# EnricoMiccoli/nodal

Hardware: NVIDIA B200
Metric: unknowns_per_second (higher is better)
Workload: dtype f64

## Files before the change

### __graft_entry__.py

```python
import os
import subprocess
import sys

ROOT = os.path.dirname(os.path.abspath(__file__))
if ROOT not in sys.path:
    sys.path.insert(0, ROOT)


def build():
    subprocess.check_call(["make", "-C", os.path.join(ROOT, "nodal_b200", "csrc"), "-j8"])
    sys.path.insert(0, os.path.join(ROOT, "tests"))
    import helpers
    helpers.stamp_host_lib()
    helpers.amg_host_lib()
    import sources_host
    sources_host.sources_host_lib()
    import amg_cycle_host
    amg_cycle_host.amg_cycle_host_lib()
    ref_nodal = os.path.join(os.environ.get("NODAL_REFERENCE", "/root/reference"), "nodal")
    if os.path.isdir(ref_nodal) and not os.path.isfile(os.path.join(ROOT, "baseline", "_ref", "nodal", "nodal.py")):
        subprocess.call([sys.executable, os.path.join(ROOT, "baseline", "install_ref.py")])
    import nodal_b200
    from nodal_b200 import _lib
    _lib.load()


def smoke():
    import numpy as np
    import nodal_b200 as n
    import nodal_b200.equiv
    from nodal_b200 import dist as ndist
    from nodal_b200 import generators as gen
    from nodal_b200.device import Device
    from oracle import mna_oracle as orc

    N = 24
    r_cpu = orc.equivalent_resistance(orc.grid2d_rows(N), "1", "g", sparse=True, backend="dict")
    r_gpu = n.equiv.equivalent_resistance(gen.grid2d(N), "1", "g", sparse=True)
    r_jac = n.equiv.equivalent_resistance(gen.grid2d(N), "1", "g", sparse=True, precond="jacobi")
    r_amg = n.equiv.equivalent_resistance(gen.grid2d(N), "1", "g", sparse=True, precond="amg", amg={"coarse": 64})
    for r in (r_gpu, r_jac, r_amg):
        assert abs(r - r_cpu) <= 1e-9 * abs(r_cpu), (r, r_cpu)
    dev = Device.get(0)
    import copy
    net = copy.deepcopy(gen.grid2d(64))
    net.process_component(["a1", "A", "1", "1", "g"])
    table = net.table()
    csr, rhs = dev.assemble_csr(table)
    x, info = ndist.single_solver(dev).solve_amg(csr.n, np.array([0, csr.n], dtype=np.int32), csr.indptr, csr.indices,
                                                  csr.data, rhs, rtol=1e-10, gather_below=300)
    r_dist = float(x[net.nodenum["1"]])
    r64 = orc.equivalent_resistance(orc.grid2d_rows(64), "1", "g", sparse=True, backend="dict")
    assert info["status"] == 0 and info["distributed_levels"] >= 1 and abs(r_dist - r64) <= 1e-9 * abs(r64), (info, r_dist, r64)
    pg = gen.power_grid(16, 5, vdd=1.0, load=1e-3, seed=0)
    sol = n.Circuit(pg, sparse=True, eliminate_sources=True).solve()
    red = sol.stats["reduction"]
    assert red["eliminated"] and red["relres_full"] <= 1e-9 and np.all(sol.potentials() <= 1.0), sol.stats
    print(f"smoke ok: R({N}x{N} grid) default={float(r_gpu)!r} jacobi={float(r_jac)!r} amg={float(r_amg)!r} "
          f"oracle={float(r_cpu)!r}; R(64x64) partitioned-AMG form={r_dist!r} oracle={float(r64)!r}; "
          f"power grid 16x16 relres_full={red['relres_full']:.1e}")


if __name__ == "__main__":
    build()
    if len(sys.argv) > 1 and sys.argv[1] == "smoke":
        smoke()
```

### include/nodal_b200.h

```cpp
#ifndef NODAL_B200_H
#define NODAL_B200_H

#include <stdint.h>

#ifdef __cplusplus
extern "C" {
#endif

#define NODAL_ABI_VERSION 1

enum {
    NODAL_OK = 0,
    NODAL_SINGULAR = 1,
    NODAL_NOT_CONVERGED = 2,
    NODAL_BREAKDOWN = 3,
    NODAL_CUDA_ERROR = 4,
    NODAL_BAD_ARG = -1
};

enum { NODAL_T_R = 0, NODAL_T_A = 1, NODAL_T_E = 2, NODAL_T_VCVS = 3, NODAL_T_VCCS = 4,
       NODAL_T_CCVS = 5, NODAL_T_CCCS = 6 };
#define NODAL_GROUND (-1)
#define NODAL_UNUSED (-2)

typedef struct nodal_ctx nodal_ctx;

int nodal_abi_version(void);
const char* nodal_last_error(void);
uint64_t nodal_launch_count(void);
int nodal_ctx_create(int device, nodal_ctx** out);
int nodal_ctx_destroy(nodal_ctx* ctx);
int64_t nodal_ctx_workspace_bytes(nodal_ctx* ctx);

int nodal_stamp_coo(nodal_ctx* ctx, int64_t ncomp,
                    const uint8_t* type, const double* value,
                    const int32_t* a, const int32_t* b, const int32_t* c, const int32_t* d,
                    const int32_t* drv, const int32_t* branch,
                    int32_t kcl, int32_t n, int32_t stride, int32_t colbits,
                    uint64_t* keys, double* vals, void* stream);

int nodal_csr_build(nodal_ctx* ctx, int32_t n, int64_t nslots, int32_t colbits,
                    uint64_t* keys, double* vals, double* rhs,
                    int64_t* nnz_h, void* stream);
int nodal_csr_fetch(nodal_ctx* ctx, int32_t n, int64_t nnz,
                    int32_t* indptr, int32_t* indices, double* data, void* stream);
int nodal_csr_build_ordered(nodal_ctx* ctx, int32_t n, int64_t nslots, int32_t colbits,
                            uint64_t* keys, double* vals, int32_t order, double* rhs, int64_t* nnz_h,
                            void* stream);

int nodal_csr_to_dense(nodal_ctx* ctx, int32_t n, const int32_t* indptr, const int32_t* indices,
                       const double* data, double* G, void* stream);
int nodal_coo_to_dense_atomic(nodal_ctx* ctx, int32_t n, int64_t nslots, int32_t colbits,
                              const uint64_t* keys, const double* vals, double* G, double* rhs,
                              void* stream);

int nodal_spmv(nodal_ctx* ctx, int32_t n, int64_t nnz, const int32_t* indptr,
               const int32_t* indices, const double* data, const double* x, double* y,
               void* stream);

typedef struct nodal_sell nodal_sell;
int nodal_sell_create(nodal_ctx* ctx, int32_t n, int64_t nnz, const int32_t* indptr,
                      const int32_t* indices, const double* data, nodal_sell** out, void* stream);
int nodal_sell_destroy(nodal_sell* m);
int64_t nodal_sell_padded_nnz(const nodal_sell* m);
int nodal_sell_spmv(nodal_ctx* ctx, const nodal_sell* m, const double* x, double* y, void* stream);

int nodal_pcg(nodal_ctx* ctx, int32_t n, int64_t nnz, const int32_t* indptr,
              const int32_t* indices, const double* data, const double* rhs, double* x,
              double rtol, int32_t maxit, int32_t flags,
              int32_t* iters_h, double* relres_h, double* stats_h, void* stream);
#define NODAL_PCG_FORCE_CSR 1
#define NODAL_PCG_NO_GRAPH 2
#define NODAL_PCG_PROFILE 4
#define NODAL_PCG_NO_SCALE 8

int nodal_gmres(nodal_ctx* ctx, int32_t n, int64_t nnz, const int32_t* indptr,
                const int32_t* indices, const double* data, const double* rhs, double* x,
                double rtol, int32_t restart, int32_t maxit,
                int32_t* iters_h, double* relres_h, void* stream);

typedef struct nodal_amg nodal_amg;
int nodal_amg_create(nodal_ctx* ctx, int32_t n, int64_t nnz, const int32_t* indptr,
                     const int32_t* indices, const double* data, const double* params,
                     nodal_amg** out, void* stream);
int nodal_amg_destroy(nodal_amg* amg);
int nodal_amg_info(const nodal_amg* amg, int32_t cap, int32_t* nlevels, int64_t* rows, int64_t* nnz,
                   double* setup_ms, int32_t* direct);
int nodal_amg_fetch_level(nodal_ctx* ctx, const nodal_amg* amg, int32_t level, int32_t* agg,
                          int32_t* indptr, int32_t* indices, double* data, void* stream);
int nodal_amg_apply(nodal_ctx* ctx, const nodal_amg* amg, const double* r, double* z, void* stream);
int nodal_amg_pcg(nodal_ctx* ctx, nodal_amg* amg, const double* rhs, double* x, double rtol,
                  int32_t maxit, int32_t* iters_h, double* relres_h, double* stats_h, void* stream);

int nodal_connected_components(nodal_ctx* ctx, int64_t ncomp, const int32_t* a, const int32_t* b,
                               int32_t kcl, int32_t* labels, int32_t* ncomponents_h,
                               int32_t* reached_h, void* stream);

int nodal_source_forest(nodal_ctx* ctx, int64_t ncomp, const uint8_t* type, const double* value,
                        const int32_t* a, const int32_t* b, const int32_t* branch, int32_t kcl, int32_t be,
                        int32_t* erow, int32_t* adj_ptr, int32_t* adj_row, int32_t* rep_row, double* offset,
                        int32_t* parent_edge, int32_t* depth, int32_t* roots, int64_t* info_h, void* stream);
int nodal_source_reduce_scan(nodal_ctx* ctx, int64_t ncomp, const uint8_t* type, const int32_t* a,
                             const int32_t* b, int32_t kcl, const int32_t* rep_row, const double* offset,
                             uint32_t* pos, int64_t* count_h, void* stream);
int nodal_source_reduce_table(nodal_ctx* ctx, int64_t ncomp, const uint8_t* type, const double* value,
                              const int32_t* a, const int32_t* b, int32_t kcl, const int32_t* rep_row,
                              const double* offset, const uint32_t* pos, uint8_t* out_type, double* out_value,
                              int32_t* out_a, int32_t* out_b, void* stream);
int nodal_source_expand(nodal_ctx* ctx, int32_t kcl, int32_t n, int32_t nsrc, const int32_t* erow,
                        const int32_t* a, const int32_t* b, const int32_t* branch, const int32_t* adj_ptr,
                        const int32_t* adj_row, const int32_t* rep_row, const double* offset,
                        const int32_t* depth, int32_t max_depth, const double* y, const double* rhs,
                        int64_t nnz, const int32_t* indptr, const int32_t* indices, const double* data,
                        double* x, double* relres_h, void* stream);
int nodal_source_potentials(nodal_ctx* ctx, int32_t kcl, int32_t n, const int32_t* rep_row, const double* offset,
                            const double* y, double* x, void* stream);
int nodal_source_tree_rows(nodal_ctx* ctx, int32_t kcl, int32_t n, int64_t nnz_full, int32_t rb, int32_t re,
                           const int32_t* depth, const double* rhs, int64_t nnz, const int32_t* indptr,
                           const int32_t* indices, const double* data, const double* x, int32_t* out_row,
                           double* out_rhs, double* out_gx, int64_t* count_h, void* stream);
int nodal_source_currents(nodal_ctx* ctx, int32_t kcl, int32_t nsrc, const int32_t* erow, const int32_t* a,
                          const int32_t* b, const int32_t* branch, const int32_t* adj_ptr, const int32_t* adj_row,
                          const int32_t* depth, int32_t max_depth, int64_t ntree, const int32_t* tree_row,
                          const double* tree_rhs, const double* tree_gx, double* x, void* stream);
int nodal_source_residual(nodal_ctx* ctx, int32_t n, int64_t nnz_full, int32_t rows, const double* rhs, int64_t nnz,
                          const int32_t* indptr, const int32_t* indices, const double* data, const double* x,
                          double* sums_h, void* stream);

int nodal_lu_solve(nodal_ctx* ctx, int32_t n, double* G, const double* rhs, double* x,
                   int32_t* info_h, void* stream);

int nodal_dgemm_sub_profile(nodal_ctx* ctx, double* C, const double* A, const double* B, int32_t M, int32_t N,
                            int32_t K, int32_t ld, int32_t reps, double* ms_out, void* stream);

int nodal_lu_batched(nodal_ctx* ctx, int64_t batch, int32_t ncomp,
                     const uint8_t* type, const int32_t* a, const int32_t* b,
                     const int32_t* c, const int32_t* d, const int32_t* drv, const int32_t* branch,
                     int32_t kcl, int32_t n, const double* values, double* x, int32_t* info,
                     void* stream);

int nodal_lu_batched_soa(nodal_ctx* ctx, int64_t batch, int32_t ncomp,
                         const uint8_t* type, const int32_t* a, const int32_t* b,
                         const int32_t* c, const int32_t* d, const int32_t* drv, const int32_t* branch,
                         int32_t kcl, int32_t n, const double* values_t, double* x_t, int32_t* info,
                         void* stream);

typedef struct nodal_dist nodal_dist;
int nodal_dist_unique_id(uint8_t id_h[128]);
int nodal_dist_create(nodal_ctx* ctx, const uint8_t id_h[128], int32_t rank, int32_t nranks,
                      nodal_dist** out);
int nodal_dist_create_single(nodal_ctx* ctx, nodal_dist** out);
int nodal_dist_destroy(nodal_dist* d);
int nodal_dist_pcg(nodal_ctx* ctx, nodal_dist* d, int32_t n_global, const int32_t* bounds_h,
                   int64_t nnz, const int32_t* indptr, const int32_t* indices, const double* data,
                   const double* rhs_local, double* x_local,
                   double rtol, int32_t maxit,
                   int32_t* iters_h, double* relres_h, double* stats_h, void* stream);

int nodal_amg_pcg_multi(nodal_ctx* ctx, nodal_amg* amg, int32_t K, const double* rhs, double* x, double rtol,
                        int32_t maxit, int32_t* iters_h, double* relres_h, int32_t* status_h, void* stream);

int nodal_amg_profile_sweeps(nodal_ctx* ctx, nodal_amg* h, int32_t reps, double* ms_out, void* stream);

int nodal_amg_profile_cycle(nodal_ctx* ctx, nodal_amg* h, int32_t reps, double* ms_out, void* stream);

int nodal_table_select_scan(nodal_ctx* ctx, int64_t ncomp, const int32_t* a, const int32_t* b,
                            int32_t rb, int32_t re, uint32_t* pos, int64_t* count_h, void* stream);
int nodal_table_select_gather(nodal_ctx* ctx, int64_t ncomp, const uint32_t* pos, int32_t rb, int32_t re,
                              const uint8_t* type, const double* value, const int32_t* a, const int32_t* b,
                              const int32_t* c, const int32_t* d, const int32_t* drv, const int32_t* branch,
                              uint8_t* out_type, double* out_value, int32_t* out_a, int32_t* out_b,
                              int32_t* out_c, int32_t* out_d, int32_t* out_drv, int32_t* out_branch,
                              void* stream);
int nodal_table_select_mna_scan(nodal_ctx* ctx, int64_t ncomp, const uint8_t* type, const int32_t* a,
                                const int32_t* b, const int32_t* branch, int32_t kcl, int32_t rb, int32_t re,
                                uint32_t* pos, int64_t* count_h, void* stream);
int nodal_table_select_mna_gather(nodal_ctx* ctx, int64_t ncomp, const uint32_t* pos, int32_t kcl, int32_t rb,
                                  int32_t re, const uint8_t* type, const double* value, const int32_t* a,
                                  const int32_t* b, const int32_t* c, const int32_t* d, const int32_t* drv,
                                  const int32_t* branch, uint8_t* out_type, double* out_value, int32_t* out_a,
                                  int32_t* out_b, int32_t* out_c, int32_t* out_d, int32_t* out_drv,
                                  int32_t* out_branch, void* stream);
int nodal_table_select_type_scan(nodal_ctx* ctx, int64_t ncomp, const uint8_t* type, const int32_t* a,
                                 const int32_t* b, int32_t t, uint32_t* pos, int64_t* count_h, void* stream);
int nodal_table_select_type_gather(nodal_ctx* ctx, int64_t ncomp, const uint32_t* pos, int32_t t,
                                   const uint8_t* type, const double* value, const int32_t* a, const int32_t* b,
                                   const int32_t* c, const int32_t* d, const int32_t* drv, const int32_t* branch,
                                   uint8_t* out_type, double* out_value, int32_t* out_a, int32_t* out_b,
                                   int32_t* out_c, int32_t* out_d, int32_t* out_drv, int32_t* out_branch,
                                   void* stream);

int nodal_dist_amg_pcg(nodal_ctx* ctx, nodal_dist* d, int32_t n_global, const int32_t* bounds_h,
                       int64_t nnz, const int32_t* indptr, const int32_t* indices, const double* data,
                       const double* rhs_local, double* x_local, const double* params,
                       double rtol, int32_t maxit,
                       int32_t* iters_h, double* relres_h, double* stats_h, void* stream);

#ifdef __cplusplus
}
#endif
#endif
```

### nodal_b200/_lib.py

```python
from __future__ import annotations

import ctypes as C
import os

_HERE = os.path.dirname(os.path.abspath(__file__))
LIB_PATH = os.path.join(_HERE, "libnodal_b200.so")

OK, SINGULAR, NOT_CONVERGED, BREAKDOWN, CUDA_ERROR, BAD_ARG = 0, 1, 2, 3, 4, -1
PCG_FORCE_CSR, PCG_NO_GRAPH, PCG_PROFILE, PCG_NO_SCALE = 1, 2, 4, 8

_vp, _i32, _i64, _f64 = C.c_void_p, C.c_int32, C.c_int64, C.c_double

SIGNATURES = {
    "nodal_abi_version": (C.c_int, []),
    "nodal_last_error": (C.c_char_p, []),
    "nodal_launch_count": (C.c_uint64, []),
    "nodal_ctx_create": (C.c_int, [C.c_int, C.POINTER(_vp)]),
    "nodal_ctx_destroy": (C.c_int, [_vp]),
    "nodal_ctx_workspace_bytes": (_i64, [_vp]),
    "nodal_stamp_coo": (C.c_int, [_vp, _i64, _vp, _vp, _vp, _vp, _vp, _vp, _vp, _vp,
                                  _i32, _i32, _i32, _i32, _vp, _vp, _vp]),
    "nodal_csr_build": (C.c_int, [_vp, _i32, _i64, _i32, _vp, _vp, _vp, C.POINTER(_i64), _vp]),
    "nodal_csr_build_ordered": (C.c_int, [_vp, _i32, _i64, _i32, _vp, _vp, _i32, _vp, C.POINTER(_i64), _vp]),
    "nodal_csr_fetch": (C.c_int, [_vp, _i32, _i64, _vp, _vp, _vp, _vp]),
    "nodal_csr_to_dense": (C.c_int, [_vp, _i32, _vp, _vp, _vp, _vp, _vp]),
    "nodal_coo_to_dense_atomic": (C.c_int, [_vp, _i32, _i64, _i32, _vp, _vp, _vp, _vp, _vp]),
    "nodal_spmv": (C.c_int, [_vp, _i32, _i64, _vp, _vp, _vp, _vp, _vp, _vp]),
    "nodal_sell_create": (C.c_int, [_vp, _i32, _i64, _vp, _vp, _vp, C.POINTER(_vp), _vp]),
    "nodal_sell_destroy": (C.c_int, [_vp]),
    "nodal_sell_padded_nnz": (_i64, [_vp]),
    "nodal_sell_spmv": (C.c_int, [_vp, _vp, _vp, _vp, _vp]),
    "nodal_pcg": (C.c_int, [_vp, _i32, _i64, _vp, _vp, _vp, _vp, _vp, _f64, _i32, _i32,
                            C.POINTER(_i32), C.POINTER(_f64), C.POINTER(_f64), _vp]),
    "nodal_gmres": (C.c_int, [_vp, _i32, _i64, _vp, _vp, _vp, _vp, _vp, _f64, _i32, _i32,
                              C.POINTER(_i32), C.POINTER(_f64), _vp]),
    "nodal_amg_create": (C.c_int, [_vp, _i32, _i64, _vp, _vp, _vp, C.POINTER(_f64), C.POINTER(_vp), _vp]),
    "nodal_amg_destroy": (C.c_int, [_vp]),
    "nodal_amg_info": (C.c_int, [_vp, _i32, C.POINTER(_i32), C.POINTER(_i64), C.POINTER(_i64),
                                 C.POINTER(_f64), C.POINTER(_i32)]),
    "nodal_amg_fetch_level": (C.c_int, [_vp, _vp, _i32, _vp, _vp, _vp, _vp, _vp]),
    "nodal_amg_apply": (C.c_int, [_vp, _vp, _vp, _vp, _vp]),
    "nodal_amg_pcg": (C.c_int, [_vp, _vp, _vp, _vp, _f64, _i32, C.POINTER(_i32), C.POINTER(_f64),
                                C.POINTER(_f64), _vp]),
    "nodal_connected_components": (C.c_int, [_vp, _i64, _vp, _vp, _i32, _vp, C.POINTER(_i32),
                                             C.POINTER(_i32), _vp]),
    "nodal_source_forest": (C.c_int, [_vp, _i64, _vp, _vp, _vp, _vp, _vp, _i32, _i32] + [_vp] * 8
                            + [C.POINTER(_i64), _vp]),
    "nodal_source_reduce_scan": (C.c_int, [_vp, _i64, _vp, _vp, _vp, _i32, _vp, _vp, _vp, C.POINTER(_i64), _vp]),
    "nodal_source_reduce_table": (C.c_int, [_vp, _i64, _vp, _vp, _vp, _vp, _i32, _vp, _vp, _vp, _vp, _vp, _vp, _vp,
                                            _vp]),
    "nodal_source_expand": (C.c_int, [_vp, _i32, _i32, _i32] + [_vp] * 9 + [_i32, _vp, _vp, _i64, _vp, _vp, _vp, _vp,
                                                                             C.POINTER(_f64), _vp]),
    "nodal_lu_solve": (C.c_int, [_vp, _i32, _vp, _vp, _vp, C.POINTER(_i32), _vp]),
    "nodal_dgemm_sub_profile": (C.c_int, [_vp, _vp, _vp, _vp, _i32, _i32, _i32, _i32, _i32, C.POINTER(_f64), _vp]),
    "nodal_lu_batched": (C.c_int, [_vp, _i64, _i32, _vp, _vp, _vp, _vp, _vp, _vp, _vp,
                                   _i32, _i32, _vp, _vp, _vp, _vp]),
    "nodal_lu_batched_soa": (C.c_int, [_vp, _i64, _i32, _vp, _vp, _vp, _vp, _vp, _vp, _vp,
                                       _i32, _i32, _vp, _vp, _vp, _vp]),
    "nodal_dist_unique_id": (C.c_int, [_vp]),
    "nodal_dist_create": (C.c_int, [_vp, _vp, _i32, _i32, C.POINTER(_vp)]),
    "nodal_dist_create_single": (C.c_int, [_vp, C.POINTER(_vp)]),
    "nodal_dist_destroy": (C.c_int, [_vp]),
    "nodal_dist_pcg": (C.c_int, [_vp, _vp, _i32, _vp, _i64, _vp, _vp, _vp, _vp, _vp, _f64, _i32,
                                 C.POINTER(_i32), C.POINTER(_f64), C.POINTER(_f64), _vp]),
    "nodal_amg_pcg_multi": (C.c_int, [_vp, _vp, _i32, _vp, _vp, _f64, _i32, C.POINTER(_i32), C.POINTER(_f64),
                                      C.POINTER(_i32), _vp]),
    "nodal_amg_profile_sweeps": (C.c_int, [_vp, _vp, _i32, C.POINTER(_f64), _vp]),
    "nodal_amg_profile_cycle": (C.c_int, [_vp, _vp, _i32, C.POINTER(_f64), _vp]),
    "nodal_table_select_scan": (C.c_int, [_vp, _i64, _vp, _vp, _i32, _i32, _vp, C.POINTER(_i64), _vp]),
    "nodal_table_select_gather": (C.c_int, [_vp, _i64, _vp, _i32, _i32] + [_vp] * 16 + [_vp]),
    "nodal_table_select_mna_scan": (C.c_int, [_vp, _i64, _vp, _vp, _vp, _vp, _i32, _i32, _i32, _vp, C.POINTER(_i64),
                                              _vp]),
    "nodal_table_select_mna_gather": (C.c_int, [_vp, _i64, _vp, _i32, _i32, _i32] + [_vp] * 16 + [_vp]),
    "nodal_table_select_type_scan": (C.c_int, [_vp, _i64, _vp, _vp, _vp, _i32, _vp, C.POINTER(_i64), _vp]),
    "nodal_table_select_type_gather": (C.c_int, [_vp, _i64, _vp, _i32] + [_vp] * 16 + [_vp]),
    "nodal_source_potentials": (C.c_int, [_vp, _i32, _i32, _vp, _vp, _vp, _vp, _vp]),
    "nodal_source_tree_rows": (C.c_int, [_vp, _i32, _i32, _i64, _i32, _i32, _vp, _vp, _i64, _vp, _vp, _vp, _vp, _vp,
                                         _vp, _vp, C.POINTER(_i64), _vp]),
    "nodal_source_currents": (C.c_int, [_vp, _i32, _i32] + [_vp] * 7 + [_i32, _i64, _vp, _vp, _vp, _vp, _vp]),
    "nodal_source_residual": (C.c_int, [_vp, _i32, _i64, _i32, _vp, _i64, _vp, _vp, _vp, _vp, C.POINTER(_f64), _vp]),
    "nodal_dist_amg_pcg": (C.c_int, [_vp, _vp, _i32, _vp, _i64, _vp, _vp, _vp, _vp, _vp, C.POINTER(_f64), _f64,
                                     _i32, C.POINTER(_i32), C.POINTER(_f64), C.POINTER(_f64), _vp]),
}

_lib = None


class NodalLibraryError(RuntimeError):
    """The CUDA extension is missing or a CUDA call failed."""


def load():
    global _lib
    if _lib is not None:
        return _lib
    if not os.path.exists(LIB_PATH):
        raise NodalLibraryError(
            f"{LIB_PATH} not found: build it with `python -c 'import __graft_entry__ as g; g.build()'`"
            " (or `make -C nodal_b200/csrc`). nodal_b200 has no CPU fallback.")
    lib = C.CDLL(LIB_PATH)
    for name, (res, args) in SIGNATURES.items():
        fn = getattr(lib, name)
        fn.restype = res
        fn.argtypes = args
    if lib.nodal_abi_version() != 1:
        raise NodalLibraryError("libnodal_b200.so ABI version mismatch")
    _lib = lib
    return lib


def last_error():
    return load().nodal_last_error().decode("utf-8", "replace")


def check(status, what, allowed=(OK,)):
    if status in allowed:
        return status
    raise NodalLibraryError(f"{what} failed with status {status}: {last_error()}")
```

### nodal_b200/csrc/amg.cu

```cuda
#include <algorithm>
#include <cmath>

#include "amg_host.cuh"

void amg_free_csr(nodal_ctx* ctx, AmgCsr& a) {
    if (a.owned) {
        ctx_pool_free(ctx, const_cast<int32_t*>(a.indptr));
        ctx_pool_free(ctx, const_cast<int32_t*>(a.indices));
        ctx_pool_free(ctx, const_cast<double*>(a.data));
    }
    a = AmgCsr();
}

int amg_aggregate(nodal_ctx* ctx, int rounds, const AmgCsr& A, int32_t nown, int32_t base,
                  int32_t** agg_out, int32_t* nc_out, cudaStream_t st) {
    const int32_t n = A.n;
    AmgScratch<int32_t> match(ctx, n), best(ctx, n);
    AmgScratch<u32> leader(ctx, n);
    if (!match.ptr || !best.ptr || !leader.ptr) return NODAL_CUDA_ERROR;
    const int grid = amg_rows_grid(ctx, n);
    CUDA_TRY(cudaMemsetAsync(match, 0xFF, sizeof(int32_t) * (size_t)n, st));
    for (int r = 0; r < rounds; ++r) {
        amg_propose_kernel<<<grid, AT, 0, st>>>(n, A.indptr, A.indices, A.data, match, best, nown, base);
        KERNEL_CHECK();
        amg_accept_kernel<<<grid, AT, 0, st>>>(n, best, match);
        KERNEL_CHECK();
    }
    int32_t* root = best;
    amg_root_kernel<<<grid, AT, 0, st>>>(n, A.indptr, A.indices, A.data, match, root, leader, nown, base);
    KERNEL_CHECK();
    NODAL_TRY(ctx_reserve(ctx, scan_scratch_bytes(n) + 4096));
    u32* total = carve<u32>(ctx, 16);
    if (!total) return NODAL_CUDA_ERROR;
    NODAL_TRY(scan_exclusive_u32(ctx, leader, leader, n, total, st));
    int32_t* agg = match;
    amg_assign_kernel<<<grid, AT, 0, st>>>(n, root, leader, agg);
    KERNEL_CHECK();
    u32* total_h = reinterpret_cast<u32*>(ctx->pinned);
    CUDA_TRY(cudaMemcpyAsync(total_h, total, sizeof(u32), cudaMemcpyDeviceToHost, st));
    CUDA_TRY(cudaStreamSynchronize(st));
    *nc_out = (int32_t)total_h[0];
    *agg_out = match.keep();
    return NODAL_OK;
}

int amg_transpose_pattern(nodal_ctx* ctx, int32_t n, const int32_t* agg, int32_t** pt_ptr_out,
                          int32_t** pt_idx_out, cudaStream_t st) {
    AmgScratch<u64> keys(ctx, n);
    AmgScratch<double> vals(ctx, n), rhs(ctx, (size_t)n + 1), ones(ctx, n);
    if (!keys.ptr || !vals.ptr || !rhs.ptr || !ones.ptr) return NODAL_CUDA_ERROR;
    const int cb = amg_bit_length(n);
    amg_pt_keys_kernel<<<amg_rows_grid(ctx, n), AT, 0, st>>>(n, agg, cb, keys, vals);
    KERNEL_CHECK();
    int64_t cnt = 0;
    NODAL_TRY(nodal_csr_build(ctx, n, n, cb, reinterpret_cast<uint64_t*>(keys.ptr), vals, rhs, &cnt, st));
    if (cnt != n) {
        nodal_set_error("amg: internal error, P^T has %lld entries for %d rows", (long long)cnt, n);
        return NODAL_CUDA_ERROR;
    }
    AmgScratch<int32_t> pp(ctx, (size_t)n + 1), pi(ctx, n);
    if (!pp.ptr || !pi.ptr) return NODAL_CUDA_ERROR;
    NODAL_TRY(nodal_csr_fetch(ctx, n, n, pp, pi, ones, st));
    *pt_ptr_out = pp.keep();
    *pt_idx_out = pi.keep();
    return NODAL_OK;
}

int amg_members(nodal_ctx* ctx, int32_t n, const int32_t* agg, int32_t nc, int32_t** pt_ptr_out,
                int32_t** pt_idx_out, cudaStream_t st) {
    AmgScratch<u32> cnt(ctx, (size_t)nc + 1), cursor(ctx, (size_t)nc + 1);
    AmgScratch<int32_t> pp(ctx, (size_t)nc + 1), pi(ctx, (size_t)std::max(n, 1));
    if (!cnt.ptr || !cursor.ptr || !pp.ptr || !pi.ptr) return NODAL_CUDA_ERROR;
    CUDA_TRY(cudaMemsetAsync(cnt, 0, sizeof(u32) * ((size_t)nc + 1), st));
    CUDA_TRY(cudaMemsetAsync(cursor, 0, sizeof(u32) * ((size_t)nc + 1), st));
    const int grid = amg_rows_grid(ctx, n);
    amg_count_members_kernel<<<grid, AT, 0, st>>>(n, agg, cnt);
    KERNEL_CHECK();
    NODAL_TRY(ctx_reserve(ctx, scan_scratch_bytes((int64_t)nc + 1) + 4096));
    NODAL_TRY(scan_exclusive_u32(ctx, cnt, reinterpret_cast<u32*>(pp.ptr), (int64_t)nc + 1, nullptr, st));
    amg_place_members_kernel<<<grid, AT, 0, st>>>(n, agg, pp, cursor, pi);
    KERNEL_CHECK();
    amg_sort_members_kernel<<<amg_rows_grid(ctx, nc), AT, 0, st>>>(nc, pp, pi);
    KERNEL_CHECK();
    *pt_ptr_out = pp.keep();
    *pt_idx_out = pi.keep();
    return NODAL_OK;
}

int amg_galerkin_merge(nodal_ctx* ctx, const AmgCsr& A, const int32_t* pt_ptr, const int32_t* pt_idx, int32_t nc,
                       const int32_t* label, int32_t ncol_limit, AmgCsr* out, cudaStream_t st) {
    if (A.nnz >= ((int64_t)1 << 32) - 1) return NODAL_BAD_ARG;
    AmgScratch<u32> bound(ctx, (size_t)nc + 1), kept(ctx, (size_t)nc + 1);
    AmgScratch<int32_t> tmp_cols(ctx, (size_t)std::max<int64_t>(A.nnz, 1)), ip(ctx, (size_t)nc + 1);
    AmgScratch<double> tmp_vals(ctx, (size_t)std::max<int64_t>(A.nnz, 1));
    if (!bound.ptr || !kept.ptr || !tmp_cols.ptr || !tmp_vals.ptr || !ip.ptr) return NODAL_CUDA_ERROR;
    const int grid = amg_rows_grid(ctx, nc);
    CUDA_TRY(cudaMemsetAsync(bound.ptr + nc, 0, sizeof(u32), st));
    CUDA_TRY(cudaMemsetAsync(kept.ptr + nc, 0, sizeof(u32), st));
    amg_merge_bound_kernel<<<grid, AT, 0, st>>>(nc, pt_ptr, pt_idx, A.indptr, bound);
    KERNEL_CHECK();
    NODAL_TRY(ctx_reserve(ctx, scan_scratch_bytes((int64_t)nc + 1) + 4096));
    u32* total = carve<u32>(ctx, 16);
    if (!total) return NODAL_CUDA_ERROR;
    const size_t mark = ctx->arena_used;
    NODAL_TRY(scan_exclusive_u32(ctx, bound, bound, (int64_t)nc + 1, nullptr, st));
    ctx->arena_used = mark;
    amg_merge_rows_kernel<<<grid, AT, 0, st>>>(nc, pt_ptr, pt_idx, A.indptr, A.indices, A.data, label, ncol_limit,
                                               bound, tmp_cols, tmp_vals, kept);
    KERNEL_CHECK();
    NODAL_TRY(scan_exclusive_u32(ctx, kept, reinterpret_cast<u32*>(ip.ptr), (int64_t)nc + 1, total, st));
    u32* total_h = reinterpret_cast<u32*>(ctx->pinned);
    CUDA_TRY(cudaMemcpyAsync(total_h, total, sizeof(u32), cudaMemcpyDeviceToHost, st));
    CUDA_TRY(cudaStreamSynchronize(st));
    const int64_t nnzc = total_h[0];
    AmgScratch<int32_t> ix(ctx, (size_t)std::max<int64_t>(nnzc, 1));
    AmgScratch<double> dv(ctx, (size_t)std::max<int64_t>(nnzc, 1));
    if (!ix.ptr || !dv.ptr) return NODAL_CUDA_ERROR;
    amg_merge_compact_kernel<<<grid, AT, 0, st>>>(nc, bound, ip, tmp_cols, tmp_vals, ix, dv);
    KERNEL_CHECK();
    out->n = nc;
    out->nnz = nnzc;
    out->indptr = ip.keep();
    out->indices = ix.keep();
    out->data = dv.keep();
    out->owned = true;
    return NODAL_OK;
}

namespace {

int rows_grid(const nodal_ctx* ctx, int64_t work) { return amg_rows_grid(ctx, work); }
int sell_grid(const nodal_ctx* ctx, int32_t nslices) { return amg_sell_grid(ctx, nslices); }
int bit_length(int64_t v) { return amg_bit_length(v); }
template <typename T>
T* pool(nodal_ctx* ctx, size_t count) { return amg_pool<T>(ctx, count); }
template <typename T>
using Scratch = AmgScratch<T>;
using Csr = AmgCsr;
void free_csr(nodal_ctx* ctx, Csr& a) { amg_free_csr(ctx, a); }
int aggregate(nodal_amg* h, const Csr& A, int32_t** agg_out, int32_t* nc_out, cudaStream_t st) {
    return amg_aggregate(h->ctx, h->rounds, A, 0x7fffffff, 0, agg_out, nc_out, st);
}

bool sorted_galerkin() {
    static const bool on = getenv("NODAL_AMG_SORT_GALERKIN") != nullptr;
    return on;
}

int galerkin(nodal_amg* h, const Csr& A, const int32_t* agg, int32_t nc, Csr* out, cudaStream_t st) {
    nodal_ctx* ctx = h->ctx;
    if (!sorted_galerkin() && amg_merge_pays(A.nnz, nc)) {
        int32_t *pp = nullptr, *pi = nullptr;
        NODAL_TRY(amg_members(ctx, A.n, agg, nc, &pp, &pi, st));
        const int rc = amg_galerkin_merge(ctx, A, pp, pi, nc, agg, 0x7fffffff, out, st);
        ctx_pool_free(ctx, pp);
        ctx_pool_free(ctx, pi);
        return rc;
    }
    Scratch<u64> keys(ctx, A.nnz);
    Scratch<double> vals(ctx, A.nnz), rhs(ctx, (size_t)nc + 1);
    if (!keys.ptr || !vals.ptr || !rhs.ptr) return NODAL_CUDA_ERROR;
    const int cb = bit_length(nc);
    amg_relabel_kernel<<<rows_grid(ctx, A.n), AT, 0, st>>>(A.n, A.indptr, A.indices, A.data, agg, cb,
                                                         keys, vals);
    KERNEL_CHECK();
    int64_t nnzc = 0;
    NODAL_TRY(nodal_csr_build(ctx, nc, A.nnz, cb, reinterpret_cast<uint64_t*>(keys.ptr), vals, rhs,
                              &nnzc, st));
    Scratch<int32_t> ip(ctx, (size_t)nc + 1), ix(ctx, nnzc);
    Scratch<double> dv(ctx, nnzc);
    if (!ip.ptr || !ix.ptr || !dv.ptr) return NODAL_CUDA_ERROR;
    NODAL_TRY(nodal_csr_fetch(ctx, nc, nnzc, ip, ix, dv, st));
    out->n = nc;
    out->nnz = nnzc;
    out->indptr = ip.keep();
    out->indices = ix.keep();
    out->data = dv.keep();
    out->owned = true;
    return NODAL_OK;
}

int transpose_pattern(nodal_amg* h, AmgLevel& L, cudaStream_t st) {
    if (!sorted_galerkin()) return amg_members(h->ctx, L.n, L.agg, L.nc, &L.pt_ptr, &L.pt_idx, st);
    return amg_transpose_pattern(h->ctx, L.n, L.agg, &L.pt_ptr, &L.pt_idx, st);
}

int invert_coarsest(nodal_amg* h, const AmgLevel& L, cudaStream_t st) {
    nodal_ctx* ctx = h->ctx;
    const int32_t n = L.n;
    const size_t elems = (size_t)n * 2 * n;
    Scratch<double> m0(ctx, elems + 32), m1(ctx, elems);
    if (!m0.ptr || !m1.ptr) return NODAL_CUDA_ERROR;
    int* bad = reinterpret_cast<int*>(m0.ptr + elems);
    CUDA_TRY(cudaMemsetAsync(m0, 0, sizeof(double) * (elems + 32), st));
    amg_dense_init_kernel<<<rows_grid(ctx, n), AT, 0, st>>>(n, L.indptr, L.indices, L.data, m0);
    KERNEL_CHECK();
    double *src = m0.ptr, *dst = m1.ptr;
    const int grid = rows_grid(ctx, (int64_t)elems);
    for (int32_t k = 0; k < n; ++k) {
        amg_gj_step_kernel<<<grid, AT, 0, st>>>(n, k, src, dst, bad);
        KERNEL_CHECK();
        std::swap(src, dst);
    }
    h->inv = pool<double>(ctx, (size_t)n * n);
    if (!h->inv) return NODAL_CUDA_ERROR;
    amg_dense_extract_kernel<<<rows_grid(ctx, (int64_t)n * n), AT, 0, st>>>(n, src, h->inv);
    KERNEL_CHECK();
    int* bad_h = reinterpret_cast<int*>(ctx->pinned);
    CUDA_TRY(cudaMemcpyAsync(bad_h, bad, sizeof(int), cudaMemcpyDeviceToHost, st));
    CUDA_TRY(cudaStreamSynchronize(st));
    if (*bad_h != 0) {
        nodal_set_error("amg: the coarsest operator is not positive definite (pivot %d of %d); "
                        "the matrix is not SPD", *bad_h, n);
        return NODAL_BREAKDOWN;
    }
    return NODAL_OK;
}

int build_hierarchy(nodal_amg* h, int32_t n, int64_t nnz, const int32_t* indptr, const int32_t* indices,
                    const double* data, cudaStream_t st) {
    nodal_ctx* ctx = h->ctx;
    Csr cur;
    cur.n = n; cur.nnz = nnz; cur.indptr = indptr; cur.indices = indices; cur.data = data;
    while (cur.n > h->coarse && (int)h->lv.size() < h->maxlevels) {
        Csr A = cur;
        A.owned = false;
        int32_t* comp = nullptr;
        int rc = NODAL_OK;
        for (int pass = 0; pass < h->passes && rc == NODAL_OK; ++pass) {
            int32_t* agg = nullptr;
            int32_t nc = 0;
            Csr Ac;
            rc = aggregate(h, A, &agg, &nc, st);
            if (rc == NODAL_OK) rc = galerkin(h, A, agg, nc, &Ac, st);
            if (rc == NODAL_OK && comp) {
                amg_compose_kernel<<<rows_grid(ctx, cur.n), AT, 0, st>>>(cur.n, comp, agg);
                ++g_nodal_launches;
                if (cudaGetLastError() != cudaSuccess) {
                    nodal_set_error("amg: amg_compose_kernel launch failed");
                    rc = NODAL_CUDA_ERROR;
                }
            }
            if (!comp) comp = agg;
            else ctx_pool_free(ctx, agg);
            free_csr(ctx, A);
            A = Ac;
        }
        double total_nnz = (double)cur.nnz + (double)A.nnz;
        for (const AmgLevel& P : h->lv) total_nnz += (double)P.nnz;
        const bool too_dense = (double)A.nnz > h->max_fill * (double)cur.nnz ||
                               total_nnz > h->max_complexity * (double)(h->lv.empty() ? cur.nnz : h->lv[0].nnz);
        if (rc != NODAL_OK || (double)A.n > 0.9 * (double)cur.n || too_dense) {
            free_csr(ctx, A);
            ctx_pool_free(ctx, comp);
            if (rc != NODAL_OK) {
                free_csr(ctx, cur);
                return rc;
            }
            break;
        }
        AmgLevel L;
        L.n = cur.n; L.nnz = cur.nnz; L.indptr = cur.indptr; L.indices = cur.indices; L.data = cur.data;
        L.owned = cur.owned;
        L.agg = comp;
        L.nc = A.n;
        h->lv.push_back(L);
        cur = A;
        rc = transpose_pattern(h, h->lv.back(), st);
        if (rc != NODAL_OK) {
            free_csr(ctx, cur);
            return rc;
        }
    }
    AmgLevel L;
    L.n = cur.n; L.nnz = cur.nnz; L.indptr = cur.indptr; L.indices = cur.indices; L.data = cur.data;
    L.owned = cur.owned;
    h->lv.push_back(L);
    for (size_t l = 0; l < h->lv.size(); ++l) {
        AmgLevel& V = h->lv[l];
        NODAL_TRY(sell_from_csr(ctx, V.n, V.nnz, V.indptr, V.indices, V.data, &V.sell, st, nullptr));
        V.x = pool<double>(ctx, V.n);
        V.r = pool<double>(ctx, V.n);
        if (l > 0) V.b = pool<double>(ctx, V.n);
        if (!V.x || !V.r || (l > 0 && !V.b)) return NODAL_CUDA_ERROR;
    }
    if (h->lv.back().n <= h->direct_max) NODAL_TRY(invert_coarsest(h, h->lv.back(), st));
    return NODAL_OK;
}

template <int MODE>
int sell_sweep(const nodal_amg* h, const AmgLevel& V, const double* b, const double* x, double* y,
               double* part, cudaStream_t st) {
    const nodal_sell* m = V.sell;
    amg_sell_kernel<MODE><<<sell_grid(h->ctx, m->nslices), AT, 0, st>>>(
        m->n, m->nslices, m->slice_w, m->cols, m->vals, m->dinv, b, x, h->omega, y, part);
    KERNEL_CHECK();
    return NODAL_OK;
}

template <int MODE>
int cycle_sweep(const nodal_amg* h, const AmgLevel& V, const double* b, const double* xc, double* y,
                cudaStream_t st) {
    const nodal_sell* m = V.sell;
    amg_cycle_sweep_kernel<MODE><<<sell_grid(h->ctx, m->nslices), AT, 0, st>>>(
        m->n, m->nslices, m->slice_w, m->cols, m->vals, m->dinv, b, h->omega, V.agg, xc, h->scale, y);
    KERNEL_CHECK();
    return NODAL_OK;
}

int cycle(const nodal_amg* h, const double* b0, double* z0, cudaStream_t st) {
    const nodal_ctx* ctx = h->ctx;
    const int last = (int)h->lv.size() - 1;
    for (int l = 0; l < last; ++l) {
        const AmgLevel& V = h->lv[l];
        const double* b = l == 0 ? b0 : V.b;
        NODAL_TRY(cycle_sweep<1>(h, V, b, nullptr, V.r, st));
        amg_restrict_kernel<<<rows_grid(ctx, V.nc), AT, 0, st>>>(V.nc, V.pt_ptr, V.pt_idx, V.r,
                                                              h->lv[l + 1].b);
        KERNEL_CHECK();
    }
    {
        const AmgLevel& V = h->lv[last];
        const double* b = last == 0 ? b0 : V.b;
        double* x = last == 0 ? z0 : V.x;
        if (h->inv) amg_gemv_kernel<<<rows_grid(ctx, (int64_t)V.n * 32), AT, 0, st>>>(V.n, h->inv, b, x);
        else amg_jacobi0_kernel<<<rows_grid(ctx, V.n), AT, 0, st>>>(V.n, V.sell->dinv, b, h->omega, x);
        KERNEL_CHECK();
    }
    for (int l = last - 1; l >= 0; --l) {
        const AmgLevel& V = h->lv[l];
        const double* b = l == 0 ? b0 : V.b;
        NODAL_TRY(cycle_sweep<2>(h, V, b, h->lv[l + 1].x, l == 0 ? z0 : V.x, st));
    }
    return NODAL_OK;
}

}

extern "C" int nodal_amg_destroy(nodal_amg* h) {
    if (!h) return NODAL_OK;
    cudaSetDevice(h->device);
    nodal_ctx* ctx = h->ctx;
    for (AmgLevel& V : h->lv) {
        sell_free(V.sell);
        if (V.owned) {
            ctx_pool_free(ctx, const_cast<int32_t*>(V.indptr));
            ctx_pool_free(ctx, const_cast<int32_t*>(V.indices));
            ctx_pool_free(ctx, const_cast<double*>(V.data));
        }
        ctx_pool_free(ctx, V.agg);
        ctx_pool_free(ctx, V.pt_ptr);
        ctx_pool_free(ctx, V.pt_idx);
        ctx_pool_free(ctx, V.b);
        ctx_pool_free(ctx, V.x);
        ctx_pool_free(ctx, V.r);
    }
    ctx_pool_free(ctx, h->inv);
    ctx_pool_free(ctx, h->p);
    ctx_pool_free(ctx, h->q);
    ctx_pool_free(ctx, h->r);
    ctx_pool_free(ctx, h->z);
    ctx_pool_free(ctx, h->part);
    delete h;
    return NODAL_OK;
}

extern "C" int nodal_amg_create(nodal_ctx* ctx, int32_t n, int64_t nnz, const int32_t* indptr,
                                const int32_t* indices, const double* data, const double* params,
                                nodal_amg** out, void* stream) {
    NvtxRange nvtx_range("nodal_amg_create");
    if (!ctx || n < 0 || nnz < 0 || !out) return NODAL_BAD_ARG;
    *out = nullptr;
    cudaStream_t st = (cudaStream_t)stream;
    CUDA_TRY(cudaSetDevice(ctx->device));
    nodal_amg* h = new nodal_amg();
    h->ctx = ctx;
    h->device = ctx->device;
    if (params) {
        if (params[0] >= 1.0) h->passes = (int)params[0];
        if (params[1] >= 1.0) h->coarse = (int)params[1];
        if (params[2] > 0.0) h->omega = params[2];
        if (params[3] > 0.0) h->scale = params[3];
        if (params[4] >= 1.0) h->maxlevels = (int)params[4];
        if (params[5] >= 1.0) h->rounds = (int)params[5];
        if (params[6] >= 1.0) h->direct_max = (int)params[6];
        if (params[7] > 0.0) h->max_fill = params[7];
    }
    cudaEvent_t e0, e1;
    CUDA_TRY(cudaEventCreate(&e0));
    CUDA_TRY(cudaEventCreate(&e1));
    cudaEventRecord(e0, st);
    int rc = NODAL_OK;
    if (n > 0) rc = build_hierarchy(h, n, nnz, indptr, indices, data, st);
    if (rc == NODAL_OK && n > 0) {
        h->nparts = std::max(sell_grid(ctx, h->lv[0].sell->nslices), rows_grid(ctx, n));
        h->p = pool<double>(ctx, n);
        h->q = pool<double>(ctx, n);
        h->r = pool<double>(ctx, n);
        h->z = pool<double>(ctx, n);
        h->part = pool<double>(ctx, 3 * (size_t)h->nparts + 16);
        if (!h->p || !h->q || !h->r || !h->z || !h->part) rc = NODAL_CUDA_ERROR;
    }
    cudaEventRecord(e1, st);
    if (cudaEventSynchronize(e1) == cudaSuccess) cudaEventElapsedTime(&h->setup_ms, e0, e1);
    cudaEventDestroy(e0);
    cudaEventDestroy(e1);
    if (rc != NODAL_OK) {
        nodal_amg_destroy(h);
        return rc;
    }
    *out = h;
    return NODAL_OK;
}

extern "C" int nodal_amg_info(const nodal_amg* h, int32_t cap, int32_t* nlevels, int64_t* rows,
                              int64_t* nnz, double* setup_ms, int32_t* direct) {
    if (!h || !nlevels) return NODAL_BAD_ARG;
    *nlevels = (int32_t)h->lv.size();
    for (int32_t l = 0; l < *nlevels && l < cap; ++l) {
        if (rows) rows[l] = h->lv[l].n;
        if (nnz) nnz[l] = h->lv[l].nnz;
    }
    if (setup_ms) *setup_ms = h->setup_ms;
    if (direct) *direct = h->inv ? 1 : 0;
    return NODAL_OK;
}

extern "C" int nodal_amg_fetch_level(nodal_ctx* ctx, const nodal_amg* h, int32_t level, int32_t* agg,
                                     int32_t* indptr, int32_t* indices, double* data, void* stream) {
    if (!ctx || !h || level < 0 || level >= (int32_t)h->lv.size()) return NODAL_BAD_ARG;
    cudaStream_t st = (cudaStream_t)stream;
    CUDA_TRY(cudaSetDevice(ctx->device));
    const AmgLevel& V = h->lv[level];
    if (agg) {
        if (!V.agg) return NODAL_BAD_ARG;
        CUDA_TRY(cudaMemcpyAsync(agg, V.agg, sizeof(int32_t) * (size_t)V.n, cudaMemcpyDeviceToDevice, st));
    }
    if (indptr) CUDA_TRY(cudaMemcpyAsync(indptr, V.indptr, sizeof(int32_t) * ((size_t)V.n + 1), cudaMemcpyDeviceToDevice, st));
    if (indices) CUDA_TRY(cudaMemcpyAsync(indices, V.indices, sizeof(int32_t) * (size_t)V.nnz, cudaMemcpyDeviceToDevice, st));
    if (data) CUDA_TRY(cudaMemcpyAsync(data, V.data, sizeof(double) * (size_t)V.nnz, cudaMemcpyDeviceToDevice, st));
    return NODAL_OK;
}

extern "C" int nodal_amg_apply(nodal_ctx* ctx, const nodal_amg* h, const double* r, double* z,
                               void* stream) {
    if (!ctx || !h || h->ctx != ctx) return NODAL_BAD_ARG;
    if (h->lv.empty()) return NODAL_OK;
    CUDA_TRY(cudaSetDevice(ctx->device));
    return cycle(h, r, z, (cudaStream_t)stream);
}

extern "C" int nodal_amg_pcg(nodal_ctx* ctx, nodal_amg* h, const double* rhs, double* x, double rtol,
                             int32_t maxit, int32_t* iters_h, double* relres_h, double* stats_h,
                             void* stream) {
    NvtxRange nvtx_range("nodal_amg_pcg");
    if (!ctx || !h || h->ctx != ctx || !iters_h || !relres_h) return NODAL_BAD_ARG;
    *iters_h = 0;
    *relres_h = 0.0;
    if (stats_h) memset(stats_h, 0, 16 * sizeof(double));
    if (h->lv.empty()) return NODAL_OK;
    cudaStream_t st = (cudaStream_t)stream;
    CUDA_TRY(cudaSetDevice(ctx->device));
    const AmgLevel& A = h->lv[0];
    const int32_t n = A.n;
    const int gv = rows_grid(ctx, n);
    const int gs = sell_grid(ctx, A.sell->nslices);
    double* part_pq = h->part;
    double* part_rr = h->part + h->nparts;
    double* part_rz = h->part + 2 * (size_t)h->nparts;
    double* scal = h->part + 3 * (size_t)h->nparts;
    double* host = reinterpret_cast<double*>(ctx->pinned);
    cudaEvent_t e0, e1;
    CUDA_TRY(cudaEventCreate(&e0));
    CUDA_TRY(cudaEventCreate(&e1));
    int iters = 0, restarts = 0, rc = NODAL_NOT_CONVERGED;
    double relres = 0.0;
    bool timed = false;

    auto dot_to_host = [&](const double* a, const double* b, double* result) -> int {
        apcg_dot_kernel<<<gv, AT, 0, st>>>(n, a, b, part_rr);
        KERNEL_CHECK();
        apcg_sum_kernel<<<1, AT, 0, st>>>(part_rr, gv, scal + 2);
        KERNEL_CHECK();
        CUDA_TRY(cudaMemcpyAsync(host, scal + 2, sizeof(double), cudaMemcpyDeviceToHost, st));
        CUDA_TRY(cudaStreamSynchronize(st));
        *result = host[0];
        return NODAL_OK;
    };
    auto run = [&]() -> int {
        CUDA_TRY(cudaEventRecord(e0, st));
        double bb = 0.0, rr = 0.0;
        NODAL_TRY(dot_to_host(rhs, rhs, &bb));
        if (!(bb > 0.0)) {
            if (bb == 0.0) {
                CUDA_TRY(cudaMemsetAsync(x, 0, sizeof(double) * (size_t)n, st));
                rc = NODAL_OK;
                return NODAL_OK;
            }
            nodal_set_error("nodal_amg_pcg: the right-hand side is not finite");
            rc = NODAL_BREAKDOWN;
            return NODAL_OK;
        }
        const double bnorm = sqrt(bb);
        NODAL_TRY(sell_sweep<1>(h, A, rhs, x, h->r, nullptr, st));
        NODAL_TRY(dot_to_host(h->r, h->r, &rr));
        relres = sqrt(rr) / bnorm;
        while (true) {
            if (relres <= rtol) { rc = NODAL_OK; break; }
            if (iters >= maxit) { rc = NODAL_NOT_CONVERGED; break; }
            if (restarts > 8) { rc = NODAL_NOT_CONVERGED; break; }
            int par = 0;
            NODAL_TRY(cycle(h, h->r, h->z, st));
            apcg_dot_kernel<<<gv, AT, 0, st>>>(n, h->r, h->z, part_rz);
            KERNEL_CHECK();
            apcg_direction_kernel<<<gv, AT, 0, st>>>(n, part_rz, gv, scal + (par ^ 1), scal + par, h->z, h->p, 1);
            KERNEL_CHECK();
            bool broke = false;
            while (iters < maxit) {
                NODAL_TRY(sell_sweep<0>(h, A, nullptr, h->p, h->q, part_pq, st));
                apcg_update_kernel<<<gv, AT, 0, st>>>(n, part_pq, gs, scal + par, h->p, h->q, x, h->r, part_rr);
                KERNEL_CHECK();
                apcg_sum_kernel<<<1, AT, 0, st>>>(part_rr, gv, scal + 2);
                KERNEL_CHECK();
                CUDA_TRY(cudaMemcpyAsync(host, scal + 2, sizeof(double), cudaMemcpyDeviceToHost, st));
                CUDA_TRY(cudaStreamSynchronize(st));
                ++iters;
                rr = host[0];
                if (!std::isfinite(rr)) { broke = true; break; }
                if (sqrt(rr) <= rtol * bnorm) break;
                NODAL_TRY(cycle(h, h->r, h->z, st));
                apcg_dot_kernel<<<gv, AT, 0, st>>>(n, h->r, h->z, part_rz);
                KERNEL_CHECK();
                apcg_direction_kernel<<<gv, AT, 0, st>>>(n, part_rz, gv, scal + par, scal + (par ^ 1), h->z, h->p, 0);
                KERNEL_CHECK();
                par ^= 1;
            }
            if (broke) {
                nodal_set_error("nodal_amg_pcg: breakdown (non-finite residual) at iteration %d", iters);
                rc = NODAL_BREAKDOWN;
                break;
            }
            NODAL_TRY(sell_sweep<1>(h, A, rhs, x, h->r, nullptr, st));
            NODAL_TRY(dot_to_host(h->r, h->r, &rr));
            relres = sqrt(rr) / bnorm;
            if (!std::isfinite(relres)) { rc = NODAL_BREAKDOWN; break; }
            if (relres > rtol) ++restarts;
        }
        CUDA_TRY(cudaEventRecord(e1, st));
        CUDA_TRY(cudaEventSynchronize(e1));
        timed = true;
        return NODAL_OK;
    };
    const int st_run = run();
    float ms = 0.f;
    if (st_run == NODAL_OK && timed) cudaEventElapsedTime(&ms, e0, e1);
    cudaEventDestroy(e0);
    cudaEventDestroy(e1);
    if (st_run != NODAL_OK) return st_run;
    *iters_h = iters;
    *relres_h = relres;
    if (stats_h) {
        double rows = 0.0, nnz = 0.0;
        for (const AmgLevel& V : h->lv) { rows += V.n; nnz += (double)V.nnz; }
        stats_h[0] = (double)h->lv.size();
        stats_h[1] = A.nnz ? nnz / (double)A.nnz : 0.0;
        stats_h[2] = restarts;
        stats_h[3] = ms;
        stats_h[4] = h->setup_ms;
        stats_h[5] = h->lv.back().n;
        stats_h[6] = n ? rows / n : 0.0;
        stats_h[7] = h->inv ? 1.0 : 0.0;
    }
    return rc;
}

extern "C" int nodal_amg_profile_sweeps(nodal_ctx* ctx, nodal_amg* h, int32_t reps, double* ms_out, void* stream) {
    if (!ctx || !h || h->ctx != ctx || !ms_out || reps < 1 || h->lv.empty()) return NODAL_BAD_ARG;
    cudaStream_t st = (cudaStream_t)stream;
    CUDA_TRY(cudaSetDevice(ctx->device));
    const AmgLevel& A = h->lv[0];
    CUDA_TRY(cudaMemsetAsync(h->p, 0, sizeof(double) * (size_t)A.n, st));
    CUDA_TRY(cudaMemsetAsync(h->r, 0, sizeof(double) * (size_t)A.n, st));
    cudaEvent_t e0, e1;
    CUDA_TRY(cudaEventCreate(&e0));
    CUDA_TRY(cudaEventCreate(&e1));
    int rc = NODAL_OK;
    for (int mode = 0; mode < 3 && rc == NODAL_OK; ++mode) {
        for (int k = -2; k < reps && rc == NODAL_OK; ++k) {
            if (k == 0) cudaEventRecord(e0, st);
            if (mode == 0) rc = sell_sweep<0>(h, A, nullptr, h->p, h->q, h->part, st);
            if (mode == 1) rc = sell_sweep<1>(h, A, h->r, h->p, h->q, nullptr, st);
            if (mode == 2) rc = sell_sweep<2>(h, A, h->r, h->p, h->q, nullptr, st);
        }
        cudaEventRecord(e1, st);
        float ms = 0.f;
        if (cudaEventSynchronize(e1) == cudaSuccess) cudaEventElapsedTime(&ms, e0, e1);
        ms_out[mode] = ms / reps;
    }
    cudaEventDestroy(e0);
    cudaEventDestroy(e1);
    return rc;
}

extern "C" int nodal_amg_profile_cycle(nodal_ctx* ctx, nodal_amg* h, int32_t reps, double* ms_out, void* stream) {
    if (!ctx || !h || h->ctx != ctx || !ms_out || reps < 1 || h->lv.size() < 2) return NODAL_BAD_ARG;
    cudaStream_t st = (cudaStream_t)stream;
    CUDA_TRY(cudaSetDevice(ctx->device));
    const AmgLevel& A = h->lv[0];
    const AmgLevel& C = h->lv[1];
    double* b = h->r;
    CUDA_TRY(cudaMemsetAsync(b, 0, sizeof(double) * (size_t)A.n, st));
    CUDA_TRY(cudaMemsetAsync(A.x, 0, sizeof(double) * (size_t)A.n, st));
    CUDA_TRY(cudaMemsetAsync(C.x, 0, sizeof(double) * (size_t)C.n, st));
    cudaEvent_t e0, e1;
    CUDA_TRY(cudaEventCreate(&e0));
    CUDA_TRY(cudaEventCreate(&e1));
    int rc = NODAL_OK;
    for (int k = 0; k < 6 && rc == NODAL_OK; ++k) {
        for (int i = -2; i < reps && rc == NODAL_OK; ++i) {
            if (i == 0) cudaEventRecord(e0, st);
            switch (k) {
                case 0:
                    amg_jacobi0_kernel<<<rows_grid(ctx, A.n), AT, 0, st>>>(A.n, A.sell->dinv, b, h->omega, A.x);
                    KERNEL_CHECK();
                    break;
                case 1: rc = sell_sweep<1>(h, A, b, A.x, A.r, nullptr, st); break;
                case 2:
                    amg_prolong_kernel<<<rows_grid(ctx, A.n), AT, 0, st>>>(A.n, A.agg, C.x, h->scale, A.x, A.r);
                    KERNEL_CHECK();
                    break;
                case 3: rc = sell_sweep<2>(h, A, b, A.r, h->z, nullptr, st); break;
                case 4: rc = cycle_sweep<1>(h, A, b, nullptr, A.r, st); break;
                default: rc = cycle_sweep<2>(h, A, b, C.x, h->z, st); break;
            }
        }
        cudaEventRecord(e1, st);
        float ms = 0.f;
        if (cudaEventSynchronize(e1) == cudaSuccess) cudaEventElapsedTime(&ms, e0, e1);
        ms_out[k] = ms / reps;
    }
    cudaEventDestroy(e0);
    cudaEventDestroy(e1);
    return rc;
}
```

### nodal_b200/csrc/amg_kernels.cuh

```cuda
#pragma once
#include "amg_core.cuh"
#include "amg_merge_core.cuh"
#include "sparse.cuh"

constexpr int AT = 256;

#define ROW_LOOP(i, n)                                                              \
    for (int64_t i = (int64_t)blockIdx.x * blockDim.x + threadIdx.x; i < (int64_t)(n); \
         i += (int64_t)gridDim.x * blockDim.x)

static __global__ void __launch_bounds__(AT)
amg_propose_kernel(int32_t n, const int32_t* __restrict__ indptr, const int32_t* __restrict__ indices,
                   const double* __restrict__ data, const int32_t* __restrict__ match,
                   int32_t* __restrict__ best, int32_t nown, int32_t base) {
    ROW_LOOP(i, n) best[i] = match[i] >= 0 ? -1 : amg_pick((int32_t)i, indptr, indices, data, match, nown, base);
}

static __global__ void __launch_bounds__(AT)
amg_accept_kernel(int32_t n, const int32_t* __restrict__ best, int32_t* __restrict__ match) {
    ROW_LOOP(i, n) {
        if (match[i] >= 0) continue;
        const int32_t b = best[i];
        if (b >= 0 && best[b] == (int32_t)i) match[i] = b;
    }
}

static __global__ void __launch_bounds__(AT)
amg_root_kernel(int32_t n, const int32_t* __restrict__ indptr, const int32_t* __restrict__ indices,
                const double* __restrict__ data, const int32_t* __restrict__ match,
                int32_t* __restrict__ root, u32* __restrict__ leader, int32_t nown, int32_t base) {
    ROW_LOOP(i, n) {
        const int32_t r = amg_root((int32_t)i, indptr, indices, data, match, nown, base);
        root[i] = r;
        leader[i] = r == (int32_t)i ? 1u : 0u;
    }
}

static __global__ void __launch_bounds__(AT)
amg_assign_kernel(int32_t n, const int32_t* __restrict__ root, const u32* __restrict__ ids,
                  int32_t* __restrict__ agg) {
    ROW_LOOP(i, n) agg[i] = (int32_t)ids[root[i]];
}

static __global__ void __launch_bounds__(AT)
amg_compose_kernel(int32_t n, int32_t* __restrict__ comp, const int32_t* __restrict__ next) {
    ROW_LOOP(i, n) comp[i] = next[comp[i]];
}

static __global__ void __launch_bounds__(AT)
amg_relabel_kernel(int32_t n, const int32_t* __restrict__ indptr, const int32_t* __restrict__ indices,
                   const double* __restrict__ data, const int32_t* __restrict__ agg, int cb,
                   u64* __restrict__ keys, double* __restrict__ vals) {
    ROW_LOOP(i, n) {
        const u64 hi = (u64)agg[i] << cb;
        const int32_t e = indptr[i + 1];
        for (int32_t p = indptr[i]; p < e; ++p) {
            keys[p] = hi | (u64)agg[indices[p]];
            vals[p] = data[p];
        }
    }
}

static __global__ void __launch_bounds__(AT)
amg_pt_keys_kernel(int32_t n, const int32_t* __restrict__ agg, int cb, u64* __restrict__ keys,
                   double* __restrict__ vals) {
    ROW_LOOP(i, n) {
        keys[i] = ((u64)agg[i] << cb) | (u64)i;
        vals[i] = 1.0;
    }
}

static __global__ void __launch_bounds__(AT)
amg_dense_init_kernel(int32_t n, const int32_t* __restrict__ indptr, const int32_t* __restrict__ indices,
                      const double* __restrict__ data, double* __restrict__ M) {
    const int64_t W = 2 * (int64_t)n;
    ROW_LOOP(i, n) {
        M[i * W + n + i] = 1.0;
        const int32_t e = indptr[i + 1];
        for (int32_t p = indptr[i]; p < e; ++p) M[i * W + indices[p]] = data[p];
    }
}

static __global__ void __launch_bounds__(AT)
amg_gj_step_kernel(int32_t n, int32_t k, const double* __restrict__ src, double* __restrict__ dst,
                   int* __restrict__ bad) {
    const int64_t W = 2 * (int64_t)n;
    const double piv = src[k * W + k];
    if (blockIdx.x == 0 && threadIdx.x == 0 && !(piv > 0.0) && *bad == 0) *bad = k + 1;
    ROW_LOOP(idx, (int64_t)n * W) {
        const int64_t i = idx / W, j = idx - i * W;
        const double rkj = src[k * W + j] / piv;
        dst[idx] = i == k ? rkj : src[idx] - src[i * W + k] * rkj;
    }
}

static __global__ void __launch_bounds__(AT)
amg_dense_extract_kernel(int32_t n, const double* __restrict__ M, double* __restrict__ inv) {
    const int64_t W = 2 * (int64_t)n;
    ROW_LOOP(idx, (int64_t)n * n) {
        const int64_t i = idx / n, j = idx - i * n;
        inv[idx] = M[i * W + n + j];
    }
}

static __global__ void __launch_bounds__(AT)
amg_gemv_kernel(int32_t n, const double* __restrict__ inv, const double* __restrict__ b,
                double* __restrict__ x) {
    const int lane = threadIdx.x & 31;
    const int64_t warp = ((int64_t)blockIdx.x * blockDim.x + threadIdx.x) >> 5;
    const int64_t nwarps = ((int64_t)gridDim.x * blockDim.x) >> 5;
    for (int64_t r = warp; r < n; r += nwarps) {
        double acc = 0.0;
        for (int32_t j = lane; j < n; j += 32) acc = fma(inv[r * n + j], b[j], acc);
        acc = warp_sum(acc);
        if (lane == 0) x[r] = acc;
    }
}

static __global__ void __launch_bounds__(AT)
amg_jacobi0_kernel(int32_t n, const double* __restrict__ dinv, const double* __restrict__ b,
                   double omega, double* __restrict__ x) {
    ROW_LOOP(i, n) x[i] = amg_jacobi_start(omega, dinv[i], b[i]);
}

template <int MODE>
static __global__ void __launch_bounds__(AT, 5)
amg_sell_kernel(int32_t n, int32_t nslices, const u32* __restrict__ slice_w,
                const int32_t* __restrict__ cols, const double* __restrict__ vals,
                const double* __restrict__ dinv, const double* __restrict__ b,
                const double* __restrict__ x, double omega, double* __restrict__ y,
                double* __restrict__ part) {
    __shared__ double red[33];
    const int lane = threadIdx.x & 31;
    const int64_t warp = ((int64_t)blockIdx.x * blockDim.x + threadIdx.x) >> 5;
    const int64_t nwarps = ((int64_t)gridDim.x * blockDim.x) >> 5;
    double dot = 0.0;
    for (int64_t s = warp; s < nslices; s += nwarps) {
        const u32 w0 = slice_w[s];
        const int w = (int)(slice_w[s + 1] - w0);
        const double acc = sell_row_dot(cols, vals, (int64_t)w0 * 32 + lane, w, x);
        const int64_t r = s * 32 + lane;
        if (r < n) {
            if (MODE == 0) { y[r] = acc; dot = fma(x[r], acc, dot); }
            if (MODE == 1) y[r] = amg_residual(b[r], acc);
            if (MODE == 2) y[r] = amg_jacobi_update(omega, dinv[r], b[r], acc, x[r]);
        }
    }
    if (MODE == 0) {
        const double t = block_sum(dot, red);
        if (threadIdx.x == 0) part[blockIdx.x] = t;
    }
}

static __global__ void __launch_bounds__(AT)
amg_restrict_kernel(int32_t nc, const int32_t* __restrict__ pt_ptr, const int32_t* __restrict__ pt_idx,
                    const double* __restrict__ r, double* __restrict__ bc) {
    ROW_LOOP(I, nc) {
        double s = 0.0;
        const int32_t e = pt_ptr[I + 1];
        for (int32_t p = pt_ptr[I]; p < e; ++p) s += r[pt_idx[p]];
        bc[I] = s;
    }
}

static __global__ void __launch_bounds__(AT)
amg_prolong_kernel(int32_t n, const int32_t* __restrict__ agg, const double* __restrict__ xc,
                   double scale, const double* __restrict__ x, double* __restrict__ xa) {
    ROW_LOOP(i, n) xa[i] = amg_prolong_add(scale, xc[agg[i]], x[i]);
}

struct JacobiStartAt {
    const double* __restrict__ dinv;
    const double* __restrict__ b;
    double omega;
    __device__ __forceinline__ double operator()(int32_t c) const {
        return amg_jacobi_start(omega, __ldg(&dinv[c]), __ldg(&b[c]));
    }
};

struct ProlongatedAt {
    JacobiStartAt x0;
    const int32_t* __restrict__ agg;
    const double* __restrict__ xc;
    double scale;
    __device__ __forceinline__ double operator()(int32_t c) const {
        return amg_prolong_add(scale, __ldg(&xc[__ldg(&agg[c])]), x0(c));
    }
};

template <int MODE>
static __global__ void __launch_bounds__(AT, 5)
amg_cycle_sweep_kernel(int32_t n, int32_t nslices, const u32* __restrict__ slice_w,
                       const int32_t* __restrict__ cols, const double* __restrict__ vals,
                       const double* __restrict__ dinv, const double* __restrict__ b, double omega,
                       const int32_t* __restrict__ agg, const double* __restrict__ xc, double scale,
                       double* __restrict__ y) {
    const int lane = threadIdx.x & 31;
    const int64_t warp = ((int64_t)blockIdx.x * blockDim.x + threadIdx.x) >> 5;
    const int64_t nwarps = ((int64_t)gridDim.x * blockDim.x) >> 5;
    const JacobiStartAt x0{dinv, b, omega};
    const ProlongatedAt xa{x0, agg, xc, scale};
    for (int64_t s = warp; s < nslices; s += nwarps) {
        const u32 w0 = slice_w[s];
        const int w = (int)(slice_w[s + 1] - w0);
        const int64_t base = (int64_t)w0 * 32 + lane;
        const int64_t r = s * 32 + lane;
        if (MODE == 1) {
            const double acc = sell_row_gather(cols, vals, base, w, x0);
            if (r < n) y[r] = amg_residual(b[r], acc);
        }
        if (MODE == 2) {
            const double acc = sell_row_gather(cols, vals, base, w, xa);
            if (r < n) y[r] = amg_jacobi_update(omega, dinv[r], b[r], acc, xa((int32_t)r));
        }
    }
}

static __global__ void __launch_bounds__(AT)
apcg_dot_kernel(int32_t n, const double* __restrict__ a, const double* __restrict__ b,
                double* __restrict__ part) {
    __shared__ double red[33];
    double t = 0.0;
    ROW_LOOP(i, n) t = fma(a[i], b[i], t);
    t = block_sum(t, red);
    if (threadIdx.x == 0) part[blockIdx.x] = t;
}

static __global__ void __launch_bounds__(AT)
apcg_sum_kernel(const double* __restrict__ part, int count, double* __restrict__ out) {
    __shared__ double red[33];
    const double t = reduce_partials(part, count, red);
    if (threadIdx.x == 0) out[0] = t;
}

static __global__ void __launch_bounds__(AT)
apcg_update_kernel(int32_t n, const double* __restrict__ part_pq, int npq, const double* __restrict__ rz,
                   const double* __restrict__ p, const double* __restrict__ q, double* __restrict__ x,
                   double* __restrict__ r, double* __restrict__ part_rr) {
    __shared__ double red[33];
    const double pq = reduce_partials(part_pq, npq, red);
    const double alpha = rz[0] / pq;
    double t = 0.0;
    ROW_LOOP(i, n) {
        x[i] = fma(alpha, p[i], x[i]);
        const double ri = fma(-alpha, q[i], r[i]);
        r[i] = ri;
        t = fma(ri, ri, t);
    }
    t = block_sum(t, red);
    if (threadIdx.x == 0) part_rr[blockIdx.x] = t;
}

static __global__ void __launch_bounds__(AT)
apcg_direction_kernel(int32_t n, const double* __restrict__ part_rz, int nrz,
                      const double* __restrict__ rz_old, double* __restrict__ rz_new,
                      const double* __restrict__ z, double* __restrict__ p, int first) {
    __shared__ double red[33];
    const double rzn = reduce_partials(part_rz, nrz, red);
    const double beta = first ? 0.0 : rzn / rz_old[0];
    ROW_LOOP(i, n) p[i] = first ? z[i] : fma(beta, p[i], z[i]);
    if (blockIdx.x == 0 && threadIdx.x == 0) rz_new[0] = rzn;
}


static __global__ void __launch_bounds__(AT)
amg_count_members_kernel(int32_t n, const int32_t* __restrict__ agg, u32* __restrict__ cnt) {
    ROW_LOOP(i, n) atomicAdd(&cnt[agg[i]], 1u);
}

static __global__ void __launch_bounds__(AT)
amg_place_members_kernel(int32_t n, const int32_t* __restrict__ agg, const int32_t* __restrict__ pt_ptr,
                         u32* __restrict__ cursor, int32_t* __restrict__ pt_idx) {
    ROW_LOOP(i, n) {
        const int32_t a = agg[i];
        pt_idx[pt_ptr[a] + (int32_t)atomicAdd(&cursor[a], 1u)] = (int32_t)i;
    }
}

static __global__ void __launch_bounds__(AT)
amg_sort_members_kernel(int32_t nc, const int32_t* __restrict__ pt_ptr, int32_t* __restrict__ pt_idx) {
    ROW_LOOP(I, nc) {
        const int32_t b = pt_ptr[I], e = pt_ptr[I + 1];
        for (int32_t p = b + 1; p < e; ++p) {
            const int32_t v = pt_idx[p];
            int32_t q = p;
            while (q > b && pt_idx[q - 1] > v) { pt_idx[q] = pt_idx[q - 1]; --q; }
            pt_idx[q] = v;
        }
    }
}

static __global__ void __launch_bounds__(AT)
amg_merge_bound_kernel(int32_t nc, const int32_t* __restrict__ pt_ptr, const int32_t* __restrict__ pt_idx,
                       const int32_t* __restrict__ indptr, u32* __restrict__ bound) {
    ROW_LOOP(I, nc) bound[I] = (u32)amg_merge_bound((int32_t)I, pt_ptr, pt_idx, indptr);
}

static __global__ void __launch_bounds__(AT)
amg_merge_rows_kernel(int32_t nc, const int32_t* __restrict__ pt_ptr, const int32_t* __restrict__ pt_idx,
                      const int32_t* __restrict__ indptr, const int32_t* __restrict__ indices,
                      const double* __restrict__ data, const int32_t* __restrict__ label, int32_t ncol_limit,
                      const u32* __restrict__ off, int32_t* tmp_cols, double* tmp_vals, u32* __restrict__ kept) {
    constexpr int LOCAL = 32;
    ROW_LOOP(I, nc) {
        const u32 o = off[I];
        if (off[I + 1] - o <= (u32)LOCAL) {
            int32_t lc[LOCAL];
            double lv[LOCAL];
            const int32_t k = amg_merge_row((int32_t)I, pt_ptr, pt_idx, indptr, indices, data, label, lc, lv, ncol_limit);
            for (int32_t e = 0; e < k; ++e) { tmp_cols[o + e] = lc[e]; tmp_vals[o + e] = lv[e]; }
            kept[I] = (u32)k;
        } else {
            kept[I] = (u32)amg_merge_row((int32_t)I, pt_ptr, pt_idx, indptr, indices, data, label, tmp_cols + o,
                                         tmp_vals + o, ncol_limit);
        }
    }
}

static __global__ void __launch_bounds__(AT)
amg_merge_compact_kernel(int32_t nc, const u32* __restrict__ off, const int32_t* __restrict__ out_ptr,
                         const int32_t* __restrict__ tmp_cols, const double* __restrict__ tmp_vals,
                         int32_t* __restrict__ out_cols, double* __restrict__ out_vals) {
    ROW_LOOP(I, nc) {
        const int32_t b = out_ptr[I], cnt = out_ptr[I + 1] - b;
        const u32 src = off[I];
        for (int32_t k = 0; k < cnt; ++k) {
            out_cols[b + k] = tmp_cols[src + k];
            out_vals[b + k] = tmp_vals[src + k];
        }
    }
}
```

### nodal_b200/csrc/dist_amg.cu

```cuda
#include <algorithm>
#include <chrono>
#include <cmath>
#include <memory>
#include <vector>

#include "amg_host.cuh"
#include "dist_common.cuh"
#include "pcg_kernels.cuh"

namespace {

constexpr int DA = 256;
constexpr size_t AMG_HDR = 8192;
constexpr int AMG_SLOTS = 60;
struct AmgMail {
    double red[2][P2P_MAXR][4];
    unsigned long long rtag[2][P2P_MAXR];
    unsigned long long flag[AMG_SLOTS][P2P_MAXR];
    unsigned long long cnt[AMG_SLOTS];
    unsigned int ticket[AMG_SLOTS];
    unsigned long long rseq;
    unsigned long long err;
};
static_assert(sizeof(AmgMail) <= AMG_HDR, "mailbox must fit the header");

#define GRID_LOOP(i, n)                                                                \
    for (int64_t i = (int64_t)blockIdx.x * blockDim.x + threadIdx.x; i < (int64_t)(n); \
         i += (int64_t)gridDim.x * blockDim.x)

__global__ void __launch_bounds__(DA)
da_flag_external_kernel(int64_t nnz, const int32_t* __restrict__ cols, int32_t rb, int32_t re, u32* __restrict__ flag) {
    GRID_LOOP(i, nnz) { const int32_t c = cols[i]; flag[i] = (c < rb || c >= re) ? 1u : 0u; }
}
__global__ void __launch_bounds__(DA)
da_compact_external_kernel(int64_t nnz, const int32_t* __restrict__ cols, int32_t rb, int32_t re,
                           const u32* __restrict__ pos, u64* __restrict__ keys) {
    GRID_LOOP(i, nnz) { const int32_t c = cols[i]; if (c < rb || c >= re) keys[pos[i]] = (u64)(u32)c; }
}
__global__ void __launch_bounds__(DA)
da_unique_flag_kernel(int64_t m, const u64* __restrict__ keys, u32* __restrict__ flag) {
    GRID_LOOP(i, m) flag[i] = (i == 0 || keys[i] != keys[i - 1]) ? 1u : 0u;
}
__global__ void __launch_bounds__(DA)
da_unique_compact_kernel(int64_t m, const u64* __restrict__ keys, const u32* __restrict__ pos, int32_t* __restrict__ halo) {
    GRID_LOOP(i, m) if (i == 0 || keys[i] != keys[i - 1]) halo[pos[i]] = (int32_t)keys[i];
}
__global__ void __launch_bounds__(DA)
da_remap_kernel(int64_t nnz, const int32_t* __restrict__ cols, int32_t rb, int32_t re,
                const int32_t* __restrict__ halo, int32_t nhalo, int32_t* __restrict__ out) {
    const int32_t nloc = re - rb;
    GRID_LOOP(i, nnz) {
        const int32_t c = cols[i];
        if (c >= rb && c < re) { out[i] = c - rb; continue; }
        int lo = 0, hi = nhalo - 1;
        while (lo < hi) {
            const int mid = (lo + hi) >> 1;
            if (halo[mid] < c) lo = mid + 1; else hi = mid;
        }
        out[i] = nloc + lo;
    }
}
__global__ void __launch_bounds__(DA)
da_rebase_kernel(int64_t m, int32_t* __restrict__ idx, int32_t rb) { GRID_LOOP(i, m) idx[i] -= rb; }
__global__ void __launch_bounds__(DA)
da_gather_kernel(int64_t m, const int32_t* __restrict__ idx, const double* __restrict__ src, double* __restrict__ dst) {
    GRID_LOOP(i, m) dst[i] = src[idx[i]];
}

__global__ void __launch_bounds__(DA)
da_labels_kernel(int32_t n, const int32_t* __restrict__ comp, int32_t first, double* __restrict__ lab) {
    GRID_LOOP(i, n) lab[i] = (double)(first + comp[i]);
}
__global__ void __launch_bounds__(DA)
da_relabel_local_kernel(int32_t n, const int32_t* __restrict__ indptr, const int32_t* __restrict__ lcols,
                        const double* __restrict__ data, const int32_t* __restrict__ agg, int32_t nown,
                        int32_t nc, int cb, u64* __restrict__ keys, double* __restrict__ vals) {
    GRID_LOOP(i, n) {
        const u64 hi = (u64)agg[i] << cb;
        const int32_t e = indptr[i + 1];
        for (int32_t p = indptr[i]; p < e; ++p) {
            const int32_t c = lcols[p];
            keys[p] = c < nown ? (hi | (u64)agg[c]) : ((u64)nc << cb);
            vals[p] = data[p];
        }
    }
}
__global__ void __launch_bounds__(DA)
da_relabel_global_kernel(int32_t n, const int32_t* __restrict__ indptr, const int32_t* __restrict__ lcols,
                         const double* __restrict__ data, const double* __restrict__ lab, int cb,
                         u64* __restrict__ keys, double* __restrict__ vals) {
    GRID_LOOP(i, n) {
        const u64 hi = (u64)(int64_t)lab[i] << cb;
        const int32_t e = indptr[i + 1];
        for (int32_t p = indptr[i]; p < e; ++p) {
            keys[p] = hi | (u64)(int64_t)lab[lcols[p]];
            vals[p] = data[p];
        }
    }
}
__global__ void __launch_bounds__(DA)
da_labels_to_i32_kernel(int32_t n, const double* __restrict__ lab, int32_t* __restrict__ out) {
    GRID_LOOP(i, n) out[i] = (int32_t)lab[i];
}
__global__ void __launch_bounds__(DA)
da_slice_indptr_kernel(int32_t nloc, const int32_t* __restrict__ src, int32_t* __restrict__ dst) {
    const int32_t first = src[0];
    GRID_LOOP(i, (int64_t)nloc + 1) dst[i] = src[i] - first;
}
__global__ void __launch_bounds__(DA)
da_offset_indptr_kernel(int32_t count, int32_t* __restrict__ indptr, int32_t add) {
    GRID_LOOP(i, count) indptr[i] += add;
}
__global__ void da_set_i32_kernel(int32_t* p, int32_t v) { if (threadIdx.x == 0 && blockIdx.x == 0) *p = v; }

__global__ void __launch_bounds__(1024)
da_exchange_kernel(const PcgDev* __restrict__ dev, int slot, int R, int me, long long voff,
                   const double* __restrict__ src, const int32_t* __restrict__ send_idx,
                   const int32_t* __restrict__ send_off, const long long* __restrict__ dest_off,
                   const int32_t* __restrict__ need_cnt, char* const* __restrict__ peer, int mode, int32_t nown) {
    __shared__ int s_last;
    __shared__ unsigned long long s_tag;
    if (dev && block_done(&dev->done)) return;
    AmgMail* mine = reinterpret_cast<AmgMail*>(peer[me]);
    if (threadIdx.x == 0) s_tag = *reinterpret_cast<volatile unsigned long long*>(&mine->cnt[slot]) + 1;
    __syncthreads();
    const unsigned long long tag = s_tag;
    const int64_t gtid = (int64_t)blockIdx.x * blockDim.x + threadIdx.x, gstride = (int64_t)gridDim.x * blockDim.x;
    if (mode == 0) {
        for (int o = 0; o < R; ++o) {
            if (o == me) continue;
            const int b = send_off[o], e = send_off[o + 1];
            double* dst = reinterpret_cast<double*>(peer[o] + voff) + dest_off[o];
            for (int64_t j = b + gtid; j < e; j += gstride) dst[j - b] = src[send_idx[j]];
        }
    } else {
        for (int o = 0; o < R; ++o) {
            double* dst = reinterpret_cast<double*>(peer[o] + voff) + dest_off[o];
            for (int64_t j = gtid; j < nown; j += gstride) dst[j] = src[j];
        }
    }
    __syncthreads();
    if (threadIdx.x == 0) {
        __threadfence_system();
        const unsigned int t = atomicAdd(&mine->ticket[slot], 1u);
        s_last = (t == gridDim.x - 1);
        if (s_last) mine->ticket[slot] = 0;
    }
    __syncthreads();
    if (!s_last) return;
    __threadfence_system();
    if (threadIdx.x < R && threadIdx.x != me) {
        const bool sends = mode == 1 ? nown > 0 : send_off[threadIdx.x + 1] > send_off[threadIdx.x];
        if (sends) st_sys_u64(&reinterpret_cast<AmgMail*>(peer[threadIdx.x])->flag[slot][me], tag);
        if (need_cnt[threadIdx.x] > 0) {
            const long long t0 = clock64();
            while (ld_sys_u64(&mine->flag[slot][threadIdx.x]) < tag) {
                if (clock64() - t0 > P2P_SPIN_LIMIT) { mine->err = 1; break; }
            }
        }
    }
    __threadfence_system();
    __syncthreads();
    if (threadIdx.x == 0) mine->cnt[slot] = tag;
}

__global__ void __launch_bounds__(DA)
acg_vector_kernel(PcgDev* __restrict__ dev, int32_t n, double* __restrict__ cur, const double* __restrict__ prev,
                  double* __restrict__ x, double* __restrict__ r, double* __restrict__ p, double* __restrict__ s,
                  const double* __restrict__ u, const double* __restrict__ w, double* __restrict__ part_rr) {
    __shared__ double sm[40];
    if (block_done(&dev->done)) return;
    const double g = cur[0], dl = cur[1], rr = cur[2];
    const double gp = prev[0], ap = prev[3];
    const bool conv = rr <= dev->tol2;
    double beta = 0.0, den = dl;
    if (ap != 0.0) { beta = g / gp; den = dl - beta * g / ap; }
    const double alpha = g / den;
    const bool bad = !(den > 0.0) || !(rr == rr) || !(g == g);
    if (blockIdx.x == 0 && threadIdx.x == 0) {
        dev->rr = rr;
        if (conv) { dev->done = 1; dev->status = NODAL_OK; }
        else if (bad) { dev->done = 1; dev->status = NODAL_BREAKDOWN; }
        else { dev->iters = dev->iters + 1; cur[3] = alpha; }
    }
    if (conv || bad) return;
    double lrr = 0.0;
    const int64_t n2 = n >> 1;
    double2* x2 = reinterpret_cast<double2*>(x);
    double2* r2 = reinterpret_cast<double2*>(r);
    double2* p2 = reinterpret_cast<double2*>(p);
    double2* s2 = reinterpret_cast<double2*>(s);
    const double2* u2 = reinterpret_cast<const double2*>(u);
    const double2* w2 = reinterpret_cast<const double2*>(w);
    GRID_LOOP(i, n2) {
        double2 pv = p2[i], sv = s2[i], rv = r2[i], xv = x2[i];
        const double2 uv = u2[i], wv = w2[i];
        pv.x = fma(beta, pv.x, uv.x);   pv.y = fma(beta, pv.y, uv.y);
        sv.x = fma(beta, sv.x, wv.x);   sv.y = fma(beta, sv.y, wv.y);
        rv.x = fma(-alpha, sv.x, rv.x); rv.y = fma(-alpha, sv.y, rv.y);
        xv.x = fma(alpha, pv.x, xv.x);  xv.y = fma(alpha, pv.y, xv.y);
        p2[i] = pv; s2[i] = sv; r2[i] = rv; x2[i] = xv;
        lrr = fma(rv.x, rv.x, lrr);
        lrr = fma(rv.y, rv.y, lrr);
    }
    if ((n & 1) && blockIdx.x == 0 && threadIdx.x == 0) {
        const int64_t i = n - 1;
        const double pv = fma(beta, p[i], u[i]);
        const double sv = fma(beta, s[i], w[i]);
        const double rv = fma(-alpha, sv, r[i]);
        p[i] = pv; s[i] = sv; r[i] = rv;
        x[i] = fma(alpha, pv, x[i]);
        lrr = fma(rv, rv, lrr);
    }
    lrr = block_sum(lrr, sm);
    if (threadIdx.x == 0) part_rr[blockIdx.x] = lrr;
}

__global__ void __launch_bounds__(DA, 5)
acg_spmv_dots_kernel(int32_t n, int32_t nslices, const u32* __restrict__ slice_w, const int32_t* __restrict__ cols,
                     const double* __restrict__ vals, const double* __restrict__ u, const double* __restrict__ r,
                     double* __restrict__ w, double* __restrict__ part_g, double* __restrict__ part_d) {
    __shared__ double sm[40];
    const int lane = threadIdx.x & 31;
    const int64_t warp = ((int64_t)blockIdx.x * blockDim.x + threadIdx.x) >> 5;
    const int64_t nwarps = ((int64_t)gridDim.x * blockDim.x) >> 5;
    double lg = 0.0, ld = 0.0;
    for (int64_t s = warp; s < nslices; s += nwarps) {
        const u32 w0 = slice_w[s];
        const int wd = (int)(slice_w[s + 1] - w0);
        const double acc = sell_row_dot(cols, vals, (int64_t)w0 * 32 + lane, wd, u);
        const int64_t row = s * 32 + lane;
        if (row < n) {
            const double uv = __ldg(&u[row]);
            w[row] = acc;
            lg = fma(r[row], uv, lg);
            ld = fma(acc, uv, ld);
        }
    }
    lg = block_sum(lg, sm);
    ld = block_sum(ld, sm);
    if (threadIdx.x == 0) { part_g[blockIdx.x] = lg; part_d[blockIdx.x] = ld; }
}

__global__ void __launch_bounds__(DA)
acg_start_kernel(int32_t n, const double* __restrict__ b, const double* __restrict__ r,
                 double* __restrict__ p, double* __restrict__ s, double* __restrict__ part_rr, double* __restrict__ part_bb) {
    __shared__ double sm[40];
    double lrr = 0.0, lbb = 0.0;
    GRID_LOOP(i, n) {
        const double bv = b[i], rv = r[i];
        p[i] = 0.0; s[i] = 0.0;
        lrr = fma(rv, rv, lrr);
        lbb = fma(bv, bv, lbb);
    }
    lrr = block_sum(lrr, sm);
    lbb = block_sum(lbb, sm);
    if (threadIdx.x == 0) { part_rr[blockIdx.x] = lrr; part_bb[blockIdx.x] = lbb; }
}

__global__ void __launch_bounds__(DA)
acg_allreduce_kernel(PcgDev* __restrict__ dev, int check_done, const double* __restrict__ a, int na,
                     const double* __restrict__ b, int nb, const double* __restrict__ c, int nc,
                     const double* __restrict__ d4, int nd, int R, int me, char* const* __restrict__ peer,
                     int use_mail, double* __restrict__ out, int enforce_maxit) {
    __shared__ double sm[40];
    __shared__ int s_timeout;
    if (check_done && block_done(&dev->done)) return;
    const double va = a ? reduce_partials(a, na, sm) : 0.0;
    const double vb = b ? reduce_partials(b, nb, sm) : 0.0;
    const double vc = c ? reduce_partials(c, nc, sm) : 0.0;
    const double vd = d4 ? reduce_partials(d4, nd, sm) : 0.0;
    if (!use_mail) {
        if (threadIdx.x == 0) {
            out[0] = va; out[1] = vb; out[2] = vc; out[3] = vd;
            if (enforce_maxit && dev->iters >= dev->maxit) { dev->done = 1; dev->status = NODAL_NOT_CONVERGED; }
        }
        return;
    }
    AmgMail* mine = reinterpret_cast<AmgMail*>(peer[me]);
    const unsigned long long s0 = *reinterpret_cast<volatile unsigned long long*>(&mine->rseq);
    const unsigned long long tag = s0 + 1;
    const int par = (int)(s0 & 1ull);
    if (threadIdx.x == 0) s_timeout = 0;
    __syncthreads();
    if (threadIdx.x < R) {
        AmgMail* m = reinterpret_cast<AmgMail*>(peer[threadIdx.x]);
        volatile double* slot = m->red[par][me];
        slot[0] = va; slot[1] = vb; slot[2] = vc; slot[3] = vd;
        __threadfence_system();
        st_sys_u64(&m->rtag[par][me], tag);
        const long long t0 = clock64();
        while (ld_sys_u64(&mine->rtag[par][threadIdx.x]) != tag) {
            if (clock64() - t0 > P2P_SPIN_LIMIT) { s_timeout = 1; break; }
        }
    }
    __threadfence_system();
    __syncthreads();
    if (threadIdx.x == 0) {
        if (s_timeout) {
            dev->done = 1; dev->status = NODAL_CUDA_ERROR; mine->err = 1;
        } else {
            double t0 = 0.0, t1 = 0.0, t2 = 0.0, t3 = 0.0;
            for (int t = 0; t < R; ++t) {
                const volatile double* slot = mine->red[par][t];
                t0 += slot[0]; t1 += slot[1]; t2 += slot[2]; t3 += slot[3];
            }
            out[0] = t0; out[1] = t1; out[2] = t2; out[3] = t3;
            mine->rseq = tag;
            if (enforce_maxit && dev->iters >= dev->maxit) { dev->done = 1; dev->status = NODAL_NOT_CONVERGED; }
        }
    }
}

__global__ void acg_scalars_kernel(PcgDev* dev, double* SC, double rtol, int maxit, int first) {
    if (threadIdx.x != 0) return;
    const double rr = SC[2], bb = SC[3];
    if (first) {
        dev->bb = bb;
        dev->tol2 = rtol * rtol * bb;
        dev->iters = 0;
        dev->maxit = maxit;
    }
    SC[3] = 0.0;
    SC[4] = 1.0;
    SC[7] = 0.0;
    dev->rr = rr;
    dev->status = NODAL_OK;
    dev->done = 0;
    if (rr <= dev->tol2) dev->done = 1;
    else if (dev->iters >= dev->maxit) { dev->done = 1; dev->status = NODAL_NOT_CONVERGED; }
    else if (!(rr == rr)) { dev->done = 1; dev->status = NODAL_BREAKDOWN; }
}

struct Halo {
    int32_t nloc = 0, nhalo = 0;
    int64_t send_total = 0;
    int32_t* halo = nullptr;
    int32_t* send_idx = nullptr;
    double* send_buf = nullptr;
    std::vector<int32_t> need_from, need_off, send_cnt, send_off, cnt;
    int32_t* send_off_dev = nullptr;
    int32_t* need_cnt_dev = nullptr;
    long long* dest_off_dev = nullptr;
    int32_t ext_len = 0;
};

struct DLevel {
    std::vector<int32_t> bounds;
    int32_t nloc = 0, row0 = 0, nglob = 0;
    AmgCsr A;
    int32_t* lcols = nullptr;
    Halo halo;
    nodal_sell* sell = nullptr;
    int32_t* agg = nullptr;
    int32_t nc = 0;
    int32_t* pt_ptr = nullptr;
    int32_t* pt_idx = nullptr;
    double* b = nullptr;
    double* x = nullptr;
    double* r = nullptr;
    long long x_off = 0, r_off = 0;
    int64_t slot_len = 0;
};

struct Solver {
    nodal_ctx* ctx = nullptr;
    nodal_dist* d = nullptr;
    int R = 1, me = 0;
    cudaStream_t st = nullptr;
    bool p2p = false;
    char* base = nullptr;
    char** peer_dev = nullptr;
    std::vector<void*> owned;
    std::vector<DLevel> lv;
    nodal_amg* rep = nullptr;
    AmgCsr repA;
    std::vector<int32_t> rep_bounds;
    int32_t rep_n = 0;
    double *bfull = nullptr, *xfull = nullptr;
    long long bfull_off = 0;
    long long* gather_dest_dev = nullptr;
    int32_t* gather_need_dev = nullptr;
    double* gather_stage = nullptr;
    int32_t gmax = 0;
    double omega = 0.8, scale = 1.8, max_fill = 1.2, max_complexity = 4.0;
    double nnz_k_fine = 0.0, nnz_k_total = 0.0;
    bool sorted_galerkin = getenv("NODAL_AMG_SORT_GALERKIN") != nullptr;
    int passes = 2, rounds = 8, maxlevels = 30;
    int64_t gather_below = 400000;
    double params_rep[8] = {0};
    unsigned long long launches_exchange = 0;
    int64_t halo_total = 0;

    template <typename T>
    T* alloc(size_t count) {
        T* p = amg_pool<T>(ctx, count);
        if (p) owned.push_back(p);
        return p;
    }
};

int exchange_nccl(Solver& S, const Halo& H, double* v, cudaStream_t sx) {
    const int R = S.R, me = S.me;
    if (R == 1) return NODAL_OK;
    if (H.send_total) {
        da_gather_kernel<<<amg_rows_grid(S.ctx, H.send_total), DA, 0, sx>>>(H.send_total, H.send_idx, v, H.send_buf);
        KERNEL_CHECK();
    }
    NCCL_TRY(g_nccl.GroupStart());
    for (int o = 0; o < R; ++o) {
        if (o == me) continue;
        if (H.send_cnt[o]) NCCL_TRY(g_nccl.Send(H.send_buf + H.send_off[o], H.send_cnt[o], ncclFloat64, o, S.d->comm, sx));
        if (H.need_from[o]) NCCL_TRY(g_nccl.Recv(v + H.nloc + H.need_off[o], H.need_from[o], ncclFloat64, o, S.d->comm, sx));
    }
    NCCL_TRY(g_nccl.GroupEnd());
    return NODAL_OK;
}

int exchange(Solver& S, const PcgDev* dev, int slot, const Halo& H, long long voff, cudaStream_t sx) {
    if (S.R == 1) return NODAL_OK;
    double* v = reinterpret_cast<double*>(S.base + voff);
    if (!S.p2p) return exchange_nccl(S, H, v, sx);
    const int grid = (int)std::max<int64_t>(1, std::min<int64_t>(16, (H.send_total + 4095) / 4096));
    da_exchange_kernel<<<grid, 1024, 0, sx>>>(dev, slot, S.R, S.me, voff, v, H.send_idx, H.send_off_dev, H.dest_off_dev,
                                              H.need_cnt_dev, S.peer_dev, 0, 0);
    KERNEL_CHECK();
    return NODAL_OK;
}

int build_halo(Solver& S, DLevel& L) {
    nodal_ctx* ctx = S.ctx;
    cudaStream_t st = S.st;
    const int R = S.R, me = S.me;
    const int32_t rb = L.bounds[me], re = L.bounds[me + 1];
    const int64_t nnz = L.A.nnz;
    Halo& H = L.halo;
    H.nloc = L.nloc;
    const size_t need = align_up((size_t)std::max<int64_t>(nnz, 1) * 4, 256) * 2 +
                        align_up((size_t)std::max<int64_t>(nnz, 1) * 8, 256) * 4 +
                        radix_sort_scratch_bytes(std::max<int64_t>(nnz, 1)) +
                        2 * scan_scratch_bytes(std::max<int64_t>(nnz, 1)) + (1 << 16);
    NODAL_TRY(ctx_reserve(ctx, need));
    u32* flag = carve<u32>(ctx, (size_t)std::max<int64_t>(nnz, 1));
    u32* tot = carve<u32>(ctx, 16);
    if (!flag || !tot) return NODAL_CUDA_ERROR;
    u32* host_tot = reinterpret_cast<u32*>(ctx->pinned);
    const int gnz = amg_rows_grid(ctx, nnz);
    int64_t next = 0, nhalo = 0;
    if (nnz > 0 && R > 1) {
        da_flag_external_kernel<<<gnz, DA, 0, st>>>(nnz, L.A.indices, rb, re, flag);
        KERNEL_CHECK();
        const size_t mark = ctx->arena_used;
        NODAL_TRY(scan_exclusive_u32(ctx, flag, flag, nnz, tot, st));
        ctx->arena_used = mark;
        CUDA_TRY(cudaMemcpyAsync(host_tot, tot, sizeof(u32), cudaMemcpyDeviceToHost, st));
        CUDA_TRY(cudaStreamSynchronize(st));
        next = host_tot[0];
    }
    if (next > 0) {
        u64* keys = carve<u64>(ctx, (size_t)next);
        u64* vals = carve<u64>(ctx, (size_t)next);
        u64* keys_alt = carve<u64>(ctx, (size_t)next);
        u64* vals_alt = carve<u64>(ctx, (size_t)next);
        u32* uflag = carve<u32>(ctx, (size_t)next);
        if (!keys || !vals || !keys_alt || !vals_alt || !uflag) return NODAL_CUDA_ERROR;
        da_compact_external_kernel<<<gnz, DA, 0, st>>>(nnz, L.A.indices, rb, re, flag, keys);
        KERNEL_CHECK();
        const int bits = amg_bit_length(L.nglob);
        bool in_alt = false;
        const size_t mark = ctx->arena_used;
        NODAL_TRY(radix_sort_pairs(ctx, keys, vals, keys_alt, vals_alt, next, bits, &in_alt, st));
        ctx->arena_used = mark;
        const u64* sk = in_alt ? keys_alt : keys;
        da_unique_flag_kernel<<<amg_rows_grid(ctx, next), DA, 0, st>>>(next, sk, uflag);
        KERNEL_CHECK();
        NODAL_TRY(scan_exclusive_u32(ctx, uflag, uflag, next, tot, st));
        ctx->arena_used = mark;
        CUDA_TRY(cudaMemcpyAsync(host_tot, tot, sizeof(u32), cudaMemcpyDeviceToHost, st));
        CUDA_TRY(cudaStreamSynchronize(st));
        nhalo = host_tot[0];
        H.halo = S.alloc<int32_t>((size_t)nhalo);
        if (!H.halo) return NODAL_CUDA_ERROR;
        da_unique_compact_kernel<<<amg_rows_grid(ctx, next), DA, 0, st>>>(next, sk, uflag, H.halo);
        KERNEL_CHECK();
    }
    H.nhalo = (int32_t)nhalo;
    H.ext_len = L.nloc + H.nhalo;
    S.halo_total += nhalo;
    L.lcols = S.alloc<int32_t>((size_t)std::max<int64_t>(nnz, 1));
    if (!L.lcols) return NODAL_CUDA_ERROR;
    if (nnz > 0) {
        da_remap_kernel<<<gnz, DA, 0, st>>>(nnz, L.A.indices, rb, re, H.halo, H.nhalo, L.lcols);
        KERNEL_CHECK();
    }
    H.need_from.assign(R, 0); H.need_off.assign(R + 1, 0);
    H.send_cnt.assign(R, 0); H.send_off.assign(R + 1, 0);
    H.cnt.assign((size_t)R * R, 0);
    L.slot_len = (int64_t)align_up((size_t)H.ext_len + 2, 32);
    if (R == 1) return NODAL_OK;
    std::vector<int32_t> halo_h((size_t)nhalo);
    if (nhalo) CUDA_TRY(cudaMemcpyAsync(halo_h.data(), H.halo, sizeof(int32_t) * (size_t)nhalo, cudaMemcpyDeviceToHost, st));
    CUDA_TRY(cudaStreamSynchronize(st));
    {
        int o = 0;
        for (int64_t i = 0; i < nhalo; ++i) {
            while (halo_h[i] >= L.bounds[o + 1]) ++o;
            H.need_from[o]++;
        }
        for (int o2 = 0; o2 < R; ++o2) H.need_off[o2 + 1] = H.need_off[o2] + H.need_from[o2];
    }
    const int W = R + 1;
    int32_t* cnt_dev = S.alloc<int32_t>((size_t)W * (R + 1));
    if (!cnt_dev) return NODAL_CUDA_ERROR;
    std::vector<int32_t> mine_row(W, 0);
    for (int o = 0; o < R; ++o) mine_row[o] = H.need_from[o];
    mine_row[R] = (int32_t)(L.slot_len / 32);
    CUDA_TRY(cudaMemcpyAsync(cnt_dev + (size_t)W * R, mine_row.data(), sizeof(int32_t) * W, cudaMemcpyHostToDevice, st));
    NCCL_TRY(g_nccl.AllGather(cnt_dev + (size_t)W * R, cnt_dev, W, ncclInt32, S.d->comm, st));
    std::vector<int32_t> gathered((size_t)W * R);
    CUDA_TRY(cudaMemcpyAsync(gathered.data(), cnt_dev, sizeof(int32_t) * (size_t)W * R, cudaMemcpyDeviceToHost, st));
    CUDA_TRY(cudaStreamSynchronize(st));
    int64_t max_units = 0;
    for (int s2 = 0; s2 < R; ++s2) {
        for (int o = 0; o < R; ++o) H.cnt[(size_t)s2 * R + o] = gathered[(size_t)s2 * W + o];
        max_units = std::max<int64_t>(max_units, gathered[(size_t)s2 * W + R]);
    }
    L.slot_len = max_units * 32;
    for (int s = 0; s < R; ++s) H.send_cnt[s] = H.cnt[(size_t)s * R + me];
    for (int s = 0; s < R; ++s) H.send_off[s + 1] = H.send_off[s] + H.send_cnt[s];
    H.send_total = H.send_off[R];
    H.send_idx = S.alloc<int32_t>((size_t)std::max<int64_t>(H.send_total, 1));
    H.send_buf = S.alloc<double>((size_t)std::max<int64_t>(H.send_total, 1));
    if (!H.send_idx || !H.send_buf) return NODAL_CUDA_ERROR;
    NCCL_TRY(g_nccl.GroupStart());
    for (int o = 0; o < R; ++o) {
        if (o == me) continue;
        if (H.need_from[o]) NCCL_TRY(g_nccl.Send(H.halo + H.need_off[o], H.need_from[o], ncclInt32, o, S.d->comm, st));
        if (H.send_cnt[o]) NCCL_TRY(g_nccl.Recv(H.send_idx + H.send_off[o], H.send_cnt[o], ncclInt32, o, S.d->comm, st));
    }
    NCCL_TRY(g_nccl.GroupEnd());
    if (H.send_total) {
        da_rebase_kernel<<<amg_rows_grid(ctx, H.send_total), DA, 0, st>>>(H.send_total, H.send_idx, rb);
        KERNEL_CHECK();
    }
    std::vector<long long> dest_off(R, 0);
    for (int o = 0; o < R; ++o) {
        long long off = L.bounds[o + 1] - L.bounds[o];
        for (int o2 = 0; o2 < me; ++o2) off += H.cnt[(size_t)o * R + o2];
        dest_off[o] = off;
    }
    H.send_off_dev = S.alloc<int32_t>((size_t)R + 1);
    H.need_cnt_dev = S.alloc<int32_t>((size_t)R);
    H.dest_off_dev = S.alloc<long long>((size_t)R);
    if (!H.send_off_dev || !H.need_cnt_dev || !H.dest_off_dev) return NODAL_CUDA_ERROR;
    CUDA_TRY(cudaMemcpyAsync(H.send_off_dev, H.send_off.data(), sizeof(int32_t) * (size_t)(R + 1), cudaMemcpyHostToDevice, st));
    CUDA_TRY(cudaMemcpyAsync(H.need_cnt_dev, H.need_from.data(), sizeof(int32_t) * (size_t)R, cudaMemcpyHostToDevice, st));
    CUDA_TRY(cudaMemcpyAsync(H.dest_off_dev, dest_off.data(), sizeof(long long) * (size_t)R, cudaMemcpyHostToDevice, st));
    CUDA_TRY(cudaStreamSynchronize(st));
    return NODAL_OK;
}

int gather_counts(Solver& S, int32_t mine, std::vector<int32_t>& bounds) {
    const int R = S.R;
    bounds.assign(R + 1, 0);
    if (R == 1) { bounds[1] = mine; return NODAL_OK; }
    int32_t* dev = S.alloc<int32_t>((size_t)R + 1);
    if (!dev) return NODAL_CUDA_ERROR;
    CUDA_TRY(cudaMemcpyAsync(dev + R, &mine, sizeof(int32_t), cudaMemcpyHostToDevice, S.st));
    NCCL_TRY(g_nccl.AllGather(dev + R, dev, 1, ncclInt32, S.d->comm, S.st));
    std::vector<int32_t> h(R);
    CUDA_TRY(cudaMemcpyAsync(h.data(), dev, sizeof(int32_t) * (size_t)R, cudaMemcpyDeviceToHost, S.st));
    CUDA_TRY(cudaStreamSynchronize(S.st));
    for (int o = 0; o < R; ++o) bounds[o + 1] = bounds[o] + h[o];
    return NODAL_OK;
}

int build_rows(Solver& S, int32_t n_shape, int64_t nslots, int cb, u64* keys, double* vals, int32_t row_first,
               int32_t nrows, AmgCsr* out) {
    nodal_ctx* ctx = S.ctx;
    cudaStream_t st = S.st;
    AmgScratch<double> rhs(ctx, (size_t)n_shape + 1);
    if (!rhs.ptr) return NODAL_CUDA_ERROR;
    int64_t nnz = 0;
    NODAL_TRY(nodal_csr_build(ctx, n_shape, nslots, cb, reinterpret_cast<uint64_t*>(keys), vals, rhs, &nnz, st));
    AmgScratch<int32_t> ip_full(ctx, (size_t)n_shape + 1), ix(ctx, (size_t)std::max<int64_t>(nnz, 1));
    AmgScratch<double> dv(ctx, (size_t)std::max<int64_t>(nnz, 1));
    if (!ip_full.ptr || !ix.ptr || !dv.ptr) return NODAL_CUDA_ERROR;
    NODAL_TRY(nodal_csr_fetch(ctx, n_shape, nnz, ip_full, ix, dv, st));
    out->n = nrows;
    out->nnz = nnz;
    out->owned = true;
    if (row_first == 0 && nrows == n_shape) {
        out->indptr = ip_full.keep();
    } else {
        AmgScratch<int32_t> ip(ctx, (size_t)nrows + 1);
        if (!ip.ptr) return NODAL_CUDA_ERROR;
        da_slice_indptr_kernel<<<amg_rows_grid(ctx, nrows + 1), DA, 0, st>>>(nrows, ip_full.ptr + row_first, ip);
        KERNEL_CHECK();
        out->indptr = ip.keep();
    }
    out->indices = ix.keep();
    out->data = dv.keep();
    return NODAL_OK;
}

int coarsen(Solver& S, DLevel& L, AmgCsr* next, std::vector<int32_t>* next_bounds, bool* stalled) {
    nodal_ctx* ctx = S.ctx;
    cudaStream_t st = S.st;
    const int32_t nloc = L.nloc;
    const int64_t nnz = L.A.nnz;
    *stalled = false;
    AmgCsr loc;
    loc.n = nloc; loc.nnz = nnz; loc.indptr = L.A.indptr; loc.indices = L.lcols; loc.data = L.A.data;
    int32_t* comp = nullptr;
    int32_t ncur = nloc;
    AmgCsr cur = loc;
    int32_t cur_own = nloc, cur_base = L.row0;
    for (int pass = 0; pass < S.passes; ++pass) {
        int32_t* agg = nullptr;
        int32_t nc = 0;
        NODAL_TRY(amg_aggregate(ctx, S.rounds, cur, cur_own, cur_base, &agg, &nc, st));
        if (comp) {
            amg_compose_kernel<<<amg_rows_grid(ctx, nloc), AT, 0, st>>>(nloc, comp, agg);
            KERNEL_CHECK();
        }
        if (pass + 1 < S.passes && !S.sorted_galerkin && amg_merge_pays(cur.nnz, nc)) {
            int32_t *pp = nullptr, *pi = nullptr;
            NODAL_TRY(amg_members(ctx, cur.n, agg, nc, &pp, &pi, st));
            AmgCsr nxt;
            const int rc = amg_galerkin_merge(ctx, cur, pp, pi, nc, agg, cur_own, &nxt, st);
            ctx_pool_free(ctx, pp);
            ctx_pool_free(ctx, pi);
            NODAL_TRY(rc);
            if (cur.owned) amg_free_csr(ctx, cur);
            cur = nxt;
            std::vector<int32_t> ib;
            NODAL_TRY(gather_counts(S, nc, ib));
            cur_own = nc;
            cur_base = ib[S.me];
        } else if (pass + 1 < S.passes) {
            AmgScratch<u64> keys(ctx, (size_t)std::max<int64_t>(cur.nnz, 1));
            AmgScratch<double> vals(ctx, (size_t)std::max<int64_t>(cur.nnz, 1));
            if (!keys.ptr || !vals.ptr) return NODAL_CUDA_ERROR;
            const int cb = amg_bit_length(nc);
            da_relabel_local_kernel<<<amg_rows_grid(ctx, cur.n), DA, 0, st>>>(cur.n, cur.indptr, cur.indices, cur.data, agg,
                                                                             cur_own, nc, cb, keys, vals);
            KERNEL_CHECK();
            AmgCsr nxt;
            NODAL_TRY(build_rows(S, nc, cur.nnz, cb, keys, vals, 0, nc, &nxt));
            if (cur.owned) amg_free_csr(ctx, cur);
            cur = nxt;
            std::vector<int32_t> ib;
            NODAL_TRY(gather_counts(S, nc, ib));
            cur_own = nc;
            cur_base = ib[S.me];
        }
        if (!comp) comp = agg;
        else ctx_pool_free(ctx, agg);
        ncur = nc;
    }
    if (cur.owned) amg_free_csr(ctx, cur);
    NODAL_TRY(gather_counts(S, ncur, *next_bounds));
    const int32_t nc_glob = (*next_bounds)[S.R];
    if ((double)nc_glob > 0.9 * (double)L.nglob) {
        ctx_pool_free(ctx, comp);
        *stalled = true;
        return NODAL_OK;
    }
    AmgScratch<double> lab(ctx, (size_t)L.halo.ext_len + 2);
    if (!lab.ptr) return NODAL_CUDA_ERROR;
    da_labels_kernel<<<amg_rows_grid(ctx, nloc), DA, 0, st>>>(nloc, comp, (*next_bounds)[S.me], lab);
    KERNEL_CHECK();
    NODAL_TRY(exchange_nccl(S, L.halo, lab, st));
    bool have_members = false;
    if (!S.sorted_galerkin && amg_merge_pays(nnz, ncur)) {
        AmgScratch<int32_t> lab32(ctx, (size_t)L.halo.ext_len + 2);
        if (!lab32.ptr) return NODAL_CUDA_ERROR;
        da_labels_to_i32_kernel<<<amg_rows_grid(ctx, L.halo.ext_len), DA, 0, st>>>(L.halo.ext_len, lab, lab32);
        KERNEL_CHECK();
        NODAL_TRY(amg_members(ctx, nloc, comp, ncur, &L.pt_ptr, &L.pt_idx, st));
        S.owned.push_back(L.pt_ptr);
        S.owned.push_back(L.pt_idx);
        have_members = true;
        NODAL_TRY(amg_galerkin_merge(ctx, loc, L.pt_ptr, L.pt_idx, ncur, lab32, 0x7fffffff, next, st));
    } else {
        AmgScratch<u64> keys(ctx, (size_t)std::max<int64_t>(nnz, 1));
        AmgScratch<double> vals(ctx, (size_t)std::max<int64_t>(nnz, 1));
        if (!keys.ptr || !vals.ptr) return NODAL_CUDA_ERROR;
        const int cb = amg_bit_length(nc_glob);
        da_relabel_global_kernel<<<amg_rows_grid(ctx, nloc), DA, 0, st>>>(nloc, L.A.indptr, L.lcols, L.A.data, lab, cb, keys, vals);
        KERNEL_CHECK();
        NODAL_TRY(build_rows(S, nc_glob, nnz, cb, keys, vals, (*next_bounds)[S.me], ncur, next));
    }
    {
        std::vector<int32_t> fine_k, coarse_k;
        NODAL_TRY(gather_counts(S, (int32_t)(nnz >> 10) + 1, fine_k));
        NODAL_TRY(gather_counts(S, (int32_t)(next->nnz >> 10) + 1, coarse_k));
        S.nnz_k_total += (double)coarse_k[S.R];
        if (S.nnz_k_fine == 0.0) { S.nnz_k_fine = (double)fine_k[S.R]; S.nnz_k_total += S.nnz_k_fine; }
        if ((double)coarse_k[S.R] > S.max_fill * (double)fine_k[S.R] || S.nnz_k_total > S.max_complexity * S.nnz_k_fine) {
            amg_free_csr(ctx, *next);
            ctx_pool_free(ctx, comp);
            *stalled = true;
            return NODAL_OK;
        }
    }
    L.agg = comp;
    S.owned.push_back(comp);
    L.nc = ncur;
    if (!have_members) {
        NODAL_TRY(amg_transpose_pattern(ctx, nloc, comp, &L.pt_ptr, &L.pt_idx, st));
        S.owned.push_back(L.pt_ptr);
        S.owned.push_back(L.pt_idx);
    }
    return NODAL_OK;
}

int gather_operator(Solver& S, const AmgCsr& A, const std::vector<int32_t>& bounds, AmgCsr* out) {
    nodal_ctx* ctx = S.ctx;
    cudaStream_t st = S.st;
    const int R = S.R, me = S.me;
    if (R == 1) { *out = A; out->owned = false; return NODAL_OK; }
    if (A.nnz >= ((int64_t)1 << 31)) return NODAL_BAD_ARG;
    std::vector<int32_t> nzb;
    NODAL_TRY(gather_counts(S, (int32_t)A.nnz, nzb));
    const int32_t n = bounds[R];
    const int64_t nnz = nzb[R];
    AmgScratch<int32_t> ip(ctx, (size_t)n + 1), ix(ctx, (size_t)std::max<int64_t>(nnz, 1));
    AmgScratch<double> dv(ctx, (size_t)std::max<int64_t>(nnz, 1));
    if (!ip.ptr || !ix.ptr || !dv.ptr) return NODAL_CUDA_ERROR;
    const int32_t nloc = bounds[me + 1] - bounds[me];
    CUDA_TRY(cudaMemcpyAsync(ip.ptr + bounds[me], A.indptr, sizeof(int32_t) * (size_t)nloc, cudaMemcpyDeviceToDevice, st));
    if (A.nnz) {
        CUDA_TRY(cudaMemcpyAsync(ix.ptr + nzb[me], A.indices, sizeof(int32_t) * (size_t)A.nnz, cudaMemcpyDeviceToDevice, st));
        CUDA_TRY(cudaMemcpyAsync(dv.ptr + nzb[me], A.data, sizeof(double) * (size_t)A.nnz, cudaMemcpyDeviceToDevice, st));
    }
    NCCL_TRY(g_nccl.GroupStart());
    for (int o = 0; o < R; ++o) {
        const int32_t rows = bounds[o + 1] - bounds[o], cnt = nzb[o + 1] - nzb[o];
        if (rows) NCCL_TRY(g_nccl.Broadcast(ip.ptr + bounds[o], ip.ptr + bounds[o], rows, ncclInt32, o, S.d->comm, st));
        if (cnt) {
            NCCL_TRY(g_nccl.Broadcast(ix.ptr + nzb[o], ix.ptr + nzb[o], cnt, ncclInt32, o, S.d->comm, st));
            NCCL_TRY(g_nccl.Broadcast(dv.ptr + nzb[o], dv.ptr + nzb[o], cnt, ncclFloat64, o, S.d->comm, st));
        }
    }
    NCCL_TRY(g_nccl.GroupEnd());
    for (int o = 0; o < R; ++o) {
        const int32_t rows = bounds[o + 1] - bounds[o];
        if (rows && nzb[o]) {
            da_offset_indptr_kernel<<<amg_rows_grid(ctx, rows), DA, 0, st>>>(rows, ip.ptr + bounds[o], nzb[o]);
            KERNEL_CHECK();
        }
    }
    da_set_i32_kernel<<<1, 32, 0, st>>>(ip.ptr + n, (int32_t)nnz);
    KERNEL_CHECK();
    out->n = n; out->nnz = nnz; out->owned = true;
    out->indptr = ip.keep(); out->indices = ix.keep(); out->data = dv.keep();
    return NODAL_OK;
}

template <int MODE>
int sweep(Solver& S, const DLevel& L, const double* b, const double* x, double* y, cudaStream_t sx) {
    const nodal_sell* m = L.sell;
    amg_sell_kernel<MODE><<<amg_sell_grid(S.ctx, m->nslices), AT, 0, sx>>>(
        m->n, m->nslices, m->slice_w, m->cols, m->vals, m->dinv, b, x, S.omega, y, nullptr);
    KERNEL_CHECK();
    return NODAL_OK;
}

template <int MODE>
int cycle_sweep(Solver& S, const DLevel& L, const double* b, const double* xc, double* y, cudaStream_t sx) {
    const nodal_sell* m = L.sell;
    amg_cycle_sweep_kernel<MODE><<<amg_sell_grid(S.ctx, m->nslices), AT, 0, sx>>>(
        m->n, m->nslices, m->slice_w, m->cols, m->vals, m->dinv, b, S.omega, L.agg, xc, S.scale, y);
    KERNEL_CHECK();
    return NODAL_OK;
}

int cycle(Solver& S, const PcgDev* dev, const double* r0, double* u0, cudaStream_t sx) {
    nodal_ctx* ctx = S.ctx;
    const int ND = (int)S.lv.size() - 1;
    const bool fused = S.R == 1;
    for (int l = 0; l < ND; ++l) {
        DLevel& L = S.lv[l];
        const double* b = l == 0 ? r0 : L.b;
        if (fused) {
            NODAL_TRY(cycle_sweep<1>(S, L, b, nullptr, L.r, sx));
        } else {
            amg_jacobi0_kernel<<<amg_rows_grid(ctx, L.nloc), AT, 0, sx>>>(L.nloc, L.sell->dinv, b, S.omega, L.x);
            KERNEL_CHECK();
            NODAL_TRY(exchange(S, dev, 2 * l, L.halo, L.x_off, sx));
            NODAL_TRY(sweep<1>(S, L, b, L.x, L.r, sx));
        }
        amg_restrict_kernel<<<amg_rows_grid(ctx, L.nc), AT, 0, sx>>>(L.nc, L.pt_ptr, L.pt_idx, L.r, S.lv[l + 1].b);
        KERNEL_CHECK();
    }
    {
        DLevel& G = S.lv[ND];
        const double* b = ND == 0 ? r0 : G.b;
        if (S.R == 1) {
            NODAL_TRY(nodal_amg_apply(ctx, S.rep, b, S.xfull, sx));
        } else {
            if (S.p2p) {
                const int grid = (int)std::max<int64_t>(1, std::min<int64_t>(16, ((int64_t)G.nloc * S.R + 4095) / 4096));
                da_exchange_kernel<<<grid, 1024, 0, sx>>>(dev, AMG_SLOTS - 1, S.R, S.me, S.bfull_off, b, nullptr, nullptr,
                                                          S.gather_dest_dev, S.gather_need_dev, S.peer_dev, 1, G.nloc);
                KERNEL_CHECK();
            } else {
                CUDA_TRY(cudaMemcpyAsync(S.gather_stage + (size_t)S.R * S.gmax, b, sizeof(double) * (size_t)G.nloc,
                                         cudaMemcpyDeviceToDevice, sx));
                NCCL_TRY(g_nccl.AllGather(S.gather_stage + (size_t)S.R * S.gmax, S.gather_stage, S.gmax, ncclFloat64,
                                          S.d->comm, sx));
                for (int o = 0; o < S.R; ++o) {
                    const int32_t rows = S.rep_bounds[o + 1] - S.rep_bounds[o];
                    if (rows) CUDA_TRY(cudaMemcpyAsync(S.bfull + S.rep_bounds[o], S.gather_stage + (size_t)o * S.gmax,
                                                       sizeof(double) * (size_t)rows, cudaMemcpyDeviceToDevice, sx));
                }
            }
            NODAL_TRY(nodal_amg_apply(ctx, S.rep, S.bfull, S.xfull, sx));
        }
        if (ND == 0) {
            CUDA_TRY(cudaMemcpyAsync(u0, S.xfull + G.row0, sizeof(double) * (size_t)G.nloc, cudaMemcpyDeviceToDevice, sx));
            return NODAL_OK;
        }
    }
    for (int l = ND - 1; l >= 0; --l) {
        DLevel& L = S.lv[l];
        const double* b = l == 0 ? r0 : L.b;
        const double* xc = (l + 1 == ND) ? S.xfull + S.lv[ND].row0 : S.lv[l + 1].x;
        if (fused) {
            NODAL_TRY(cycle_sweep<2>(S, L, b, xc, l == 0 ? u0 : L.x, sx));
        } else {
            amg_prolong_kernel<<<amg_rows_grid(ctx, L.nloc), AT, 0, sx>>>(L.nloc, L.agg, xc, S.scale, L.x, L.r);
            KERNEL_CHECK();
            NODAL_TRY(exchange(S, dev, 2 * l + 1, L.halo, L.r_off, sx));
            NODAL_TRY(sweep<2>(S, L, b, L.r, l == 0 ? u0 : L.x, sx));
        }
    }
    return NODAL_OK;
}

}

extern "C" int nodal_dist_amg_pcg(nodal_ctx* ctx, nodal_dist* d, int32_t n_global, const int32_t* bounds_h,
                                  int64_t nnz, const int32_t* indptr, const int32_t* indices,
                                  const double* data, const double* rhs_local, double* x_local,
                                  const double* params, double rtol, int32_t maxit, int32_t* iters_h,
                                  double* relres_h, double* stats_h, void* stream) {
    NvtxRange nvtx_range("nodal_dist_amg_pcg");
    if (!ctx || !d || !bounds_h || !iters_h || !relres_h) return NODAL_BAD_ARG;
    *iters_h = 0;
    *relres_h = 0.0;
    if (stats_h) memset(stats_h, 0, 32 * sizeof(double));
    CUDA_TRY(cudaSetDevice(ctx->device));
    Solver S;
    S.ctx = ctx; S.d = d; S.R = d->nranks; S.me = d->rank; S.st = (cudaStream_t)stream;
    const int R = S.R, me = S.me;
    cudaStream_t st = S.st;
    const int32_t nloc0 = bounds_h[me + 1] - bounds_h[me];
    if (nloc0 <= 0 || bounds_h[0] != 0 || bounds_h[R] != n_global) {
        nodal_set_error("nodal_dist_amg_pcg: every rank must own at least one row and bounds must span [0, n)");
        return NODAL_BAD_ARG;
    }
    double coarse = 0.0, direct_max = 0.0;
    if (params) {
        if (params[0] >= 1.0) S.passes = (int)params[0];
        coarse = params[1];
        if (params[2] > 0.0) S.omega = params[2];
        if (params[3] > 0.0) S.scale = params[3];
        if (params[4] >= 1.0) S.maxlevels = (int)params[4];
        if (params[5] >= 1.0) S.rounds = (int)params[5];
        direct_max = params[6];
        if (params[7] >= 1.0) S.gather_below = (int64_t)params[7];
        if (params[8] > 0.0) S.max_fill = params[8];
    }
    S.params_rep[0] = S.passes; S.params_rep[1] = coarse; S.params_rep[2] = S.omega; S.params_rep[3] = S.scale;
    S.params_rep[4] = S.maxlevels; S.params_rep[5] = S.rounds; S.params_rep[6] = direct_max;
    S.params_rep[7] = S.max_fill;

    cudaEvent_t ev0, ev1, ev2, ev_poll[2];
    CUDA_TRY(cudaEventCreate(&ev0));
    CUDA_TRY(cudaEventCreate(&ev1));
    CUDA_TRY(cudaEventCreate(&ev2));
    CUDA_TRY(cudaEventCreateWithFlags(&ev_poll[0], cudaEventDisableTiming));
    CUDA_TRY(cudaEventCreateWithFlags(&ev_poll[1], cudaEventDisableTiming));
    cudaGraph_t graph[2] = {nullptr, nullptr};
    cudaGraphExec_t gexec[2] = {nullptr, nullptr};
    cudaStream_t cap = nullptr;
    PcgDev host{};
    int restarts = 0;
    float ms_setup = 0.f, ms_solve = 0.f;
    double relres = 0.0;
    unsigned long long launches_per_iter = 0;
    char* local_buf = nullptr;

    auto run = [&]() -> int {
        CUDA_TRY(cudaEventRecord(ev0, st));
        std::unique_ptr<NvtxRange> phase(new NvtxRange("amg setup (hierarchy, halo plans, buffers)"));
        {
            DLevel L;
            L.bounds.assign(bounds_h, bounds_h + R + 1);
            L.nloc = nloc0; L.row0 = bounds_h[me]; L.nglob = n_global;
            L.A.n = nloc0; L.A.nnz = nnz; L.A.indptr = indptr; L.A.indices = indices; L.A.data = data; L.A.owned = false;
            S.lv.push_back(L);
        }
        for (;;) {
            DLevel& L = S.lv.back();
            const bool fine = S.lv.size() == 1;
            const bool distribute = (int64_t)L.nglob > S.gather_below && (int)S.lv.size() < S.maxlevels;
            if (fine || distribute) {
                NODAL_TRY(build_halo(S, L));
                NODAL_TRY(sell_from_csr(ctx, L.nloc, L.A.nnz, L.A.indptr, L.lcols, L.A.data, &L.sell, st, nullptr));
            }
            if (!distribute) break;
            AmgCsr next;
            std::vector<int32_t> nb;
            bool stalled = false;
            NODAL_TRY(coarsen(S, L, &next, &nb, &stalled));
            if (stalled) break;
            DLevel C;
            C.bounds = nb;
            C.nloc = nb[me + 1] - nb[me]; C.row0 = nb[me]; C.nglob = nb[R];
            C.A = next;
            S.lv.push_back(C);
        }
        const int ND = (int)S.lv.size() - 1;
        if (ND == 0 && (int64_t)S.lv[0].nglob > S.gather_below) {
            nodal_set_error("nodal_dist_amg_pcg: the aggregation hierarchy stalled on the finest level "
                            "(expander-like graph); use the Jacobi-preconditioned solver");
            return NODAL_BREAKDOWN;
        }
        if (2 * ND + 2 > AMG_SLOTS - 1) { nodal_set_error("nodal_dist_amg_pcg: too many distributed levels"); return NODAL_BAD_ARG; }
        {
            DLevel& G = S.lv[ND];
            S.rep_bounds = G.bounds;
            S.rep_n = G.nglob;
            NODAL_TRY(gather_operator(S, G.A, G.bounds, &S.repA));
            NODAL_TRY(nodal_amg_create(ctx, S.repA.n, S.repA.nnz, S.repA.indptr, S.repA.indices, S.repA.data,
                                       S.params_rep, &S.rep, st));
            for (int o = 0; o < R; ++o) S.gmax = std::max(S.gmax, G.bounds[o + 1] - G.bounds[o]);
        }
        size_t bytes = AMG_HDR;
        auto place = [&](int64_t doubles) { const long long off = (long long)bytes; bytes += align_up((size_t)doubles * 8, 256); return off; };
        const long long u_off = place(S.lv[0].slot_len);
        const long long xs_off = place(S.lv[0].slot_len);
        for (int l = 0; l < ND; ++l) { S.lv[l].x_off = place(S.lv[l].slot_len); S.lv[l].r_off = place(S.lv[l].slot_len); }
        S.bfull_off = place((int64_t)S.rep_n + 2);
        bool usable = false;
        NODAL_TRY(peer_heap_ensure(ctx, d, &d->amg, bytes, AMG_HDR, st, &usable));
        S.p2p = usable;
        if (S.p2p) {
            S.base = d->amg.shm;
            S.peer_dev = d->amg.peer_dev;
        } else {
            local_buf = static_cast<char*>(ctx_pool_alloc(ctx, bytes));
            if (!local_buf) return NODAL_CUDA_ERROR;
            CUDA_TRY(cudaMemsetAsync(local_buf, 0, AMG_HDR, st));
            S.base = local_buf;
        }
        double* u = reinterpret_cast<double*>(S.base + u_off);
        for (int l = 0; l < ND; ++l) {
            DLevel& L = S.lv[l];
            L.x = reinterpret_cast<double*>(S.base + L.x_off);
            L.r = reinterpret_cast<double*>(S.base + L.r_off);
        }
        for (int l = 1; l <= ND; ++l) {
            S.lv[l].b = S.alloc<double>((size_t)S.lv[l].nloc + 2);
            if (!S.lv[l].b) return NODAL_CUDA_ERROR;
        }
        S.bfull = reinterpret_cast<double*>(S.base + S.bfull_off);
        S.xfull = S.alloc<double>((size_t)S.rep_n + 2);
        if (!S.xfull) return NODAL_CUDA_ERROR;
        if (R > 1) {
            std::vector<long long> gd(R, (long long)S.rep_bounds[me]);
            std::vector<int32_t> gn(R);
            for (int o = 0; o < R; ++o) gn[o] = S.rep_bounds[o + 1] - S.rep_bounds[o];
            S.gather_dest_dev = S.alloc<long long>((size_t)R);
            S.gather_need_dev = S.alloc<int32_t>((size_t)R);
            S.gather_stage = S.alloc<double>((size_t)(R + 1) * S.gmax + 2);
            if (!S.gather_dest_dev || !S.gather_need_dev || !S.gather_stage) return NODAL_CUDA_ERROR;
            CUDA_TRY(cudaMemcpyAsync(S.gather_dest_dev, gd.data(), sizeof(long long) * (size_t)R, cudaMemcpyHostToDevice, st));
            CUDA_TRY(cudaMemcpyAsync(S.gather_need_dev, gn.data(), sizeof(int32_t) * (size_t)R, cudaMemcpyHostToDevice, st));
            CUDA_TRY(cudaStreamSynchronize(st));
        }
        DLevel& F = S.lv[0];
        const int32_t n = F.nloc;
        const int gv = amg_rows_grid(ctx, n);
        const int gs = amg_sell_grid(ctx, F.sell->nslices);
        const int gmaxp = std::max(gv, gs) + 1;
        double* r = S.alloc<double>((size_t)n + 2);
        double* p = S.alloc<double>((size_t)n + 2);
        double* s = S.alloc<double>((size_t)n + 2);
        double* w = S.alloc<double>((size_t)n + 2);
        double* part = S.alloc<double>(4 * (size_t)gmaxp + 64);
        PcgDev* dev = S.alloc<PcgDev>(1);
        if (!r || !p || !s || !w || !part || !dev) return NODAL_CUDA_ERROR;
        double* part_g = part;
        double* part_d = part + gmaxp;
        double* part_rr = part + 2 * (size_t)gmaxp;
        double* part_bb = part + 3 * (size_t)gmaxp;
        double* SC = part + 4 * (size_t)gmaxp;
        CUDA_TRY(cudaMemsetAsync(dev, 0, sizeof(PcgDev), st));
        CUDA_TRY(cudaMemsetAsync(SC, 0, sizeof(double) * 32, st));
        const int use_mail = (S.p2p && R > 1) ? 1 : 0;

        auto allreduce = [&](int check_done, const double* a, int na, const double* b, int nb, const double* c, int nc,
                             const double* dd, int nd, double* out, int enforce, cudaStream_t sx) -> int {
            acg_allreduce_kernel<<<1, DA, 0, sx>>>(dev, check_done, a, na, b, nb, c, nc, dd, nd, R, me, S.peer_dev, use_mail,
                                                   out, enforce);
            KERNEL_CHECK();
            if (R > 1 && !use_mail) NCCL_TRY(g_nccl.AllReduce(out, out, 4, ncclFloat64, ncclSum, d->comm, sx));
            return NODAL_OK;
        };
        double* xstage = reinterpret_cast<double*>(S.base + xs_off);
        auto start = [&](int first) -> int {
            CUDA_TRY(cudaMemcpyAsync(xstage, x_local, sizeof(double) * (size_t)n, cudaMemcpyDeviceToDevice, st));
            NODAL_TRY(exchange(S, nullptr, AMG_SLOTS - 2, F.halo, xs_off, st));
            NODAL_TRY(sweep<1>(S, F, rhs_local, xstage, r, st));
            acg_start_kernel<<<gv, DA, 0, st>>>(n, rhs_local, r, p, s, part_rr, part_bb);
            KERNEL_CHECK();
            NODAL_TRY(cycle(S, nullptr, r, u, st));
            NODAL_TRY(exchange(S, nullptr, 2 * ND, F.halo, u_off, st));
            acg_spmv_dots_kernel<<<gs, DA, 0, st>>>(n, F.sell->nslices, F.sell->slice_w, F.sell->cols, F.sell->vals, u, r, w,
                                                    part_g, part_d);
            KERNEL_CHECK();
            NODAL_TRY(allreduce(0, part_g, gs, part_d, gs, part_rr, gv, part_bb, gv, SC, 0, st));
            acg_scalars_kernel<<<1, 32, 0, st>>>(dev, SC, rtol, maxit, first);
            KERNEL_CHECK();
            return NODAL_OK;
        };
        auto iteration = [&](int par, cudaStream_t sx) -> int {
            double* cur = SC + par * 4;
            double* nxt = SC + (par ^ 1) * 4;
            acg_vector_kernel<<<gv, DA, 0, sx>>>(dev, n, cur, nxt, x_local, r, p, s, u, w, part_rr);
            KERNEL_CHECK();
            NODAL_TRY(cycle(S, dev, r, u, sx));
            NODAL_TRY(exchange(S, dev, 2 * ND, F.halo, u_off, sx));
            acg_spmv_dots_kernel<<<gs, DA, 0, sx>>>(n, F.sell->nslices, F.sell->slice_w, F.sell->cols, F.sell->vals, u, r, w,
                                                    part_g, part_d);
            KERNEL_CHECK();
            NODAL_TRY(allreduce(1, part_g, gs, part_d, gs, part_rr, gv, nullptr, 0, nxt, 1, sx));
            return NODAL_OK;
        };
        nvtxRangePushA("amg first residual + cycle");
        const int start_rc = start(1);
        nvtxRangePop();
        NODAL_TRY(start_rc);
        const bool use_graph = getenv("NODAL_DIST_NO_GRAPH") == nullptr;
        if (use_graph) {
            const unsigned long long before = g_nodal_launches;
            CUDA_TRY(cudaStreamCreateWithFlags(&cap, cudaStreamNonBlocking));
            for (int par = 0; par < 2; ++par) {
                CUDA_TRY(cudaStreamBeginCapture(cap, cudaStreamCaptureModeThreadLocal));
                const int crc = iteration(par, cap);
                cudaError_t ce = cudaStreamEndCapture(cap, &graph[par]);
                if (crc != NODAL_OK) return crc;
                CUDA_TRY(ce);
                CUDA_TRY(cudaGraphInstantiate(&gexec[par], graph[par], 0));
            }
            launches_per_iter = (g_nodal_launches - before) / 2;
            g_nodal_launches = before;
        }
        CUDA_TRY(cudaEventRecord(ev1, st));
        phase.reset();
        phase.reset(new NvtxRange("amg-pcg iterations"));
        PcgDev* poll = reinterpret_cast<PcgDev*>(ctx->pinned);
        double last_true_rr = -1.0;
        int par = 0;
        for (;;) {
            int64_t k = 0;
            const int64_t max_iters = (int64_t)maxit + 4;
            for (;; ++k) {
                if (use_graph) {
                    CUDA_TRY(cudaGraphLaunch(gexec[par], st));
                    g_nodal_launches += launches_per_iter;
                } else {
                    NODAL_TRY(iteration(par, st));
                }
                par ^= 1;
                CUDA_TRY(cudaMemcpyAsync(&poll[k & 1], dev, sizeof(PcgDev), cudaMemcpyDeviceToHost, st));
                CUDA_TRY(cudaEventRecord(ev_poll[k & 1], st));
                if (R > 1 && !use_mail) {
                    CUDA_TRY(cudaEventSynchronize(ev_poll[k & 1]));
                    if (poll[k & 1].done) break;
                    if (k > max_iters) break;
                    continue;
                }
                if (k >= 1) {
                    CUDA_TRY(cudaEventSynchronize(ev_poll[(k - 1) & 1]));
                    if (poll[(k - 1) & 1].done) break;
                }
                if (k > max_iters) break;
            }
            CUDA_TRY(cudaStreamSynchronize(st));
            host = poll[k & 1];
            if (!host.done) host.status = NODAL_NOT_CONVERGED;
            if (host.status == NODAL_BREAKDOWN || host.status == NODAL_CUDA_ERROR) break;
            const int recurrence_status = host.status;
            const int iters_so_far = host.iters;
            NODAL_TRY(start(0));
            par = 0;
            CUDA_TRY(cudaMemcpyAsync(&poll[0], dev, sizeof(PcgDev), cudaMemcpyDeviceToHost, st));
            CUDA_TRY(cudaStreamSynchronize(st));
            host = poll[0];
            host.iters = iters_so_far;
            if (host.rr <= host.tol2) { host.status = NODAL_OK; break; }
            if (!(host.rr == host.rr)) { host.status = NODAL_BREAKDOWN; break; }
            if (recurrence_status == NODAL_NOT_CONVERGED || host.iters >= host.maxit) { host.status = NODAL_NOT_CONVERGED; break; }
            if (restarts >= 8 || (last_true_rr >= 0.0 && host.rr > 0.25 * last_true_rr)) { host.status = NODAL_NOT_CONVERGED; break; }
            last_true_rr = host.rr;
            ++restarts;
        }
        CUDA_TRY(cudaEventRecord(ev2, st));
        CUDA_TRY(cudaEventSynchronize(ev2));
        CUDA_TRY(cudaEventElapsedTime(&ms_setup, ev0, ev1));
        CUDA_TRY(cudaEventElapsedTime(&ms_solve, ev1, ev2));
        relres = host.bb > 0.0 ? sqrt(host.rr / host.bb) : 0.0;
        if (S.p2p) {
            unsigned long long err = 0;
            CUDA_TRY(cudaMemcpy(&err, &reinterpret_cast<AmgMail*>(S.base)->err, sizeof(err), cudaMemcpyDeviceToHost));
            if (err) {
                nodal_set_error("nodal_dist_amg_pcg: a peer-memory exchange timed out (rank %d)", me);
                CUDA_TRY(cudaMemset(&reinterpret_cast<AmgMail*>(S.base)->err, 0, sizeof(err)));
                return NODAL_CUDA_ERROR;
            }
        }
        return host.status;
    };
    const int rc = run();
    cudaStreamSynchronize(st);
    *iters_h = host.iters;
    *relres_h = relres;
    if (stats_h) {
        int32_t nl = 0;
        int64_t rows[64], nnzs[64];
        double rep_ms = 0.0;
        int32_t direct = 0;
        if (S.rep) nodal_amg_info(S.rep, 64, &nl, rows, nnzs, &rep_ms, &direct);
        stats_h[0] = (double)((int)S.lv.size() - 1 + nl);
        stats_h[2] = restarts;
        stats_h[3] = ms_solve;
        stats_h[4] = ms_setup;
        stats_h[5] = nl > 0 ? (double)rows[nl - 1] : 0.0;
        stats_h[7] = direct;
        stats_h[8] = (double)((int)S.lv.size() - 1);
        stats_h[9] = S.p2p ? 2.0 : 0.0;
        stats_h[10] = (double)launches_per_iter;
        stats_h[11] = (double)S.rep_n;
        stats_h[12] = (double)S.halo_total;
        for (size_t l = 0; l < S.lv.size() && l < 12; ++l) stats_h[16 + l] = (double)S.lv[l].nglob;
    }
    for (int par = 0; par < 2; ++par) {
        if (gexec[par]) cudaGraphExecDestroy(gexec[par]);
        if (graph[par]) cudaGraphDestroy(graph[par]);
    }
    if (cap) cudaStreamDestroy(cap);
    if (S.rep) nodal_amg_destroy(S.rep);
    if (S.repA.owned) amg_free_csr(ctx, S.repA);
    for (size_t l = 0; l < S.lv.size(); ++l) {
        if (S.lv[l].sell) sell_free(S.lv[l].sell);
        if (l > 0 && S.lv[l].A.owned) amg_free_csr(ctx, S.lv[l].A);
    }
    for (void* ptr : S.owned) ctx_pool_free(ctx, ptr);
    if (local_buf) ctx_pool_free(ctx, local_buf);
    cudaEventDestroy(ev0); cudaEventDestroy(ev1); cudaEventDestroy(ev2);
    cudaEventDestroy(ev_poll[0]); cudaEventDestroy(ev_poll[1]);
    return rc;
}
```

### nodal_b200/csrc/sparse.cuh

```cuda
#pragma once
#include "common.cuh"

struct nodal_sell {
    nodal_ctx* ctx = nullptr;
    int device = 0;
    int32_t n = 0;
    int32_t nslices = 0;
    int64_t padded = 0;
    int64_t nnz = 0;
    u32* slice_w = nullptr;
    int32_t* cols = nullptr;
    double* vals = nullptr;
    size_t store_bytes = 0;
    double* dinv = nullptr;
};

int sell_from_csr(nodal_ctx* ctx, int32_t n, int64_t nnz, const int32_t* indptr,
                  const int32_t* indices, const double* data, nodal_sell** out, cudaStream_t st,
                  const double* sc = nullptr);
void sell_free(nodal_sell* m);
int sell_set_l2_window(nodal_ctx* ctx, const nodal_sell* m, cudaStream_t st);
void sell_clear_l2_window(cudaStream_t st);

int csr_spmv_launch(nodal_ctx* ctx, int32_t n, int64_t nnz, const int32_t* indptr,
                    const int32_t* indices, const double* data, const double* x, double* y,
                    cudaStream_t st);
int csr_spmv_rows_launch(nodal_ctx* ctx, int32_t rows, const int32_t* indptr, const int32_t* indices,
                         const double* data, const double* x, double* y, int32_t shape_n, int64_t shape_nnz,
                         cudaStream_t st);

#ifdef __CUDACC__
#include "amg_cycle_core.cuh"

struct SellLoad {
    const double* __restrict__ x;
    __device__ __forceinline__ double operator()(int32_t c) const { return __ldg(&x[c]); }
};

template <int W, class G>
__device__ __forceinline__ double sell_dot_fixed(const int32_t* __restrict__ cols,
                                                 const double* __restrict__ vals, int64_t base,
                                                 const G& gather, double acc) {
    int32_t c[W];
    double v[W], xv[W];
#pragma unroll
    for (int i = 0; i < W; ++i) {
        c[i] = cols[base + (int64_t)i * 32];
        v[i] = vals[base + (int64_t)i * 32];
    }
#pragma unroll
    for (int i = 0; i < W; ++i) xv[i] = gather(c[i]);
#pragma unroll
    for (int i = 0; i < W; ++i) acc = amg_dot_step(v[i], xv[i], acc);
    return acc;
}

template <class G>
__device__ __forceinline__ double sell_row_gather(const int32_t* __restrict__ cols,
                                                  const double* __restrict__ vals, int64_t base, int w,
                                                  const G& x) {
    double acc = 0.0;
    int k = 0;
    for (; k + 8 <= w; k += 8) acc = sell_dot_fixed<8>(cols, vals, base + (int64_t)k * 32, x, acc);
    const int64_t b = base + (int64_t)k * 32;
    switch (w - k) {
        case 7: acc = sell_dot_fixed<7>(cols, vals, b, x, acc); break;
        case 6: acc = sell_dot_fixed<6>(cols, vals, b, x, acc); break;
        case 5: acc = sell_dot_fixed<5>(cols, vals, b, x, acc); break;
        case 4: acc = sell_dot_fixed<4>(cols, vals, b, x, acc); break;
        case 3: acc = sell_dot_fixed<3>(cols, vals, b, x, acc); break;
        case 2: acc = sell_dot_fixed<2>(cols, vals, b, x, acc); break;
        case 1: acc = sell_dot_fixed<1>(cols, vals, b, x, acc); break;
        default: break;
    }
    return acc;
}

__device__ __forceinline__ double sell_row_dot(const int32_t* __restrict__ cols,
                                               const double* __restrict__ vals, int64_t base, int w,
                                               const double* __restrict__ x) {
    return sell_row_gather(cols, vals, base, w, SellLoad{x});
}
#endif
```

### nodal_b200/csrc/spmv.cu

```cuda
#include <algorithm>

#include "sparse.cuh"

constexpr int SPMV_THREADS = 256;

template <int TPR>
__global__ void __launch_bounds__(SPMV_THREADS)
csr_spmv_kernel(int32_t n, const int32_t* __restrict__ indptr, const int32_t* __restrict__ indices,
                const double* __restrict__ data, const double* __restrict__ x,
                double* __restrict__ y) {
    constexpr int RPW = 32 / TPR;
    const int lane = threadIdx.x & 31, sub = lane & (TPR - 1);
    const int64_t warp = ((int64_t)blockIdx.x * blockDim.x + threadIdx.x) >> 5;
    const int64_t nwarps = ((int64_t)gridDim.x * blockDim.x) >> 5;
    for (int64_t r0 = warp * RPW; r0 < n; r0 += nwarps * RPW) {
        const int64_t row = r0 + lane / TPR;
        double acc = 0.0;
        if (row < n) {
            const int32_t e = indptr[row + 1];
            for (int32_t j = indptr[row] + sub; j < e; j += TPR)
                acc = fma(data[j], __ldg(&x[indices[j]]), acc);
        }
#pragma unroll
        for (int o = TPR >> 1; o > 0; o >>= 1) acc += __shfl_xor_sync(0xffffffffu, acc, o);
        if (sub == 0 && row < n) y[row] = acc;
    }
}

static int pick_tpr(int32_t n, int64_t nnz) {
    const double mean = n > 0 ? (double)nnz / n : 1.0;
    if (mean <= 2.5) return 2;
    if (mean <= 6.0) return 4;
    if (mean <= 12.0) return 8;
    if (mean <= 24.0) return 16;
    return 32;
}

int csr_spmv_launch(nodal_ctx* ctx, int32_t n, int64_t nnz, const int32_t* indptr,
                    const int32_t* indices, const double* data, const double* x, double* y,
                    cudaStream_t st) {
    return csr_spmv_rows_launch(ctx, n, indptr, indices, data, x, y, n, nnz, st);
}

int csr_spmv_rows_launch(nodal_ctx* ctx, int32_t n, const int32_t* indptr, const int32_t* indices,
                         const double* data, const double* x, double* y, int32_t shape_n, int64_t shape_nnz,
                         cudaStream_t st) {
    if (n == 0) return NODAL_OK;
    const int tpr = pick_tpr(shape_n, shape_nnz);
    int64_t blocks = ((int64_t)n * tpr + SPMV_THREADS - 1) / SPMV_THREADS;
    const int64_t cap = (int64_t)ctx->num_sms * 8;
    const int grid = (int)(blocks < cap ? blocks : cap);
#define GO(T) csr_spmv_kernel<T><<<grid, SPMV_THREADS, 0, st>>>(n, indptr, indices, data, x, y)
    switch (tpr) {
        case 2: GO(2); break;
        case 4: GO(4); break;
        case 8: GO(8); break;
        case 16: GO(16); break;
        default: GO(32); break;
    }
#undef GO
    KERNEL_CHECK();
    return NODAL_OK;
}

extern "C" int nodal_spmv(nodal_ctx* ctx, int32_t n, int64_t nnz, const int32_t* indptr,
                          const int32_t* indices, const double* data, const double* x, double* y,
                          void* stream) {
    if (!ctx || n < 0) return NODAL_BAD_ARG;
    CUDA_TRY(cudaSetDevice(ctx->device));
    return csr_spmv_launch(ctx, n, nnz, indptr, indices, data, x, y, (cudaStream_t)stream);
}

__global__ void __launch_bounds__(SPMV_THREADS)
sell_widths_kernel(int32_t n, int32_t nslices, const int32_t* __restrict__ indptr,
                   u32* __restrict__ slice_w) {
    const int lane = threadIdx.x & 31;
    const int64_t warp = ((int64_t)blockIdx.x * blockDim.x + threadIdx.x) >> 5;
    const int64_t nwarps = ((int64_t)gridDim.x * blockDim.x) >> 5;
    for (int64_t s = warp; s < nslices; s += nwarps) {
        const int64_t r = s * 32 + lane;
        u32 len = 0;
        if (r < n) len = (u32)(indptr[r + 1] - indptr[r]);
#pragma unroll
        for (int o = 16; o > 0; o >>= 1) len = max(len, __shfl_xor_sync(0xffffffffu, len, o));
        if (lane == 0) slice_w[s] = len;
    }
}

__global__ void __launch_bounds__(SPMV_THREADS)
sell_fill_kernel(int32_t n, int32_t nslices, const int32_t* __restrict__ indptr,
                 const int32_t* __restrict__ indices, const double* __restrict__ data,
                 const u32* __restrict__ slice_w, const double* __restrict__ sc,
                 int32_t* __restrict__ cols, double* __restrict__ vals, double* __restrict__ dinv) {
    const int lane = threadIdx.x & 31;
    const int64_t warp = ((int64_t)blockIdx.x * blockDim.x + threadIdx.x) >> 5;
    const int64_t nwarps = ((int64_t)gridDim.x * blockDim.x) >> 5;
    for (int64_t s = warp; s < nslices; s += nwarps) {
        const int64_t r = s * 32 + lane;
        const u32 w0 = slice_w[s], w = slice_w[s + 1] - w0;
        int32_t b = 0, e = 0;
        if (r < n) { b = indptr[r]; e = indptr[r + 1]; }
        double diag = 0.0;
        const int64_t base = (int64_t)w0 * 32 + lane;
        for (u32 k = 0; k < w; ++k) {
            int32_t c = r < n ? (int32_t)r : 0;
            double v = 0.0;
            if (b + (int32_t)k < e) {
                c = indices[b + k];
                v = data[b + k];
                if (sc) v = (v * sc[r]) * sc[c];
                if (c == r) diag += v;
            }
            cols[base + (int64_t)k * 32] = c;
            vals[base + (int64_t)k * 32] = v;
        }
        if (r < n) dinv[r] = diag != 0.0 ? 1.0 / diag : 1.0;
    }
}

void sell_free(nodal_sell* m) {
    if (!m) return;
    cudaSetDevice(m->device);
    ctx_pool_free(m->ctx, m->slice_w);
    ctx_pool_free(m->ctx, m->vals);
    ctx_pool_free(m->ctx, m->dinv);
    delete m;
}

int sell_from_csr(nodal_ctx* ctx, int32_t n, int64_t nnz, const int32_t* indptr,
                  const int32_t* indices, const double* data, nodal_sell** out, cudaStream_t st,
                  const double* sc) {
    *out = nullptr;
    nodal_sell* m = new nodal_sell();
    m->ctx = ctx;
    m->device = ctx->device;
    m->n = n;
    m->nnz = nnz;
    m->nslices = (n + 31) / 32;
    const int64_t ns = m->nslices;
    int rc = NODAL_OK;
    auto fail = [&](int code) { sell_free(m); return code; };
#define CT(expr)                                                                             \
    do {                                                                                     \
        cudaError_t _e = (expr);                                                             \
        if (_e != cudaSuccess) {                                                             \
            nodal_set_error("%s:%d: %s -> %s", __FILE__, __LINE__, #expr,                    \
                            cudaGetErrorString(_e));                                         \
            return fail(NODAL_CUDA_ERROR);                                                   \
        }                                                                                    \
    } while (0)
#define PA(field, type, bytes)                                                               \
    do {                                                                                     \
        m->field = static_cast<type*>(ctx_pool_alloc(ctx, (bytes)));                         \
        if (!m->field) {                                                                     \
            nodal_set_error("%s:%d: out of device memory (%zu bytes)", __FILE__, __LINE__,   \
                            (size_t)(bytes));                                                \
            return fail(NODAL_CUDA_ERROR);                                                   \
        }                                                                                    \
    } while (0)
    PA(slice_w, u32, sizeof(u32) * (size_t)(ns + 1));
    PA(dinv, double, sizeof(double) * (size_t)(n > 0 ? n : 1));
    CT(cudaMemsetAsync(m->slice_w, 0, sizeof(u32) * (size_t)(ns + 1), st));
    if (n == 0) { *out = m; return NODAL_OK; }
    const int64_t cap = (int64_t)ctx->num_sms * 8;
    const int64_t want = (ns * 32 + SPMV_THREADS - 1) / SPMV_THREADS;
    const int grid = (int)(want < cap ? want : cap);
    sell_widths_kernel<<<grid, SPMV_THREADS, 0, st>>>(n, m->nslices, indptr, m->slice_w);
    CT(cudaGetLastError());
    rc = ctx_reserve(ctx, scan_scratch_bytes(ns + 1) + 4096);
    if (rc != NODAL_OK) return fail(rc);
    u32* tot = carve<u32>(ctx, 16);
    rc = scan_exclusive_u32(ctx, m->slice_w, m->slice_w, ns + 1, tot, st);
    if (rc != NODAL_OK) return fail(rc);
    u32* host_tot = reinterpret_cast<u32*>(ctx->pinned);
    CT(cudaMemcpyAsync(host_tot, tot, sizeof(u32), cudaMemcpyDeviceToHost, st));
    CT(cudaStreamSynchronize(st));
    m->padded = (int64_t)host_tot[0] * 32;
    const size_t alloc = (size_t)(m->padded > 0 ? m->padded : 32);
    PA(vals, double, sizeof(double) * alloc + sizeof(int32_t) * alloc);
    m->cols = reinterpret_cast<int32_t*>(m->vals + alloc);
    m->store_bytes = (sizeof(double) + sizeof(int32_t)) * alloc;
#undef PA
    sell_fill_kernel<<<grid, SPMV_THREADS, 0, st>>>(n, m->nslices, indptr, indices, data,
                                                    m->slice_w, sc, m->cols, m->vals, m->dinv);
    CT(cudaGetLastError());
#undef CT
    *out = m;
    return NODAL_OK;
}

__global__ void __launch_bounds__(SPMV_THREADS, 5)
sell_spmv_kernel(int32_t n, int32_t nslices, const u32* __restrict__ slice_w,
                 const int32_t* __restrict__ cols, const double* __restrict__ vals,
                 const double* __restrict__ x, double* __restrict__ y) {
    const int lane = threadIdx.x & 31;
    const int64_t warp = ((int64_t)blockIdx.x * blockDim.x + threadIdx.x) >> 5;
    const int64_t nwarps = ((int64_t)gridDim.x * blockDim.x) >> 5;
    for (int64_t s = warp; s < nslices; s += nwarps) {
        const u32 w0 = slice_w[s];
        const int w = (int)(slice_w[s + 1] - w0);
        const int64_t base = (int64_t)w0 * 32 + lane;
        const double acc = sell_row_dot(cols, vals, base, w, x);
        const int64_t r = s * 32 + lane;
        if (r < n) y[r] = acc;
    }
}

extern "C" int nodal_sell_create(nodal_ctx* ctx, int32_t n, int64_t nnz, const int32_t* indptr,
                                 const int32_t* indices, const double* data, nodal_sell** out,
                                 void* stream) {
    if (!ctx || n < 0 || !out) return NODAL_BAD_ARG;
    CUDA_TRY(cudaSetDevice(ctx->device));
    return sell_from_csr(ctx, n, nnz, indptr, indices, data, out, (cudaStream_t)stream, nullptr);
}

extern "C" int nodal_sell_destroy(nodal_sell* m) {
    sell_free(m);
    return NODAL_OK;
}

extern "C" int64_t nodal_sell_padded_nnz(const nodal_sell* m) { return m ? m->padded : 0; }

extern "C" int nodal_sell_spmv(nodal_ctx* ctx, const nodal_sell* m, const double* x, double* y,
                               void* stream) {
    if (!ctx || !m) return NODAL_BAD_ARG;
    if (m->n == 0) return NODAL_OK;
    CUDA_TRY(cudaSetDevice(ctx->device));
    const int64_t want = ((int64_t)m->nslices * 32 + SPMV_THREADS - 1) / SPMV_THREADS;
    const int64_t cap = (int64_t)ctx->num_sms * 5;
    sell_spmv_kernel<<<(int)(want < cap ? want : cap), SPMV_THREADS, 0, (cudaStream_t)stream>>>(
        m->n, m->nslices, m->slice_w, m->cols, m->vals, x, y);
    KERNEL_CHECK();
    return NODAL_OK;
}

int sell_set_l2_window(nodal_ctx* ctx, const nodal_sell* m, cudaStream_t st) {
    if (!m || !m->vals || !getenv("NODAL_L2_WINDOW")) return NODAL_OK;
    cudaDeviceProp prop;
    CUDA_TRY(cudaGetDeviceProperties(&prop, ctx->device));
    if (prop.persistingL2CacheMaxSize <= 0 || prop.accessPolicyMaxWindowSize <= 0) return NODAL_OK;
    const size_t persist = (size_t)prop.persistingL2CacheMaxSize;
    CUDA_TRY(cudaDeviceSetLimit(cudaLimitPersistingL2CacheSize, persist));
    cudaStreamAttrValue attr;
    memset(&attr, 0, sizeof(attr));
    const size_t window = std::min<size_t>(m->store_bytes, (size_t)prop.accessPolicyMaxWindowSize);
    attr.accessPolicyWindow.base_ptr = m->vals;
    attr.accessPolicyWindow.num_bytes = window;
    attr.accessPolicyWindow.hitRatio = (float)std::min(1.0, 0.85 * (double)persist / (double)window);
    attr.accessPolicyWindow.hitProp = cudaAccessPropertyPersisting;
    attr.accessPolicyWindow.missProp = cudaAccessPropertyStreaming;
    CUDA_TRY(cudaStreamSetAttribute(st, cudaStreamAttributeAccessPolicyWindow, &attr));
    return NODAL_OK;
}

void sell_clear_l2_window(cudaStream_t st) {
    if (!getenv("NODAL_L2_WINDOW")) return;
    cudaStreamAttrValue attr;
    memset(&attr, 0, sizeof(attr));
    attr.accessPolicyWindow.num_bytes = 0;
    cudaStreamSetAttribute(st, cudaStreamAttributeAccessPolicyWindow, &attr);
    cudaCtxResetPersistingL2Cache();
}
```

### nodal_b200/device.py

```python
from __future__ import annotations

import ctypes as C
import threading

import numpy as np

from . import _lib
from . import constants as K
from .table import ComponentTable

_STRIDE_OF_TYPE = {K.T_R: 4, K.T_A: 2, K.T_E: 5, K.T_VCVS: 6, K.T_VCCS: 6, K.T_CCVS: 6, K.T_CCCS: 5}


def _torch():
    import torch
    return torch


def coo_stride(table: ComponentTable) -> int:
    need = max((_STRIDE_OF_TYPE[t] for t in table.present_types()), default=2)
    return 2 if need <= 2 else 4 if need <= 4 else need


def colbits_for(n: int) -> int:
    return max(1, int(n).bit_length())


class DeviceCSR:

    def __init__(self, n, indptr, indices, data):
        self.n = int(n)
        self.indptr, self.indices, self.data = indptr, indices, data

    @property
    def nnz(self):
        return int(self.data.numel())

    @property
    def shape(self):
        return (self.n, self.n)

    def tocsr(self):
        import scipy.sparse as sps
        return sps.csr_matrix((self.data.cpu().numpy(), self.indices.cpu().numpy(),
                               self.indptr.cpu().numpy()), shape=self.shape)

    def toarray(self):
        return self.tocsr().toarray()

    def __array__(self, dtype=None, copy=None):
        a = self.toarray()
        return a if dtype is None else a.astype(dtype)


class DeviceAMG:

    PARAMS = ("passes", "coarse", "omega", "scale", "maxlevels", "rounds", "direct_max", "max_fill")

    def __init__(self, dev, csr, **params):
        unknown = set(params) - set(self.PARAMS)
        if unknown:
            raise TypeError(f"unknown AMG parameter(s): {sorted(unknown)}")
        self.dev, self.csr = dev, csr
        arr = (C.c_double * 8)(*[float(params.get(k, 0.0)) for k in self.PARAMS])
        h = C.c_void_p()
        p = dev.ptr
        st = dev.lib.nodal_amg_create(dev.ctx, csr.n, csr.nnz, p(csr.indptr), p(csr.indices), p(csr.data),
                                      arr, C.byref(h), dev.stream())
        _lib.check(st, "nodal_amg_create")
        self.handle = h
        cap = 64
        nl, rows, nnz = C.c_int32(0), (C.c_int64 * cap)(), (C.c_int64 * cap)()
        ms, direct = C.c_double(0.0), C.c_int32(0)
        _lib.check(dev.lib.nodal_amg_info(h, cap, C.byref(nl), rows, nnz, C.byref(ms), C.byref(direct)),
                   "nodal_amg_info")
        self.rows = [int(rows[k]) for k in range(nl.value)]
        self.nnz = [int(nnz[k]) for k in range(nl.value)]
        self.setup_ms, self.direct = ms.value, bool(direct.value)

    def close(self):
        if self.handle:
            self.dev.lib.nodal_amg_destroy(self.handle)
            self.handle = None

    def __del__(self):
        try:
            self.close()
        except Exception:
            pass

    def aggregates(self, level):
        dev = self.dev
        agg = dev.empty(max(1, self.rows[level]), dev.torch.int32)[: self.rows[level]]
        _lib.check(dev.lib.nodal_amg_fetch_level(dev.ctx, self.handle, level, dev.ptr(agg), None, None, None,
                                                 dev.stream()), "nodal_amg_fetch_level")
        return agg

    def operator(self, level):
        dev, torch = self.dev, self.dev.torch
        n, nnz = self.rows[level], self.nnz[level]
        indptr = dev.empty(n + 1, torch.int32)
        indices = dev.empty(max(1, nnz), torch.int32)[:nnz]
        data = dev.empty(max(1, nnz), torch.float64)[:nnz]
        p = dev.ptr
        _lib.check(dev.lib.nodal_amg_fetch_level(dev.ctx, self.handle, level, None, p(indptr), p(indices),
                                                 p(data), dev.stream()), "nodal_amg_fetch_level")
        return DeviceCSR(n, indptr, indices, data)

    def apply(self, r):
        dev = self.dev
        z = dev.empty(max(1, self.csr.n), dev.torch.float64)[: self.csr.n]
        _lib.check(dev.lib.nodal_amg_apply(dev.ctx, self.handle, dev.ptr(r), dev.ptr(z), dev.stream()),
                   "nodal_amg_apply")
        return z

    def solve_multi(self, rhs, rtol=1e-10, maxit=None):
        dev, n = self.dev, self.csr.n
        K = int(rhs.shape[0])
        if not 1 <= K <= 8 or int(rhs.shape[1]) != n:
            raise ValueError("rhs must be a (K, n) tensor with 1 <= K <= 8")
        rhs = rhs.contiguous()
        x = dev.zeros(max(2, K * n), dev.torch.float64)[: K * n].view(K, n)
        iters, relres, status = (C.c_int32 * K)(), (C.c_double * K)(), (C.c_int32 * K)()
        st = dev.lib.nodal_amg_pcg_multi(dev.ctx, self.handle, K, dev.ptr(rhs), dev.ptr(x), rtol, int(maxit or 1000),
                                         iters, relres, status, dev.stream())
        _lib.check(st, "nodal_amg_pcg_multi", allowed=(_lib.OK, _lib.NOT_CONVERGED, _lib.BREAKDOWN))
        infos = [dict(solver="amg_pcg_multi", status=int(status[k]), iterations=int(iters[k]), relres=float(relres[k]),
                      batch=K, level_rows=list(self.rows)) for k in range(K)]
        return x, infos

    def profile_sweeps(self, reps=64):
        ms = (C.c_double * 4)()
        _lib.check(self.dev.lib.nodal_amg_profile_sweeps(self.dev.ctx, self.handle, int(reps), ms, self.dev.stream()),
                   "nodal_amg_profile_sweeps")
        return dict(spmv_dot=ms[0], residual=ms[1], jacobi=ms[2])

    def profile_cycle(self, reps=64):
        ms = (C.c_double * 6)()
        _lib.check(self.dev.lib.nodal_amg_profile_cycle(self.dev.ctx, self.handle, int(reps), ms, self.dev.stream()),
                   "nodal_amg_profile_cycle")
        return dict(zip(("jacobi0", "residual", "prolong", "jacobi", "fused_residual", "fused_post"), list(ms)))

    def solve(self, rhs, rtol=1e-10, maxit=None, x0=None):
        dev, n = self.dev, self.csr.n
        x = dev.zeros(max(2, n), dev.torch.float64)[:n] if x0 is None else x0.clone()
        if maxit is None:
            maxit = 1000
        iters, relres = C.c_int32(0), C.c_double(0.0)
        stats = (C.c_double * 16)()
        st = dev.lib.nodal_amg_pcg(dev.ctx, self.handle, dev.ptr(rhs), dev.ptr(x), rtol, maxit,
                                   C.byref(iters), C.byref(relres), stats, dev.stream())
        _lib.check(st, "nodal_amg_pcg", allowed=(_lib.OK, _lib.NOT_CONVERGED, _lib.BREAKDOWN))
        info = dict(solver="amg_pcg", status=st, iterations=iters.value, relres=relres.value,
                    restarts=int(stats[2]), solve_ms=stats[3], setup_ms=stats[4], levels=int(stats[0]),
                    operator_complexity=stats[1], grid_complexity=stats[6], coarsest_rows=int(stats[5]),
                    coarsest_direct=bool(stats[7]), level_rows=list(self.rows))
        return x, info


class Device:

    _instances = {}
    _lock = threading.Lock()

    @classmethod
    def get(cls, index=None):
        torch = _torch()
        if not torch.cuda.is_available():
            raise _lib.NodalLibraryError(
                "nodal_b200 needs a CUDA device (sm_100a); there is no CPU fallback")
        if index is None:
            index = torch.cuda.current_device()
        key = (threading.get_ident(), int(index))
        with cls._lock:
            if key not in cls._instances:
                cls._instances[key] = cls(int(index))
            return cls._instances[key]

    def __init__(self, index):
        self.torch = _torch()
        self.index = index
        self.dev = self.torch.device("cuda", index)
        self.lib = _lib.load()
        h = C.c_void_p()
        _lib.check(self.lib.nodal_ctx_create(index, C.byref(h)), "nodal_ctx_create")
        self.ctx = h
        self.launches = 0

    def stream(self):
        return C.c_void_p(self.torch.cuda.current_stream(self.dev).cuda_stream)

    def empty(self, n, dtype):
        return self.torch.empty(int(n), dtype=dtype, device=self.dev)

    def zeros(self, n, dtype):
        return self.torch.zeros(int(n), dtype=dtype, device=self.dev)

    def to_device(self, arr, pin=False):
        t = self.torch.from_numpy(np.ascontiguousarray(arr))
        if pin:
            t = t.pin_memory()
        return t.to(self.dev, non_blocking=pin)

    @staticmethod
    def ptr(t):
        return C.c_void_p(t.data_ptr()) if t is not None else C.c_void_p(0)

    def upload_table(self, table: ComponentTable, pin=False):
        names = ("type", "value", "a", "b", "c", "d", "drv", "branch")
        if table.is_spd_structured():
            names = names[:4]
        if getattr(table, "_pinned", None):
            out = {name: table._pinned[name].to(self.dev, non_blocking=True) for name in names}
        else:
            out = {name: self.to_device(getattr(table, name), pin=pin) for name in names}
        for name in ("c", "d", "drv", "branch"):
            out.setdefault(name, None)
        return out

    @staticmethod
    def uploaded_bytes(table: ComponentTable):
        per_row = 17 if table.is_spd_structured() else 33
        return per_row * len(table)

    def stamp_coo(self, dtab, ncomp, kcl, n, stride):
        torch = self.torch
        cb = colbits_for(n)
        keys = self.empty(max(1, stride * ncomp), torch.int64)
        vals = self.empty(max(1, stride * ncomp), torch.float64)
        p = self.ptr
        _lib.check(self.lib.nodal_stamp_coo(
            self.ctx, ncomp, p(dtab["type"]), p(dtab["value"]), p(dtab["a"]), p(dtab["b"]),
            p(dtab["c"]), p(dtab["d"]), p(dtab["drv"]), p(dtab["branch"]),
            kcl, n, stride, cb, p(keys), p(vals), self.stream()), "nodal_stamp_coo")
        return keys, vals, cb

    def assemble_csr(self, table: ComponentTable, dtab=None, order="sorted"):
        if dtab is None:
            dtab = self.upload_table(table)
        return self.assemble_csr_raw(dtab, len(table), table.kcl, table.n, coo_stride(table), order=order)

    def assemble_csr_raw(self, dtab, ncomp, kcl, n, stride, order="sorted"):
        torch = self.torch
        if order not in ("sorted", "first_touch"):
            raise ValueError("order must be 'sorted' or 'first_touch'")
        keys, vals, cb = self.stamp_coo(dtab, ncomp, kcl, n, stride)
        rhs = self.empty(max(1, n), torch.float64)[:n]
        nnz = C.c_int64(0)
        p = self.ptr
        _lib.check(self.lib.nodal_csr_build_ordered(self.ctx, n, stride * ncomp, cb, p(keys), p(vals),
                                                    1 if order == "first_touch" else 0, p(rhs), C.byref(nnz),
                                                    self.stream()), "nodal_csr_build")
        nnz = nnz.value
        indptr = self.empty(n + 1, torch.int32)
        indices = self.empty(max(1, nnz), torch.int32)[:nnz]
        data = self.empty(max(1, nnz), torch.float64)[:nnz]
        _lib.check(self.lib.nodal_csr_fetch(self.ctx, n, nnz, p(indptr), p(indices), p(data),
                                            self.stream()), "nodal_csr_fetch")
        self.torch.cuda.current_stream(self.dev).synchronize()
        del keys, vals
        return DeviceCSR(n, indptr, indices, data), rhs

    _COLUMNS = ("type", "value", "a", "b", "c", "d", "drv", "branch")

    def _select(self, dtab, ncomp, scan, scan_args, gather, gather_args):
        pos = self.empty(max(1, ncomp), self.torch.int32)
        count = C.c_int64(0)
        p = self.ptr
        _lib.check(getattr(self.lib, scan)(self.ctx, ncomp, *scan_args, p(pos), C.byref(count), self.stream()), scan)
        m = count.value
        out = {k: (self.empty(max(1, m), dtab[k].dtype) if dtab[k] is not None else None) for k in self._COLUMNS}
        _lib.check(getattr(self.lib, gather)(self.ctx, ncomp, p(pos), *gather_args, *[p(dtab[k]) for k in self._COLUMNS],
                                             *[p(out[k]) for k in self._COLUMNS], self.stream()), gather)
        return out, m

    def select_local(self, dtab, ncomp, rb, re):
        p = self.ptr
        return self._select(dtab, ncomp, "nodal_table_select_scan", (p(dtab["a"]), p(dtab["b"]), int(rb), int(re)),
                            "nodal_table_select_gather", (int(rb), int(re)))

    def select_mna_rows(self, dtab, ncomp, kcl, rb, re):
        p = self.ptr
        return self._select(dtab, ncomp, "nodal_table_select_mna_scan",
                            (p(dtab["type"]), p(dtab["a"]), p(dtab["b"]), p(dtab["branch"]), int(kcl), int(rb), int(re)),
                            "nodal_table_select_mna_gather", (int(kcl), int(rb), int(re)))

    def select_type(self, dtab, ncomp, t):
        p = self.ptr
        return self._select(dtab, ncomp, "nodal_table_select_type_scan", (p(dtab["type"]), p(dtab["a"]), p(dtab["b"]),
                                                                          int(t)),
                            "nodal_table_select_type_gather", (int(t),))

    def csr_to_dense(self, csr: DeviceCSR):
        n = csr.n
        G = self.empty(max(1, n * n), self.torch.float64)[: n * n].view(n, n)
        p = self.ptr
        _lib.check(self.lib.nodal_csr_to_dense(self.ctx, n, p(csr.indptr), p(csr.indices),
                                               p(csr.data), p(G), self.stream()), "nodal_csr_to_dense")
        return G

    def assemble_dense(self, table: ComponentTable, atomic=False):
        if not atomic:
            csr, rhs = self.assemble_csr(table)
            return self.csr_to_dense(csr), rhs
        torch = self.torch
        n, ncomp = table.n, len(table)
        stride = coo_stride(table)
        dtab = self.upload_table(table)
        keys, vals, cb = self.stamp_coo(dtab, ncomp, table.kcl, n, stride)
        G = self.empty(max(1, n * n), torch.float64)[: n * n].view(n, n)
        rhs = self.empty(max(1, n), torch.float64)[:n]
        p = self.ptr
        _lib.check(self.lib.nodal_coo_to_dense_atomic(self.ctx, n, stride * ncomp, cb, p(keys),
                                                      p(vals), p(G), p(rhs), self.stream()),
                   "nodal_coo_to_dense_atomic")
        return G, rhs

    def spmv(self, csr: DeviceCSR, x):
        y = self.empty(max(1, csr.n), self.torch.float64)[: csr.n]
        p = self.ptr
        _lib.check(self.lib.nodal_spmv(self.ctx, csr.n, csr.nnz, p(csr.indptr), p(csr.indices),
                                       p(csr.data), p(x), p(y), self.stream()), "nodal_spmv")
        return y

    def pcg(self, csr: DeviceCSR, rhs, rtol=1e-10, maxit=None, flags=0, x0=None):
        n = csr.n
        x = self.zeros(max(2, n), self.torch.float64)[:n] if x0 is None else x0.clone()
        if maxit is None:
            maxit = max(5000, 40 * int(np.sqrt(max(n, 1))))
        iters, relres = C.c_int32(0), C.c_double(0.0)
        stats = (C.c_double * 16)()
        p = self.ptr
        st = self.lib.nodal_pcg(self.ctx, n, csr.nnz, p(csr.indptr), p(csr.indices), p(csr.data),
                                p(rhs), p(x), rtol, maxit, flags, C.byref(iters), C.byref(relres),
                                stats, self.stream())
        _lib.check(st, "nodal_pcg", allowed=(_lib.OK, _lib.NOT_CONVERGED, _lib.BREAKDOWN))
        info = dict(solver="pcg", status=st, iterations=iters.value, relres=relres.value,
                    restarts=int(stats[2]), solve_ms=stats[3], setup_ms=stats[4],
                    format="sell32" if stats[5] else "csr", stored_nnz=int(stats[6]),
                    spmv_grid=int(stats[7]), scaled=bool(stats[12]))
        if stats[11]:
            info["kernel_ms"] = dict(spmv_dot=stats[8], update=stats[9], direction=stats[10],
                                     samples=int(stats[11]))
        return x, info

    def connected_components(self, table: ComponentTable, want_labels=False):
        a, b = self.to_device(table.a), self.to_device(table.b)
        labels = self.empty(table.kcl + 1, self.torch.int32) if want_labels else None
        count, reached = C.c_int32(0), C.c_int32(0)
        st = self.lib.nodal_connected_components(self.ctx, len(table), self.ptr(a), self.ptr(b), table.kcl,
                                                 self.ptr(labels) if want_labels else None,
                                                 C.byref(count), C.byref(reached), self.stream())
        _lib.check(st, "nodal_connected_components")
        return count.value, reached.value, labels

    def source_forest(self, dtab, ncomp, kcl, be):
        torch = self.torch
        i32 = lambda k: self.empty(max(1, k), torch.int32)
        nodes = kcl + 1
        out = dict(erow=i32(be), adj_ptr=i32(nodes + 1), adj_row=i32(2 * be), rep_row=i32(nodes),
                   offset=self.empty(nodes, torch.float64), parent_edge=i32(nodes), depth=i32(nodes),
                   roots=i32(kcl))
        info = (C.c_int64 * 8)()
        p = self.ptr
        _lib.check(self.lib.nodal_source_forest(
            self.ctx, ncomp, p(dtab["type"]), p(dtab["value"]), p(dtab["a"]), p(dtab["b"]), p(dtab["branch"]),
            kcl, be, *[p(out[k]) for k in ("erow", "adj_ptr", "adj_row", "rep_row", "offset", "parent_edge",
                                           "depth", "roots")], info, self.stream()), "nodal_source_forest")
        keys = ("sources", "loops", "branch_conflicts", "trees", "floating_trees", "grounded_nodes", "rows", "depth")
        return {k: int(info[i]) for i, k in enumerate(keys)}, out

    def source_reduce(self, dtab, ncomp, kcl, forest):
        torch = self.torch
        pos = self.empty(max(1, ncomp), torch.int32)
        count = C.c_int64(0)
        p = self.ptr
        args = (p(dtab["type"]), p(dtab["a"]), p(dtab["b"]), kcl, p(forest["rep_row"]), p(forest["offset"]))
        _lib.check(self.lib.nodal_source_reduce_scan(self.ctx, ncomp, *args, p(pos), C.byref(count), self.stream()),
                   "nodal_source_reduce_scan")
        m = count.value
        red = dict(type=self.empty(max(1, m), torch.uint8), value=self.empty(max(1, m), torch.float64),
                   a=self.empty(max(1, m), torch.int32), b=self.empty(max(1, m), torch.int32),
                   c=None, d=None, drv=None, branch=None)
        _lib.check(self.lib.nodal_source_reduce_table(
            self.ctx, ncomp, p(dtab["type"]), p(dtab["value"]), p(dtab["a"]), p(dtab["b"]), kcl,
            p(forest["rep_row"]), p(forest["offset"]), p(pos), p(red["type"]), p(red["value"]), p(red["a"]),
            p(red["b"]), self.stream()), "nodal_source_reduce_table")
        return red, m

    def source_expand(self, dtab, kcl, forest, info, y, csr: DeviceCSR, rhs):
        n = csr.n
        x = self.empty(max(1, n), self.torch.float64)[:n]
        relres = C.c_double(0.0)
        p = self.ptr
        f = forest
        _lib.check(self.lib.nodal_source_expand(
            self.ctx, kcl, n, info["sources"], p(f["erow"]), p(dtab["a"]), p(dtab["b"]), p(dtab["branch"]),
            p(f["adj_ptr"]), p(f["adj_row"]), p(f["rep_row"]), p(f["offset"]), p(f["depth"]), info["depth"],
            p(y), p(rhs), csr.nnz, p(csr.indptr), p(csr.indices), p(csr.data), p(x), C.byref(relres),
            self.stream()), "nodal_source_expand")
        return x, relres.value

    def source_potentials(self, kcl, n, forest, y):
        x = self.empty(max(1, n), self.torch.float64)[:n]
        p = self.ptr
        _lib.check(self.lib.nodal_source_potentials(self.ctx, kcl, n, p(forest["rep_row"]), p(forest["offset"]), p(y),
                                                    p(x), self.stream()), "nodal_source_potentials")
        return x

    def source_tree_rows(self, kcl, n, nnz_full, rb, re, forest, rows, rhs, x):
        torch = self.torch
        cap = max(1, re - rb)
        row, o_rhs, o_gx = self.empty(cap, torch.int32), self.empty(cap, torch.float64), self.empty(cap, torch.float64)
        count = C.c_int64(0)
        p = self.ptr
        _lib.check(self.lib.nodal_source_tree_rows(
            self.ctx, kcl, n, nnz_full, rb, re, p(forest["depth"]), p(rhs), rows.nnz, p(rows.indptr), p(rows.indices),
            p(rows.data), p(x), p(row), p(o_rhs), p(o_gx), C.byref(count), self.stream()), "nodal_source_tree_rows")
        k = count.value
        return row[:k], o_rhs[:k], o_gx[:k]

    def source_currents(self, kcl, etab, forest, info, tree_row, tree_rhs, tree_gx, x):
        p, f = self.ptr, forest
        _lib.check(self.lib.nodal_source_currents(
            self.ctx, kcl, info["sources"], p(f["erow"]), p(etab["a"]), p(etab["b"]), p(etab["branch"]),
            p(f["adj_ptr"]), p(f["adj_row"]), p(f["depth"]), info["depth"], int(tree_row.numel()), p(tree_row),
            p(tree_rhs), p(tree_gx), p(x), self.stream()), "nodal_source_currents")

    def source_residual(self, n, nnz_full, rows, rhs, x):
        sums = (C.c_double * 2)()
        p = self.ptr
        _lib.check(self.lib.nodal_source_residual(self.ctx, n, nnz_full, int(rhs.numel()), p(rhs), rows.nnz,
                                                  p(rows.indptr), p(rows.indices), p(rows.data), p(x), sums,
                                                  self.stream()), "nodal_source_residual")
        return sums[0], sums[1]

    def amg(self, csr: DeviceCSR, **params):
        return DeviceAMG(self, csr, **params)

    def amg_pcg(self, csr: DeviceCSR, rhs, rtol=1e-10, maxit=None, x0=None, **params):
        amg = DeviceAMG(self, csr, **params)
        try:
            return amg.solve(rhs, rtol=rtol, maxit=maxit, x0=x0)
        finally:
            amg.close()

    def gmres(self, csr: DeviceCSR, rhs, rtol=1e-12, restart=60, maxit=20000):
        n = csr.n
        x = self.zeros(max(2, n), self.torch.float64)[:n]
        iters, relres = C.c_int32(0), C.c_double(0.0)
        p = self.ptr
        st = self.lib.nodal_gmres(self.ctx, n, csr.nnz, p(csr.indptr), p(csr.indices), p(csr.data),
                                  p(rhs), p(x), rtol, restart, maxit, C.byref(iters),
                                  C.byref(relres), self.stream())
        _lib.check(st, "nodal_gmres", allowed=(_lib.OK, _lib.NOT_CONVERGED, _lib.BREAKDOWN))
        return x, dict(solver="gmres", status=st, iterations=iters.value, relres=relres.value)

    def lu_solve(self, G, rhs):
        n = int(G.shape[0])
        x = self.empty(max(1, n), self.torch.float64)[:n]
        info = C.c_int32(0)
        p = self.ptr
        st = self.lib.nodal_lu_solve(self.ctx, n, p(G), p(rhs), p(x), C.byref(info), self.stream())
        _lib.check(st, "nodal_lu_solve", allowed=(_lib.OK, _lib.SINGULAR))
        return x, dict(solver="lu", status=st, info=info.value)

    def lu_batched(self, table: ComponentTable, values, layout="aos"):
        torch = self.torch
        if layout not in ("aos", "soa"):
            raise ValueError("layout must be 'aos' or 'soa'")
        soa = layout == "soa"
        batch, ncomp = (int(values.shape[1]), int(values.shape[0])) if soa else (int(values.shape[0]), int(values.shape[1]))
        if ncomp != len(table):
            raise ValueError("values must have one entry per component of the topology")
        if not values.is_contiguous():
            values = values.contiguous()
        n = table.n
        dtab = self.upload_table(table)
        x = self.empty(max(1, batch * n), torch.float64)[: batch * n]
        x = x.view(n, batch) if soa else x.view(batch, n)
        info = self.empty(max(1, batch), torch.int32)[:batch]
        p = self.ptr
        fn = self.lib.nodal_lu_batched_soa if soa else self.lib.nodal_lu_batched
        _lib.check(fn(self.ctx, batch, ncomp, p(dtab["type"]), p(dtab["a"]), p(dtab["b"]), p(dtab["c"]),
                      p(dtab["d"]), p(dtab["drv"]), p(dtab["branch"]), table.kcl, n, p(values), p(x),
                      p(info), self.stream()), "nodal_lu_batched")
        return x, info
```

### nodal_b200/dist.py

```python
from __future__ import annotations

import ctypes as C

import numpy as np

from . import _lib
from .table import ComponentTable


def partition_rows(n, world):
    base, extra = divmod(int(n), int(world))
    sizes = np.full(world, base, dtype=np.int64)
    sizes[:extra] += 1
    bounds = np.zeros(world + 1, dtype=np.int32)
    np.cumsum(sizes, out=bounds[1:])
    return bounds


def local_component_table(table: ComponentTable, rb: int, re: int) -> ComponentTable:
    if not table.is_spd_structured():
        raise NotImplementedError("row-partitioned solve is implemented for R / A netlists (PCG)")
    a, b = table.a, table.b
    mask = ((a >= rb) & (a < re)) | ((b >= rb) & (b < re))
    sel = np.flatnonzero(mask)
    return ComponentTable(table.type[sel], table.value[sel], a[sel], b[sel], table.c[sel], table.d[sel],
                          table.drv[sel], table.branch[sel], kcl=table.kcl, be=table.be)


def broadcast_bytes(payload: bytes | None, nbytes: int, src: int = 0, device=None) -> bytes:
    import torch
    import torch.distributed as dist
    buf = torch.zeros(nbytes, dtype=torch.uint8)
    if dist.get_rank() == src:
        buf = torch.tensor(list(payload), dtype=torch.uint8)
    if device is not None:
        buf = buf.to(device)
    dist.broadcast(buf, src=src)
    return bytes(buf.cpu().tolist())


class DistPCG:

    def __init__(self, dev, rank, world):
        self.dev, self.rank, self.world = dev, int(rank), int(world)
        lib = dev.lib
        ident = None
        if self.rank == 0:
            raw = (C.c_uint8 * 128)()
            _lib.check(lib.nodal_dist_unique_id(raw), "nodal_dist_unique_id")
            ident = bytes(raw)
        if self.world > 1:
            ident = broadcast_bytes(ident, 128, src=0, device=dev.dev)
        h = C.c_void_p()
        raw = (C.c_uint8 * 128).from_buffer_copy(ident)
        _lib.check(lib.nodal_dist_create(dev.ctx, raw, self.rank, self.world, C.byref(h)), "nodal_dist_create")
        self.handle = h

    @classmethod
    def single(cls, dev):
        self = cls.__new__(cls)
        self.dev, self.rank, self.world = dev, 0, 1
        h = C.c_void_p()
        _lib.check(dev.lib.nodal_dist_create_single(dev.ctx, C.byref(h)), "nodal_dist_create_single")
        self.handle = h
        return self

    def close(self):
        if self.handle:
            self.dev.lib.nodal_dist_destroy(self.handle)
            self.handle = None

    def assemble_local(self, table_local: ComponentTable, bounds, dtab=None):
        dev = self.dev
        rb, re = int(bounds[self.rank]), int(bounds[self.rank + 1])
        csr, rhs = dev.assemble_csr(table_local, dtab=dtab)
        ip = csr.indptr[rb: re + 1]
        s, e = int(ip[0]), int(ip[-1])
        indptr = (ip - ip[0]).contiguous()
        return indptr, csr.indices[s:e], csr.data[s:e], rhs[rb:re]

    AMG_PARAMS = ("passes", "coarse", "omega", "scale", "maxlevels", "rounds", "direct_max", "gather_below", "max_fill")

    def solve_amg(self, n_global, bounds, indptr, indices, data, rhs_local, rtol=1e-10, maxit=None, x0=None, **params):
        dev, torch = self.dev, self.dev.torch
        unknown = set(params) - set(self.AMG_PARAMS)
        if unknown:
            raise TypeError(f"unknown AMG parameter(s): {sorted(unknown)}")
        nloc = int(bounds[self.rank + 1] - bounds[self.rank])
        x = dev.zeros(max(2, nloc), torch.float64)[:nloc] if x0 is None else x0.clone()
        b = np.ascontiguousarray(bounds, dtype=np.int32)
        arr = (C.c_double * 9)(*[float(params.get(k, 0.0)) for k in self.AMG_PARAMS])
        iters, relres = C.c_int32(0), C.c_double(0.0)
        stats = (C.c_double * 32)()
        p = dev.ptr
        st = dev.lib.nodal_dist_amg_pcg(dev.ctx, self.handle, int(n_global), b.ctypes.data_as(C.c_void_p),
                                        int(data.numel()), p(indptr), p(indices), p(data), p(rhs_local), p(x), arr,
                                        rtol, int(maxit or 1000), C.byref(iters), C.byref(relres), stats, dev.stream())
        _lib.check(st, "nodal_dist_amg_pcg", allowed=(_lib.OK, _lib.NOT_CONVERGED, _lib.BREAKDOWN))
        nlev = int(stats[8]) + 1
        info = dict(solver="dist_amg_pcg", status=st, iterations=iters.value, relres=relres.value,
                    restarts=int(stats[2]), solve_ms=stats[3], setup_ms=stats[4], levels=int(stats[0]),
                    distributed_levels=int(stats[8]), level_rows=[int(stats[16 + l]) for l in range(min(nlev, 12))],
                    replicated_rows=int(stats[11]), coarsest_rows=int(stats[5]), coarsest_direct=bool(stats[7]),
                    comm="p2p" if stats[9] else ("nccl" if self.world > 1 else "none"),
                    kernels_per_iteration=int(stats[10]), halo_recv=int(stats[12]), nnz=int(data.numel()))
        return x, info

    def solve(self, n_global, bounds, indptr, indices, data, rhs_local, rtol=1e-10, maxit=None):
        dev, torch = self.dev, self.dev.torch
        nloc = int(bounds[self.rank + 1] - bounds[self.rank])
        x = dev.zeros(max(2, nloc), torch.float64)[:nloc]
        if maxit is None:
            maxit = max(5000, 40 * int(np.sqrt(max(n_global, 1))))
        b = np.ascontiguousarray(bounds, dtype=np.int32)
        iters, relres = C.c_int32(0), C.c_double(0.0)
        stats = (C.c_double * 16)()
        p = dev.ptr
        st = dev.lib.nodal_dist_pcg(dev.ctx, self.handle, int(n_global), b.ctypes.data_as(C.c_void_p),
                                    int(data.numel()), p(indptr), p(indices), p(data), p(rhs_local), p(x),
                                    rtol, maxit, C.byref(iters), C.byref(relres), stats, dev.stream())
        _lib.check(st, "nodal_dist_pcg", allowed=(_lib.OK, _lib.NOT_CONVERGED, _lib.BREAKDOWN))
        info = dict(solver="dist_pcg", status=st, iterations=iters.value, relres=relres.value,
                    restarts=int(stats[2]), solve_ms=stats[3], setup_ms=stats[4],
                    format="sell32" if stats[5] else "csr", stored_nnz=int(stats[6]),
                    halo_recv=int(stats[12]), halo_send=int(stats[13]), nnz=int(data.numel()),
                    comm={0: "nccl", 1: "p2p", 2: "p2p-fused"}[int(stats[9])], scaled=bool(stats[8]),
                    host_ms=dict(run=stats[14], graph_teardown=stats[15], buffer_teardown=stats[11],
                                 graph_capture=stats[10]))
        return x, info


class LocalRows:

    def __init__(self, n, bounds, rank, indptr, indices, data):
        self.n, self.bounds, self.rank = int(n), bounds, int(rank)
        self.indptr, self.indices, self.data = indptr, indices, data

    @property
    def nnz(self):
        return int(self.data.numel())

    @property
    def shape(self):
        return (int(self.bounds[self.rank + 1] - self.bounds[self.rank]), self.n)

    def tocsr(self):
        import scipy.sparse as sps
        return sps.csr_matrix((self.data.cpu().numpy(), self.indices.cpu().numpy(), self.indptr.cpu().numpy()),
                              shape=self.shape)


_SOLVERS = {}


def shared_solver(dev, rank, world):
    key = (dev.index, int(rank), int(world))
    if key not in _SOLVERS or not _SOLVERS[key].handle:
        _SOLVERS[key] = DistPCG(dev, rank, world)
    return _SOLVERS[key]


def single_solver(dev):
    key = (dev.index, "single")
    if key not in _SOLVERS or not _SOLVERS[key].handle:
        _SOLVERS[key] = DistPCG.single(dev)
    return _SOLVERS[key]


def upload_share(dev, table, names, rank, world):
    m = len(table)
    lo, hi = m * rank // world, m * (rank + 1) // world
    pinned = getattr(table, "_pinned", None)
    if pinned:
        share = {k: pinned[k][lo:hi].to(dev.dev, non_blocking=True) for k in names}
    else:
        share = {k: dev.to_device(getattr(table, k)[lo:hi]) for k in names}
    for k in ("type", "value", "a", "b", "c", "d", "drv", "branch"):
        share.setdefault(k, None)
    return share


def exchange_rows(dev, share, ncomp, bounds, rank, world, select):
    if world == 1:
        return share, ncomp
    import torch
    import torch.distributed as dist
    names = [k for k, v in share.items() if v is not None]
    pieces, counts = [], []
    for d in range(world):
        sel, cnt = select(share, ncomp, int(bounds[d]), int(bounds[d + 1]))
        pieces.append(sel)
        counts.append(cnt)
    send_counts = torch.tensor(counts, dtype=torch.int64, device=dev.dev)
    recv_counts = torch.empty_like(send_counts)
    dist.all_to_all_single(recv_counts, send_counts)
    recv_split = [int(v) for v in recv_counts.tolist()]
    total = sum(recv_split)
    local = {k: None for k in share}
    for k in names:
        send = torch.cat([pieces[d][k][: counts[d]] for d in range(world)])
        recv = torch.empty(max(1, total), dtype=send.dtype, device=dev.dev)[:total]
        dist.all_to_all_single(recv, send, output_split_sizes=recv_split, input_split_sizes=counts)
        local[k] = recv
    return local, total


class GridRunner:

    def __init__(self, dev, table, probe_row, rank, world, rtol=1e-10, precond="jacobi", amg=None, solver=None):
        if not table.is_spd_structured():
            raise NotImplementedError("row-partitioned solve is implemented for R / A netlists (PCG)")
        self.dev, self.rank, self.world, self.rtol = dev, rank, world, rtol
        self.precond, self.amg = precond, dict(amg or {})
        self.table = table
        self.n = table.n
        self.bounds = partition_rows(self.n, world)
        self.probe_row = int(probe_row)
        self.owner = int(np.searchsorted(self.bounds, self.probe_row, side="right") - 1)
        self.pcg = solver if solver is not None else DistPCG(dev, rank, world)
        self._host_x = None
        self.x_local = None

    def close(self):
        self.pcg.close()

    def step_e2e(self):
        torch = self.dev.torch
        if getattr(self.table, "_pinned", None) is None:
            self.table.pin_memory()
        if self._host_x is None:
            nloc = int(self.bounds[self.rank + 1] - self.bounds[self.rank])
            self._host_x = torch.empty(nloc, dtype=torch.float64).pin_memory()
        return self.step(None, download=True)

    def assemble(self, dtab):
        from .device import coo_stride
        dev = self.dev
        rb, re = int(self.bounds[self.rank]), int(self.bounds[self.rank + 1])
        ncomp = len(self.table)
        if self.world > 1:
            dtab, ncomp = dev.select_local(dtab, ncomp, rb, re)
        csr, rhs = dev.assemble_csr_raw(dtab, ncomp, self.table.kcl, self.n, coo_stride(self.table))
        ip = csr.indptr[rb: re + 1]
        s, e = int(ip[0]), int(ip[-1])
        return (ip - ip[0]).contiguous(), csr.indices[s:e], csr.data[s:e], rhs[rb:re]

    def assemble_from_host(self):
        from .device import coo_stride
        dev, table = self.dev, self.table
        R, r, m = self.world, self.rank, len(table)
        if not table.is_spd_structured():
            raise NotImplementedError("row-partitioned solve is implemented for R / A netlists (PCG)")
        share = upload_share(dev, table, ("type", "value", "a", "b"), r, R)
        rb, re = int(self.bounds[r]), int(self.bounds[r + 1])
        local, ncomp = exchange_rows(dev, share, m * (r + 1) // R - m * r // R, self.bounds, r, R, dev.select_local)
        csr, rhs = dev.assemble_csr_raw(local, ncomp, table.kcl, self.n, coo_stride(table))
        ip = csr.indptr[rb: re + 1]
        s, e = int(ip[0]), int(ip[-1])
        return (ip - ip[0]).contiguous(), csr.indices[s:e], csr.data[s:e], rhs[rb:re]

    def step(self, dtab, download=False):
        import time
        torch = self.dev.torch
        t0 = time.perf_counter()
        indptr, indices, data, rhs = self.assemble(dtab) if dtab is not None else self.assemble_from_host()
        torch.cuda.synchronize()
        t1 = time.perf_counter()
        if self.precond == "amg":
            x, info = self.pcg.solve_amg(self.n, self.bounds, indptr, indices, data, rhs, rtol=self.rtol, **self.amg)
        else:
            x, info = self.pcg.solve(self.n, self.bounds, indptr, indices, data, rhs, rtol=self.rtol)
        t2 = time.perf_counter()
        info["assemble_wall_ms"] = (t1 - t0) * 1e3
        info["solve_wall_ms"] = (t2 - t1) * 1e3
        if download:
            self._host_x.copy_(x, non_blocking=True)
            torch.cuda.synchronize()
        r = torch.zeros(1, dtype=torch.float64, device=self.dev.dev)
        if self.rank == self.owner:
            r[0] = x[self.probe_row - int(self.bounds[self.rank])]
        nnz = torch.tensor([info["nnz"]], dtype=torch.int64, device=self.dev.dev)
        if self.world > 1:
            import torch.distributed as dist
            dist.broadcast(r, src=self.owner)
            dist.all_reduce(nnz)
        info["nnz"] = int(nnz.item())
        self.x_local = x
        return float(r.item()), info
```

Baseline: 144.2 million.

## Add compressed stencil encoding for uniform SELL slices in AMG sweeps

While building the SELL matrix, the fill kernel checks each 32-row slice for identical column offsets and values across all lanes. Such slices get one shared (offset, value) record per column, and the AMG smoother, residual and distributed SpMV kernels read these broadcast records instead of the per-lane cols and vals arrays. This cuts memory traffic on regular grid matrices. In exchange it adds a per-slice branch, extra setup-time shuffles and atomics, a host sync during SELL creation, and some extra storage.

```diff
diff --git a/__graft_entry__.py b/__graft_entry__.py
--- a/__graft_entry__.py
+++ b/__graft_entry__.py
@@ -17,6 +17,8 @@
     sources_host.sources_host_lib()
     import amg_cycle_host
     amg_cycle_host.amg_cycle_host_lib()
+    import sell_stencil_host
+    sell_stencil_host.sell_stencil_host_lib()
     ref_nodal = os.path.join(os.environ.get("NODAL_REFERENCE", "/root/reference"), "nodal")
     if os.path.isdir(ref_nodal) and not os.path.isfile(os.path.join(ROOT, "baseline", "_ref", "nodal", "nodal.py")):
         subprocess.call([sys.executable, os.path.join(ROOT, "baseline", "install_ref.py")])
diff --git a/include/nodal_b200.h b/include/nodal_b200.h
--- a/include/nodal_b200.h
+++ b/include/nodal_b200.h
@@ -63,6 +63,7 @@
                       const int32_t* indices, const double* data, nodal_sell** out, void* stream);
 int nodal_sell_destroy(nodal_sell* m);
 int64_t nodal_sell_padded_nnz(const nodal_sell* m);
+int64_t nodal_sell_stencil_slices(const nodal_sell* m);
 int nodal_sell_spmv(nodal_ctx* ctx, const nodal_sell* m, const double* x, double* y, void* stream);
 
 int nodal_pcg(nodal_ctx* ctx, int32_t n, int64_t nnz, const int32_t* indptr,
@@ -86,6 +87,8 @@
 int nodal_amg_destroy(nodal_amg* amg);
 int nodal_amg_info(const nodal_amg* amg, int32_t cap, int32_t* nlevels, int64_t* rows, int64_t* nnz,
                    double* setup_ms, int32_t* direct);
+int nodal_amg_stencil_info(const nodal_amg* amg, int32_t cap, int64_t* slices, int64_t* records,
+                           int32_t* record_bytes);
 int nodal_amg_fetch_level(nodal_ctx* ctx, const nodal_amg* amg, int32_t level, int32_t* agg,
                           int32_t* indptr, int32_t* indices, double* data, void* stream);
 int nodal_amg_apply(nodal_ctx* ctx, const nodal_amg* amg, const double* r, double* z, void* stream);
diff --git a/nodal_b200/_lib.py b/nodal_b200/_lib.py
--- a/nodal_b200/_lib.py
+++ b/nodal_b200/_lib.py
@@ -29,6 +29,7 @@
     "nodal_sell_create": (C.c_int, [_vp, _i32, _i64, _vp, _vp, _vp, C.POINTER(_vp), _vp]),
     "nodal_sell_destroy": (C.c_int, [_vp]),
     "nodal_sell_padded_nnz": (_i64, [_vp]),
+    "nodal_sell_stencil_slices": (_i64, [_vp]),
     "nodal_sell_spmv": (C.c_int, [_vp, _vp, _vp, _vp, _vp]),
     "nodal_pcg": (C.c_int, [_vp, _i32, _i64, _vp, _vp, _vp, _vp, _vp, _f64, _i32, _i32,
                             C.POINTER(_i32), C.POINTER(_f64), C.POINTER(_f64), _vp]),
@@ -38,6 +39,7 @@
     "nodal_amg_destroy": (C.c_int, [_vp]),
     "nodal_amg_info": (C.c_int, [_vp, _i32, C.POINTER(_i32), C.POINTER(_i64), C.POINTER(_i64),
                                  C.POINTER(_f64), C.POINTER(_i32)]),
+    "nodal_amg_stencil_info": (C.c_int, [_vp, _i32, C.POINTER(_i64), C.POINTER(_i64), C.POINTER(_i32)]),
     "nodal_amg_fetch_level": (C.c_int, [_vp, _vp, _i32, _vp, _vp, _vp, _vp, _vp]),
     "nodal_amg_apply": (C.c_int, [_vp, _vp, _vp, _vp, _vp]),
     "nodal_amg_pcg": (C.c_int, [_vp, _vp, _vp, _vp, _f64, _i32, C.POINTER(_i32), C.POINTER(_f64),
diff --git a/nodal_b200/csrc/amg.cu b/nodal_b200/csrc/amg.cu
--- a/nodal_b200/csrc/amg.cu
+++ b/nodal_b200/csrc/amg.cu
@@ -290,20 +290,22 @@
 
 template <int MODE>
 int sell_sweep(const nodal_amg* h, const AmgLevel& V, const double* b, const double* x, double* y,
-               double* part, cudaStream_t st) {
+               double* part, cudaStream_t st, bool stencil = true) {
     const nodal_sell* m = V.sell;
     amg_sell_kernel<MODE><<<sell_grid(h->ctx, m->nslices), AT, 0, st>>>(
-        m->n, m->nslices, m->slice_w, m->cols, m->vals, m->dinv, b, x, h->omega, y, part);
+        m->n, m->nslices, m->slice_w, m->cols, m->vals, stencil ? m->st_off : nullptr, m->st_val, m->dinv, b, x,
+        h->omega, y, part);
     KERNEL_CHECK();
     return NODAL_OK;
 }
 
 template <int MODE>
 int cycle_sweep(const nodal_amg* h, const AmgLevel& V, const double* b, const double* xc, double* y,
-                cudaStream_t st) {
+                cudaStream_t st, bool stencil = true) {
     const nodal_sell* m = V.sell;
     amg_cycle_sweep_kernel<MODE><<<sell_grid(h->ctx, m->nslices), AT, 0, st>>>(
-        m->n, m->nslices, m->slice_w, m->cols, m->vals, m->dinv, b, h->omega, V.agg, xc, h->scale, y);
+        m->n, m->nslices, m->slice_w, m->cols, m->vals, stencil ? m->st_off : nullptr, m->st_val, m->dinv, b,
+        h->omega, V.agg, xc, h->scale, y);
     KERNEL_CHECK();
     return NODAL_OK;
 }
@@ -423,6 +425,17 @@
     }
     if (setup_ms) *setup_ms = h->setup_ms;
     if (direct) *direct = h->inv ? 1 : 0;
+    return NODAL_OK;
+}
+
+extern "C" int nodal_amg_stencil_info(const nodal_amg* h, int32_t cap, int64_t* slices, int64_t* records,
+                                      int32_t* record_bytes) {
+    if (!h) return NODAL_BAD_ARG;
+    for (int32_t l = 0; l < (int32_t)h->lv.size() && l < cap; ++l) {
+        if (slices) slices[l] = h->lv[l].sell->st_slices;
+        if (records) records[l] = h->lv[l].sell->st_cols;
+    }
+    if (record_bytes) *record_bytes = SELL_ST_RECORD_BYTES;
     return NODAL_OK;
 }
 
@@ -588,9 +601,9 @@
     for (int mode = 0; mode < 3 && rc == NODAL_OK; ++mode) {
         for (int k = -2; k < reps && rc == NODAL_OK; ++k) {
             if (k == 0) cudaEventRecord(e0, st);
-            if (mode == 0) rc = sell_sweep<0>(h, A, nullptr, h->p, h->q, h->part, st);
-            if (mode == 1) rc = sell_sweep<1>(h, A, h->r, h->p, h->q, nullptr, st);
-            if (mode == 2) rc = sell_sweep<2>(h, A, h->r, h->p, h->q, nullptr, st);
+            if (mode == 0) rc = sell_sweep<0>(h, A, nullptr, h->p, h->q, h->part, st, false);
+            if (mode == 1) rc = sell_sweep<1>(h, A, h->r, h->p, h->q, nullptr, st, false);
+            if (mode == 2) rc = sell_sweep<2>(h, A, h->r, h->p, h->q, nullptr, st, false);
         }
         cudaEventRecord(e1, st);
         float ms = 0.f;
@@ -616,7 +629,8 @@
     CUDA_TRY(cudaEventCreate(&e0));
     CUDA_TRY(cudaEventCreate(&e1));
     int rc = NODAL_OK;
-    for (int k = 0; k < 6 && rc == NODAL_OK; ++k) {
+    CUDA_TRY(cudaMemsetAsync(h->p, 0, sizeof(double) * (size_t)A.n, st));
+    for (int k = 0; k < 10 && rc == NODAL_OK; ++k) {
         for (int i = -2; i < reps && rc == NODAL_OK; ++i) {
             if (i == 0) cudaEventRecord(e0, st);
             switch (k) {
@@ -624,13 +638,17 @@
                     amg_jacobi0_kernel<<<rows_grid(ctx, A.n), AT, 0, st>>>(A.n, A.sell->dinv, b, h->omega, A.x);
                     KERNEL_CHECK();
                     break;
-                case 1: rc = sell_sweep<1>(h, A, b, A.x, A.r, nullptr, st); break;
+                case 1: rc = sell_sweep<1>(h, A, b, A.x, A.r, nullptr, st, false); break;
                 case 2:
                     amg_prolong_kernel<<<rows_grid(ctx, A.n), AT, 0, st>>>(A.n, A.agg, C.x, h->scale, A.x, A.r);
                     KERNEL_CHECK();
                     break;
-                case 3: rc = sell_sweep<2>(h, A, b, A.r, h->z, nullptr, st); break;
-                case 4: rc = cycle_sweep<1>(h, A, b, nullptr, A.r, st); break;
+                case 3: rc = sell_sweep<2>(h, A, b, A.r, h->z, nullptr, st, false); break;
+                case 4: rc = cycle_sweep<1>(h, A, b, nullptr, A.r, st, false); break;
+                case 5: rc = cycle_sweep<2>(h, A, b, C.x, h->z, st, false); break;
+                case 6: rc = sell_sweep<0>(h, A, nullptr, h->p, h->q, h->part, st, false); break;
+                case 7: rc = sell_sweep<0>(h, A, nullptr, h->p, h->q, h->part, st); break;
+                case 8: rc = cycle_sweep<1>(h, A, b, nullptr, A.r, st); break;
                 default: rc = cycle_sweep<2>(h, A, b, C.x, h->z, st); break;
             }
         }
diff --git a/nodal_b200/csrc/amg_kernels.cuh b/nodal_b200/csrc/amg_kernels.cuh
--- a/nodal_b200/csrc/amg_kernels.cuh
+++ b/nodal_b200/csrc/amg_kernels.cuh
@@ -127,6 +127,7 @@
 static __global__ void __launch_bounds__(AT, 5)
 amg_sell_kernel(int32_t n, int32_t nslices, const u32* __restrict__ slice_w,
                 const int32_t* __restrict__ cols, const double* __restrict__ vals,
+                const int32_t* __restrict__ st_off, const double* __restrict__ st_val,
                 const double* __restrict__ dinv, const double* __restrict__ b,
                 const double* __restrict__ x, double omega, double* __restrict__ y,
                 double* __restrict__ part) {
@@ -138,8 +139,9 @@
     for (int64_t s = warp; s < nslices; s += nwarps) {
         const u32 w0 = slice_w[s];
         const int w = (int)(slice_w[s + 1] - w0);
-        const double acc = sell_row_dot(cols, vals, (int64_t)w0 * 32 + lane, w, x);
         const int64_t r = s * 32 + lane;
+        const double acc = sell_row_gather_st(cols, vals, st_off, st_val, w0, w, (int64_t)w0 * 32 + lane,
+                                              (int32_t)r, SellLoad{x});
         if (r < n) {
             if (MODE == 0) { y[r] = acc; dot = fma(x[r], acc, dot); }
             if (MODE == 1) y[r] = amg_residual(b[r], acc);
@@ -192,6 +194,7 @@
 static __global__ void __launch_bounds__(AT, 5)
 amg_cycle_sweep_kernel(int32_t n, int32_t nslices, const u32* __restrict__ slice_w,
                        const int32_t* __restrict__ cols, const double* __restrict__ vals,
+                       const int32_t* __restrict__ st_off, const double* __restrict__ st_val,
                        const double* __restrict__ dinv, const double* __restrict__ b, double omega,
                        const int32_t* __restrict__ agg, const double* __restrict__ xc, double scale,
                        double* __restrict__ y) {
@@ -206,11 +209,11 @@
         const int64_t base = (int64_t)w0 * 32 + lane;
         const int64_t r = s * 32 + lane;
         if (MODE == 1) {
-            const double acc = sell_row_gather(cols, vals, base, w, x0);
+            const double acc = sell_row_gather_st(cols, vals, st_off, st_val, w0, w, base, (int32_t)r, x0);
             if (r < n) y[r] = amg_residual(b[r], acc);
         }
         if (MODE == 2) {
-            const double acc = sell_row_gather(cols, vals, base, w, xa);
+            const double acc = sell_row_gather_st(cols, vals, st_off, st_val, w0, w, base, (int32_t)r, xa);
             if (r < n) y[r] = amg_jacobi_update(omega, dinv[r], b[r], acc, xa((int32_t)r));
         }
     }
diff --git a/nodal_b200/csrc/dist_amg.cu b/nodal_b200/csrc/dist_amg.cu
--- a/nodal_b200/csrc/dist_amg.cu
+++ b/nodal_b200/csrc/dist_amg.cu
@@ -218,7 +218,8 @@
 
 __global__ void __launch_bounds__(DA, 5)
 acg_spmv_dots_kernel(int32_t n, int32_t nslices, const u32* __restrict__ slice_w, const int32_t* __restrict__ cols,
-                     const double* __restrict__ vals, const double* __restrict__ u, const double* __restrict__ r,
+                     const double* __restrict__ vals, const int32_t* __restrict__ st_off,
+                     const double* __restrict__ st_val, const double* __restrict__ u, const double* __restrict__ r,
                      double* __restrict__ w, double* __restrict__ part_g, double* __restrict__ part_d) {
     __shared__ double sm[40];
     const int lane = threadIdx.x & 31;
@@ -228,8 +229,9 @@
     for (int64_t s = warp; s < nslices; s += nwarps) {
         const u32 w0 = slice_w[s];
         const int wd = (int)(slice_w[s + 1] - w0);
-        const double acc = sell_row_dot(cols, vals, (int64_t)w0 * 32 + lane, wd, u);
         const int64_t row = s * 32 + lane;
+        const double acc = sell_row_gather_st(cols, vals, st_off, st_val, w0, wd, (int64_t)w0 * 32 + lane, (int32_t)row,
+                                              SellLoad{u});
         if (row < n) {
             const double uv = __ldg(&u[row]);
             w[row] = acc;
@@ -763,7 +765,7 @@
 int sweep(Solver& S, const DLevel& L, const double* b, const double* x, double* y, cudaStream_t sx) {
     const nodal_sell* m = L.sell;
     amg_sell_kernel<MODE><<<amg_sell_grid(S.ctx, m->nslices), AT, 0, sx>>>(
-        m->n, m->nslices, m->slice_w, m->cols, m->vals, m->dinv, b, x, S.omega, y, nullptr);
+        m->n, m->nslices, m->slice_w, m->cols, m->vals, m->st_off, m->st_val, m->dinv, b, x, S.omega, y, nullptr);
     KERNEL_CHECK();
     return NODAL_OK;
 }
@@ -772,7 +774,7 @@
 int cycle_sweep(Solver& S, const DLevel& L, const double* b, const double* xc, double* y, cudaStream_t sx) {
     const nodal_sell* m = L.sell;
     amg_cycle_sweep_kernel<MODE><<<amg_sell_grid(S.ctx, m->nslices), AT, 0, sx>>>(
-        m->n, m->nslices, m->slice_w, m->cols, m->vals, m->dinv, b, S.omega, L.agg, xc, S.scale, y);
+        m->n, m->nslices, m->slice_w, m->cols, m->vals, m->st_off, m->st_val, m->dinv, b, S.omega, L.agg, xc, S.scale, y);
     KERNEL_CHECK();
     return NODAL_OK;
 }
@@ -1021,8 +1023,8 @@
             KERNEL_CHECK();
             NODAL_TRY(cycle(S, nullptr, r, u, st));
             NODAL_TRY(exchange(S, nullptr, 2 * ND, F.halo, u_off, st));
-            acg_spmv_dots_kernel<<<gs, DA, 0, st>>>(n, F.sell->nslices, F.sell->slice_w, F.sell->cols, F.sell->vals, u, r, w,
-                                                    part_g, part_d);
+            acg_spmv_dots_kernel<<<gs, DA, 0, st>>>(n, F.sell->nslices, F.sell->slice_w, F.sell->cols, F.sell->vals,
+                                                    F.sell->st_off, F.sell->st_val, u, r, w, part_g, part_d);
             KERNEL_CHECK();
             NODAL_TRY(allreduce(0, part_g, gs, part_d, gs, part_rr, gv, part_bb, gv, SC, 0, st));
             acg_scalars_kernel<<<1, 32, 0, st>>>(dev, SC, rtol, maxit, first);
@@ -1036,8 +1038,8 @@
             KERNEL_CHECK();
             NODAL_TRY(cycle(S, dev, r, u, sx));
             NODAL_TRY(exchange(S, dev, 2 * ND, F.halo, u_off, sx));
-            acg_spmv_dots_kernel<<<gs, DA, 0, sx>>>(n, F.sell->nslices, F.sell->slice_w, F.sell->cols, F.sell->vals, u, r, w,
-                                                    part_g, part_d);
+            acg_spmv_dots_kernel<<<gs, DA, 0, sx>>>(n, F.sell->nslices, F.sell->slice_w, F.sell->cols, F.sell->vals,
+                                                    F.sell->st_off, F.sell->st_val, u, r, w, part_g, part_d);
             KERNEL_CHECK();
             NODAL_TRY(allreduce(1, part_g, gs, part_d, gs, part_rr, gv, nullptr, 0, nxt, 1, sx));
             return NODAL_OK;
@@ -1148,6 +1150,7 @@
         stats_h[10] = (double)launches_per_iter;
         stats_h[11] = (double)S.rep_n;
         stats_h[12] = (double)S.halo_total;
+        stats_h[13] = S.lv.empty() || !S.lv[0].sell ? 0.0 : (double)S.lv[0].sell->st_slices;
         for (size_t l = 0; l < S.lv.size() && l < 12; ++l) stats_h[16 + l] = (double)S.lv[l].nglob;
     }
     for (int par = 0; par < 2; ++par) {
diff --git a/nodal_b200/csrc/sell_stencil_core.cuh b/nodal_b200/csrc/sell_stencil_core.cuh
--- /dev/null
+++ b/nodal_b200/csrc/sell_stencil_core.cuh
@@ -0,0 +1,31 @@
+#pragma once
+#include <stdint.h>
+
+#if defined(__CUDACC__)
+#define SELLST_HD __host__ __device__ __forceinline__
+#else
+#include <string.h>
+#define SELLST_HD static inline
+#endif
+
+#define SELL_ST_EXPLICIT INT32_MIN
+
+SELLST_HD bool sell_st_row_ok(int64_t row, int32_t n, int32_t len, uint32_t w) {
+    return row < (int64_t)n && (uint32_t)len == w;
+}
+
+SELLST_HD int32_t sell_st_offset(int32_t col, int64_t row) { return (int32_t)((int64_t)col - row); }
+
+SELLST_HD uint64_t sell_st_bits(double v) {
+#if defined(__CUDA_ARCH__)
+    return (uint64_t)__double_as_longlong(v);
+#else
+    uint64_t b;
+    memcpy(&b, &v, sizeof b);
+    return b;
+#endif
+}
+
+SELLST_HD bool sell_st_same(int32_t off, uint64_t bits, int32_t off0, uint64_t bits0) {
+    return off == off0 && bits == bits0;
+}
diff --git a/nodal_b200/csrc/sparse.cuh b/nodal_b200/csrc/sparse.cuh
--- a/nodal_b200/csrc/sparse.cuh
+++ b/nodal_b200/csrc/sparse.cuh
@@ -1,5 +1,6 @@
 #pragma once
 #include "common.cuh"
+#include "sell_stencil_core.cuh"
 
 struct nodal_sell {
     nodal_ctx* ctx = nullptr;
@@ -13,7 +14,13 @@
     double* vals = nullptr;
     size_t store_bytes = 0;
     double* dinv = nullptr;
+    int32_t* st_off = nullptr;
+    double* st_val = nullptr;
+    int64_t st_slices = 0;
+    int64_t st_cols = 0;
 };
+
+constexpr int SELL_ST_RECORD_BYTES = (int)(sizeof(int32_t) + sizeof(double));
 
 int sell_from_csr(nodal_ctx* ctx, int32_t n, int64_t nnz, const int32_t* indptr,
                   const int32_t* indices, const double* data, nodal_sell** out, cudaStream_t st,
@@ -81,4 +88,45 @@
                                                const double* __restrict__ x) {
     return sell_row_gather(cols, vals, base, w, SellLoad{x});
 }
+
+template <int W, class G>
+__device__ __forceinline__ double sell_dot_stencil(const int32_t* __restrict__ st_off,
+                                                   const double* __restrict__ st_val, u32 k0, int32_t row,
+                                                   const G& gather, double acc) {
+    int32_t c[W];
+    double v[W], xv[W];
+#pragma unroll
+    for (int i = 0; i < W; ++i) {
+        c[i] = row + __ldg(&st_off[k0 + i]);
+        v[i] = __ldg(&st_val[k0 + i]);
+    }
+#pragma unroll
+    for (int i = 0; i < W; ++i) xv[i] = gather(c[i]);
+#pragma unroll
+    for (int i = 0; i < W; ++i) acc = amg_dot_step(v[i], xv[i], acc);
+    return acc;
+}
+
+template <class G>
+__device__ __forceinline__ double sell_row_gather_st(const int32_t* __restrict__ cols,
+                                                     const double* __restrict__ vals,
+                                                     const int32_t* __restrict__ st_off,
+                                                     const double* __restrict__ st_val, u32 w0, int w,
+                                                     int64_t base, int32_t row, const G& x) {
+    if (st_off == nullptr || w == 0 || __ldg(&st_off[w0]) == SELL_ST_EXPLICIT)
+        return sell_row_gather(cols, vals, base, w, x);
+    double acc = 0.0;
+    int k = 0;
+    for (; k + 6 <= w; k += 6) acc = sell_dot_stencil<6>(st_off, st_val, w0 + k, row, x, acc);
+    const u32 k0 = w0 + k;
+    switch (w - k) {
+        case 5: acc = sell_dot_stencil<5>(st_off, st_val, k0, row, x, acc); break;
+        case 4: acc = sell_dot_stencil<4>(st_off, st_val, k0, row, x, acc); break;
+        case 3: acc = sell_dot_stencil<3>(st_off, st_val, k0, row, x, acc); break;
+        case 2: acc = sell_dot_stencil<2>(st_off, st_val, k0, row, x, acc); break;
+        case 1: acc = sell_dot_stencil<1>(st_off, st_val, k0, row, x, acc); break;
+        default: break;
+    }
+    return acc;
+}
 #endif
diff --git a/nodal_b200/csrc/spmv.cu b/nodal_b200/csrc/spmv.cu
--- a/nodal_b200/csrc/spmv.cu
+++ b/nodal_b200/csrc/spmv.cu
@@ -91,7 +91,8 @@
 sell_fill_kernel(int32_t n, int32_t nslices, const int32_t* __restrict__ indptr,
                  const int32_t* __restrict__ indices, const double* __restrict__ data,
                  const u32* __restrict__ slice_w, const double* __restrict__ sc,
-                 int32_t* __restrict__ cols, double* __restrict__ vals, double* __restrict__ dinv) {
+                 int32_t* __restrict__ cols, double* __restrict__ vals, double* __restrict__ dinv,
+                 int32_t* __restrict__ st_off, double* __restrict__ st_val, u32* __restrict__ st_count) {
     const int lane = threadIdx.x & 31;
     const int64_t warp = ((int64_t)blockIdx.x * blockDim.x + threadIdx.x) >> 5;
     const int64_t nwarps = ((int64_t)gridDim.x * blockDim.x) >> 5;
@@ -102,6 +103,7 @@
         if (r < n) { b = indptr[r]; e = indptr[r + 1]; }
         double diag = 0.0;
         const int64_t base = (int64_t)w0 * 32 + lane;
+        bool stencil = sell_st_row_ok(r, n, e - b, w);
         for (u32 k = 0; k < w; ++k) {
             int32_t c = r < n ? (int32_t)r : 0;
             double v = 0.0;
@@ -113,8 +115,23 @@
             }
             cols[base + (int64_t)k * 32] = c;
             vals[base + (int64_t)k * 32] = v;
+            const int32_t off = sell_st_offset(c, r);
+            const u64 bits = sell_st_bits(v);
+            const int32_t off0 = __shfl_sync(0xffffffffu, off, 0);
+            const u64 bits0 = __shfl_sync(0xffffffffu, bits, 0);
+            stencil = stencil && sell_st_same(off, bits, off0, bits0);
+            if (lane == 0) { st_off[w0 + k] = off; st_val[w0 + k] = v; }
         }
         if (r < n) dinv[r] = diag != 0.0 ? 1.0 / diag : 1.0;
+        const bool all = __all_sync(0xffffffffu, stencil);
+        if (w > 0 && lane == 0) {
+            if (all) {
+                atomicAdd(&st_count[0], 1u);
+                atomicAdd(&st_count[1], w);
+            } else {
+                st_off[w0] = SELL_ST_EXPLICIT;
+            }
+        }
     }
 }
 
@@ -123,6 +140,7 @@
     cudaSetDevice(m->device);
     ctx_pool_free(m->ctx, m->slice_w);
     ctx_pool_free(m->ctx, m->vals);
+    ctx_pool_free(m->ctx, m->st_val);
     ctx_pool_free(m->ctx, m->dinv);
     delete m;
 }
@@ -180,10 +198,18 @@
     PA(vals, double, sizeof(double) * alloc + sizeof(int32_t) * alloc);
     m->cols = reinterpret_cast<int32_t*>(m->vals + alloc);
     m->store_bytes = (sizeof(double) + sizeof(int32_t)) * alloc;
+    const size_t records = (size_t)(host_tot[0] > 0 ? host_tot[0] : 1);
+    PA(st_val, double, (sizeof(double) + sizeof(int32_t)) * records);
+    m->st_off = reinterpret_cast<int32_t*>(m->st_val + records);
 #undef PA
-    sell_fill_kernel<<<grid, SPMV_THREADS, 0, st>>>(n, m->nslices, indptr, indices, data,
-                                                    m->slice_w, sc, m->cols, m->vals, m->dinv);
+    CT(cudaMemsetAsync(tot + 1, 0, 2 * sizeof(u32), st));
+    sell_fill_kernel<<<grid, SPMV_THREADS, 0, st>>>(n, m->nslices, indptr, indices, data, m->slice_w, sc, m->cols,
+                                                    m->vals, m->dinv, m->st_off, m->st_val, tot + 1);
     CT(cudaGetLastError());
+    CT(cudaMemcpyAsync(host_tot, tot + 1, 2 * sizeof(u32), cudaMemcpyDeviceToHost, st));
+    CT(cudaStreamSynchronize(st));
+    m->st_slices = host_tot[0];
+    m->st_cols = host_tot[1];
 #undef CT
     *out = m;
     return NODAL_OK;
@@ -220,6 +246,8 @@
 }
 
 extern "C" int64_t nodal_sell_padded_nnz(const nodal_sell* m) { return m ? m->padded : 0; }
+
+extern "C" int64_t nodal_sell_stencil_slices(const nodal_sell* m) { return m ? m->st_slices : 0; }
 
 extern "C" int nodal_sell_spmv(nodal_ctx* ctx, const nodal_sell* m, const double* x, double* y,
                                void* stream) {
diff --git a/nodal_b200/device.py b/nodal_b200/device.py
--- a/nodal_b200/device.py
+++ b/nodal_b200/device.py
@@ -77,6 +77,12 @@
         self.rows = [int(rows[k]) for k in range(nl.value)]
         self.nnz = [int(nnz[k]) for k in range(nl.value)]
         self.setup_ms, self.direct = ms.value, bool(direct.value)
+        slices, records, rec_bytes = (C.c_int64 * cap)(), (C.c_int64 * cap)(), C.c_int32(0)
+        _lib.check(dev.lib.nodal_amg_stencil_info(h, cap, slices, records, C.byref(rec_bytes)),
+                   "nodal_amg_stencil_info")
+        self.stencil_slices = [int(slices[k]) for k in range(nl.value)]
+        self.stencil_records = [int(records[k]) for k in range(nl.value)]
+        self.stencil_record_bytes = rec_bytes.value
 
     def close(self):
         if self.handle:
@@ -136,10 +142,11 @@
         return dict(spmv_dot=ms[0], residual=ms[1], jacobi=ms[2])
 
     def profile_cycle(self, reps=64):
-        ms = (C.c_double * 6)()
+        ms = (C.c_double * 10)()
         _lib.check(self.dev.lib.nodal_amg_profile_cycle(self.dev.ctx, self.handle, int(reps), ms, self.dev.stream()),
                    "nodal_amg_profile_cycle")
-        return dict(zip(("jacobi0", "residual", "prolong", "jacobi", "fused_residual", "fused_post"), list(ms)))
+        return dict(zip(("jacobi0", "residual", "prolong", "jacobi", "fused_residual", "fused_post", "spmv_dot",
+                         "spmv_dot_stencil", "fused_residual_stencil", "fused_post_stencil"), list(ms)))
 
     def solve(self, rhs, rtol=1e-10, maxit=None, x0=None):
         dev, n = self.dev, self.csr.n
diff --git a/nodal_b200/dist.py b/nodal_b200/dist.py
--- a/nodal_b200/dist.py
+++ b/nodal_b200/dist.py
@@ -103,7 +103,8 @@
                     distributed_levels=int(stats[8]), level_rows=[int(stats[16 + l]) for l in range(min(nlev, 12))],
                     replicated_rows=int(stats[11]), coarsest_rows=int(stats[5]), coarsest_direct=bool(stats[7]),
                     comm="p2p" if stats[9] else ("nccl" if self.world > 1 else "none"),
-                    kernels_per_iteration=int(stats[10]), halo_recv=int(stats[12]), nnz=int(data.numel()))
+                    kernels_per_iteration=int(stats[10]), halo_recv=int(stats[12]), stencil_slices=int(stats[13]),
+                    nnz=int(data.numel()))
         return x, info
 
     def solve(self, n_global, bounds, indptr, indices, data, rhs_local, rtol=1e-10, maxit=None):
```

After: 150.5 million, median of 6. +4.4%, better.
